# modal-labs/modal-client

Measured on AMD Instinct MI355X. Metric: map_items_per_sec, higher is better.
Workload: dtype bf16; 1 GPU; model=Function.map fan-out (BASELINE config 3), global_batch=12500, seq_len=0, parallelism=map1, dynamic_batching=64, chunk_items=256, workers=8

## Files before the change

csrc/core.cpp:

```cpp

#include <pybind11/pybind11.h>
#include <pybind11/stl.h>

#include "lane.h"
#include "ring.h"

#include <algorithm>
#include <atomic>
#include <functional>
#include <thread>
#include <cerrno>
#include <cstdint>
#include <cstring>
#include <fcntl.h>
#include <stdexcept>
#include <string>
#include <sys/mman.h>
#include <sys/stat.h>
#include <unistd.h>
#include <vector>

namespace py = pybind11;

namespace {

using modal_amd::BellFile;
using modal_amd::Ring;
using modal_amd::RingHub;

constexpr uint64_t kGilReleaseBytes = 64 * 1024;

bool ring_push(Ring& ring, py::buffer buf) {
  py::buffer_info info = buf.request();
  const uint8_t* src = static_cast<const uint8_t*>(info.ptr);
  const uint64_t n = (uint64_t)info.size * (uint64_t)info.itemsize;
  uint8_t* dst = ring.reserve(n);
  if (!dst) return false;
  if (n >= kGilReleaseBytes) {
    py::gil_scoped_release release;
    std::memcpy(dst, src, n);
  } else {
    std::memcpy(dst, src, n);
  }
  ring.commit();
  return true;
}

py::list ring_pop_all(Ring& ring, size_t max_frames) {
  py::list out;
  ring.pop(
      [&](const uint8_t* ptr, size_t len) {
        out.append(py::bytes(reinterpret_cast<const char*>(ptr), len));
      },
      max_frames);
  return out;
}

py::list hub_drain(RingHub& hub) {
  py::list out;
  hub.drain([&](int slot, const uint8_t* ptr, size_t len) {
    out.append(py::make_tuple(slot, py::bytes(reinterpret_cast<const char*>(ptr), len)));
  });
  return out;
}

using modal_amd::Assignment;
using modal_amd::ChunkDone;
using modal_amd::ChunkLane;
using modal_amd::FrameKind;

py::str sv_str(std::string_view s) { return py::str(s.data(), s.size()); }

py::tuple done_tuple(const ChunkDone& d) {
  py::object cis = py::none();
  if (!d.cis_nil) {
    py::list items;
    for (int64_t v : d.cis) items.append(py::int_(v));
    cis = std::move(items);
  }
  return py::make_tuple(sv_str(d.token), sv_str(d.call_id), sv_str(d.chunk_id),
                        sv_str(d.function_id), py::int_(d.count),
                        py::bytes(d.data.data(), d.data.size()), cis);
}

py::list assignment_list(const std::vector<Assignment>& assignments) {
  py::list out;
  for (const auto& a : assignments) out.append(py::make_tuple(a.token, a.worker_slot));
  return out;
}

py::object parse_chunk_done_py(py::buffer buf) {
  py::buffer_info info = buf.request();
  ChunkDone done;
  FrameKind kind = modal_amd::parse_chunk_done(
      static_cast<const uint8_t*>(info.ptr), (size_t)info.size * (size_t)info.itemsize, &done);
  if (kind != FrameKind::kDoneClean) return py::none();
  return done_tuple(done);
}

int lane_submit(ChunkLane& lane, int fn_slot, const std::string& token, uint64_t count,
                py::buffer frame, bool front) {
  py::buffer_info info = frame.request();
  return lane.submit(fn_slot, token, count, static_cast<const uint8_t*>(info.ptr),
                     (size_t)info.size * (size_t)info.itemsize, front);
}

py::tuple lane_drain(ChunkLane& lane, RingHub& hub) {
  py::list completions, raw;
  std::vector<Assignment> assignments;
  lane.drain(
      hub,
      [&](int slot, const ChunkDone& done) {
        completions.append(py::make_tuple(slot, done_tuple(done)));
      },
      [&](int slot, const uint8_t* ptr, size_t len) {
        raw.append(py::make_tuple(slot, py::bytes(reinterpret_cast<const char*>(ptr), len)));
      },
      &assignments);
  return py::make_tuple(completions, raw, assignment_list(assignments));
}

py::bytes pack_payloads(const std::vector<py::bytes>& items) {
  uint64_t total = 0;
  std::vector<std::pair<const char*, size_t>> views;
  views.reserve(items.size());
  for (const auto& item : items) {
    char* ptr;
    Py_ssize_t n;
    if (PyBytes_AsStringAndSize(item.ptr(), &ptr, &n) != 0)
      throw std::runtime_error("pack_payloads: not bytes");
    views.emplace_back(ptr, (size_t)n);
    total += 4 + (uint64_t)n;
  }
  std::string out;
  out.resize(total);
  {
    py::gil_scoped_release release;
    char* dst = out.data();
    for (const auto& [ptr, n] : views) {
      uint32_t len32 = (uint32_t)n;
      std::memcpy(dst, &len32, 4);
      std::memcpy(dst + 4, ptr, n);
      dst += 4 + n;
    }
  }
  return py::bytes(out);
}

py::list unpack_payloads(py::buffer buf) {
  py::buffer_info info = buf.request();
  const char* src = static_cast<const char*>(info.ptr);
  size_t n = (size_t)info.size * (size_t)info.itemsize;
  py::list out;
  size_t pos = 0;
  while (pos + 4 <= n) {
    uint32_t len32;
    std::memcpy(&len32, src + pos, 4);
    if (pos + 4 + len32 > n) throw std::runtime_error("unpack_payloads: truncated");
    out.append(py::bytes(src + pos + 4, len32));
    pos += 4 + len32;
  }
  if (pos != n) throw std::runtime_error("unpack_payloads: trailing bytes");
  return out;
}

}



static constexpr int kSegSize = 4096;
static constexpr int kMinMatch = 4;
static constexpr int kMFLimit = 12;
static constexpr int kLastLiterals = 5;

static inline uint32_t lz4_hash(uint32_t v) { return (v * 2654435761u) >> (32 - 12); }

static size_t lz4_compress_one(const uint8_t* src, size_t n, uint8_t* dst, size_t dst_cap) {
  uint16_t table[1 << 12];
  std::memset(table, 0, sizeof(table));
  size_t op = 0, ip = 0, anchor = 0;
  auto emit = [&](size_t lit_start, size_t lit_len, int match_len) -> bool {
    size_t need = 1 + lit_len + (lit_len >= 15 ? 1 + (lit_len - 15) / 255 : 0) +
                  (match_len >= 0 ? 2 + 1 + 16 : 0);
    if (op + need + 8 > dst_cap) return false;
    int ml = match_len >= 0 ? match_len - kMinMatch : 0;
    uint8_t token = (uint8_t)((lit_len < 15 ? lit_len : 15) << 4);
    if (match_len >= 0) token |= (uint8_t)(ml < 15 ? ml : 15);
    dst[op++] = token;
    if (lit_len >= 15) {
      size_t rest = lit_len - 15;
      while (rest >= 255) { dst[op++] = 255; rest -= 255; }
      dst[op++] = (uint8_t)rest;
    }
    std::memcpy(dst + op, src + lit_start, lit_len);
    op += lit_len;
    return true;
  };
  if (n >= (size_t)(kMinMatch + kLastLiterals)) {
    size_t mflimit = n >= kMFLimit ? n - kMFLimit : 0;
    while (ip < mflimit) {
      uint32_t seq;
      std::memcpy(&seq, src + ip, 4);
      uint32_t h = lz4_hash(seq);
      size_t cand = table[h];
      table[h] = (uint16_t)ip;
      uint32_t cseq;
      bool ok = cand < ip && ip - cand <= 0xFFFF;
      if (ok) { std::memcpy(&cseq, src + cand, 4); ok = cseq == seq; }
      if (ok) {
        size_t mlen = kMinMatch;
        size_t maxm = n - kLastLiterals - ip;
        while (mlen < maxm && src[cand + mlen] == src[ip + mlen]) mlen++;
        if (!emit(anchor, ip - anchor, (int)mlen)) return 0;
        size_t off = ip - cand;
        dst[op++] = (uint8_t)(off & 0xFF);
        dst[op++] = (uint8_t)(off >> 8);
        int ml = (int)mlen - kMinMatch;
        if (ml >= 15) {
          int rest = ml - 15;
          while (rest >= 255) { dst[op++] = 255; rest -= 255; }
          dst[op++] = (uint8_t)rest;
        }
        ip += mlen;
        anchor = ip;
      } else {
        ip++;
      }
    }
  }
  if (!emit(anchor, n - anchor, -1)) return 0;
  return op;
}

static bool lz4_decompress_one(const uint8_t* src, size_t comp_len,
                               uint8_t* dst, size_t raw_len) {
  size_t ip = 0, op = 0;
  while (ip < comp_len) {
    uint8_t token = src[ip++];
    size_t lit = token >> 4;
    if (lit == 15) {
      uint8_t b;
      do { if (ip >= comp_len) return false; b = src[ip++]; lit += b; } while (b == 255);
    }
    if (ip + lit > comp_len || op + lit > raw_len) return false;
    std::memcpy(dst + op, src + ip, lit);
    ip += lit; op += lit;
    if (ip >= comp_len) break;
    if (ip + 2 > comp_len) return false;
    size_t off = src[ip] | ((size_t)src[ip + 1] << 8);
    ip += 2;
    if (off == 0 || off > op) return false;
    size_t mlen = (token & 0xF) + kMinMatch;
    if ((token & 0xF) == 15) {
      uint8_t b;
      do { if (ip >= comp_len) return false; b = src[ip++]; mlen += b; } while (b == 255);
    }
    if (op + mlen > raw_len) return false;
    if (off >= mlen) {
      std::memcpy(dst + op, dst + op - off, mlen);
    } else {
      for (size_t k = 0; k < mlen; k++) dst[op + k] = dst[op - off + k];
    }
    op += mlen;
  }
  return op == raw_len;
}

static void parallel_for(size_t n, const std::function<void(size_t, size_t)>& body) {
  unsigned hw = std::thread::hardware_concurrency();
  size_t n_threads = std::min<size_t>(std::max(1u, hw / 2), 8);
  if (n < 8 || n_threads <= 1) { body(0, n); return; }
  std::vector<std::thread> threads;
  size_t chunk = (n + n_threads - 1) / n_threads;
  for (size_t t = 0; t < n_threads; t++) {
    size_t lo = t * chunk, hi = std::min(n, lo + chunk);
    if (lo >= hi) break;
    threads.emplace_back([&body, lo, hi] { body(lo, hi); });
  }
  for (auto& th : threads) th.join();
}

py::object malz_compress(py::bytes data, double min_gain) {
  char* buf; ssize_t n_s;
  if (PyBytes_AsStringAndSize(data.ptr(), &buf, &n_s) != 0) throw py::error_already_set();
  size_t n = (size_t)n_s;
  size_t n_seg = (n + kSegSize - 1) / kSegSize;
  if (n_seg == 0) return py::none();
  std::vector<uint32_t> comp_lens(n_seg, 0);
  std::vector<std::vector<uint8_t>> outs(n_seg);
  const uint8_t* src = (const uint8_t*)buf;
  {
    py::gil_scoped_release release;
    parallel_for(n_seg, [&](size_t lo, size_t hi) {
      for (size_t i = lo; i < hi; i++) {
        size_t seg_off = i * kSegSize;
        size_t seg_len = std::min((size_t)kSegSize, n - seg_off);
        outs[i].resize(kSegSize);
        size_t c = lz4_compress_one(src + seg_off, seg_len, outs[i].data(), seg_len > 1 ? seg_len - 1 : 0);
        if (c > 0 && c < seg_len) {
          comp_lens[i] = (uint32_t)c;
          outs[i].resize(c);
        } else {
          comp_lens[i] = 0;
          outs[i].clear();
        }
      }
    });
  }
  size_t total = 0;
  for (size_t i = 0; i < n_seg; i++) {
    size_t seg_len = std::min((size_t)kSegSize, n - i * kSegSize);
    total += comp_lens[i] ? comp_lens[i] : seg_len;
  }
  if ((double)total >= (double)n * min_gain) return py::none();
  size_t header = 6 + 12 + 4 * n_seg;
  py::bytes out_obj(nullptr, (ssize_t)(header + total));
  uint8_t* out = (uint8_t*)PyBytes_AsString(out_obj.ptr());
  std::memcpy(out, "MALZ41", 6);
  uint64_t n64 = n;
  uint32_t ns32 = (uint32_t)n_seg;
  std::memcpy(out + 6, &n64, 8);
  std::memcpy(out + 14, &ns32, 4);
  std::memcpy(out + 18, comp_lens.data(), 4 * n_seg);
  size_t op = header;
  for (size_t i = 0; i < n_seg; i++) {
    size_t seg_off = i * kSegSize;
    size_t seg_len = std::min((size_t)kSegSize, n - seg_off);
    if (comp_lens[i]) {
      std::memcpy(out + op, outs[i].data(), comp_lens[i]);
      op += comp_lens[i];
    } else {
      std::memcpy(out + op, src + seg_off, seg_len);
      op += seg_len;
    }
  }
  return out_obj;
}

py::bytes malz_decompress(py::bytes blob) {
  char* buf; ssize_t bn;
  if (PyBytes_AsStringAndSize(blob.ptr(), &buf, &bn) != 0) throw py::error_already_set();
  if (bn < 18 || std::memcmp(buf, "MALZ41", 6) != 0)
    throw std::runtime_error("not a MALZ41 container");
  uint64_t raw_len;
  uint32_t n_seg;
  std::memcpy(&raw_len, buf + 6, 8);
  std::memcpy(&n_seg, buf + 14, 4);
  size_t header = 6 + 12 + 4 * (size_t)n_seg;
  if ((size_t)bn < header) throw std::runtime_error("truncated container header");
  std::vector<uint32_t> comp_lens(n_seg);
  std::memcpy(comp_lens.data(), buf + 18, 4 * (size_t)n_seg);
  std::vector<size_t> seg_payload_off(n_seg);
  size_t pos = header;
  for (size_t i = 0; i < n_seg; i++) {
    seg_payload_off[i] = pos;
    size_t seg_len = std::min((size_t)kSegSize, (size_t)raw_len - i * kSegSize);
    pos += comp_lens[i] ? comp_lens[i] : seg_len;
  }
  if (pos > (size_t)bn) throw std::runtime_error("truncated container payload");
  py::bytes out_obj(nullptr, (ssize_t)raw_len);
  uint8_t* out = (uint8_t*)PyBytes_AsString(out_obj.ptr());
  const uint8_t* src = (const uint8_t*)buf;
  std::atomic<bool> ok{true};
  {
    py::gil_scoped_release release;
    parallel_for(n_seg, [&](size_t lo, size_t hi) {
      for (size_t i = lo; i < hi; i++) {
        size_t seg_off = i * kSegSize;
        size_t seg_len = std::min((size_t)kSegSize, (size_t)raw_len - seg_off);
        if (comp_lens[i] == 0) {
          std::memcpy(out + seg_off, src + seg_payload_off[i], seg_len);
        } else if (!lz4_decompress_one(src + seg_payload_off[i], comp_lens[i],
                                       out + seg_off, seg_len)) {
          ok.store(false, std::memory_order_relaxed);
        }
      }
    });
  }
  if (!ok.load()) throw std::runtime_error("corrupt LZ4 segment");
  return out_obj;
}




#include <sys/syscall.h>
#include <sys/resource.h>
#include <sched.h>
#include <signal.h>

namespace {

struct clone_args_compat {
  uint64_t flags;
  uint64_t pidfd;
  uint64_t child_tid;
  uint64_t parent_tid;
  uint64_t exit_signal;
  uint64_t stack;
  uint64_t stack_size;
  uint64_t tls;
  uint64_t set_tid;
  uint64_t set_tid_size;
  uint64_t cgroup;
};

#ifndef CLONE_INTO_CGROUP
#define CLONE_INTO_CGROUP 0x200000000ULL
#endif

}

static int64_t spawn_supervised(const std::vector<std::string>& argv,
                                const std::string& cwd,
                                const std::vector<std::string>& env,
                                const std::string& cgroup_dir,
                                int64_t rlimit_as_mib,
                                int stdin_fd, int stdout_fd, int stderr_fd) {
  if (argv.empty()) throw std::runtime_error("empty argv");
  int cg_fd = -1;
  if (!cgroup_dir.empty()) {
    cg_fd = ::open(cgroup_dir.c_str(), O_DIRECTORY | O_RDONLY | O_CLOEXEC);
    if (cg_fd < 0)
      throw std::runtime_error("open cgroup dir: " + std::string(strerror(errno)));
  }

  std::vector<char*> cargv;
  cargv.reserve(argv.size() + 1);
  for (const auto& a : argv) cargv.push_back(const_cast<char*>(a.c_str()));
  cargv.push_back(nullptr);
  std::vector<char*> cenv;
  cenv.reserve(env.size() + 1);
  for (const auto& e : env) cenv.push_back(const_cast<char*>(e.c_str()));
  cenv.push_back(nullptr);

  clone_args_compat ca{};
  ca.exit_signal = SIGCHLD;
  if (cg_fd >= 0) {
    ca.flags = CLONE_INTO_CGROUP;
    ca.cgroup = (uint64_t)cg_fd;
  }

  long pid = syscall(SYS_clone3, &ca, sizeof(ca));
  if (pid < 0 && cg_fd >= 0 && (errno == EINVAL || errno == ENOSYS || errno == EPERM ||
                                errno == EBADF || errno == EOPNOTSUPP)) {
    ::close(cg_fd);
    cg_fd = -1;
    throw std::runtime_error("clone3(CLONE_INTO_CGROUP) unavailable: " +
                             std::string(strerror(errno)));
  }
  if (pid < 0) {
    if (cg_fd >= 0) ::close(cg_fd);
    throw std::runtime_error("clone3: " + std::string(strerror(errno)));
  }
  if (pid == 0) {
    ::setsid();
    if (stdin_fd >= 0) ::dup2(stdin_fd, 0);
    if (stdout_fd >= 0) ::dup2(stdout_fd, 1);
    if (stderr_fd >= 0) ::dup2(stderr_fd, 2);
    for (int fd = 3; fd < 1024; ++fd) ::close(fd);
    if (!cwd.empty() && ::chdir(cwd.c_str()) != 0) _exit(126);
    if (rlimit_as_mib > 0) {
      struct rlimit rl;
      rl.rlim_cur = rl.rlim_max = (rlim_t)rlimit_as_mib << 20;
      ::setrlimit(RLIMIT_AS, &rl);
    }
    ::execve(cargv[0], cargv.data(), cenv.data());
    _exit(127);
  }
  if (cg_fd >= 0) ::close(cg_fd);
  return (int64_t)pid;
}


PYBIND11_MODULE(_core, m) {
  m.doc() = "modal_amd native core: shm ring transport + batch framing";
  py::class_<BellFile, std::shared_ptr<BellFile>>(m, "BellFile")
      .def(py::init<const std::string&, bool>(), py::arg("path"), py::arg("create") = false);
  py::class_<Ring, std::shared_ptr<Ring>>(m, "ShmRing")
      .def(py::init<const std::string&, uint64_t, bool>(), py::arg("path"),
           py::arg("capacity") = (uint64_t)64 << 20, py::arg("create") = false)
      .def("push", &ring_push)
      .def("pop_all", &ring_pop_all, py::arg("max_frames") = 0)
      .def("pending_bytes", &Ring::pending_bytes)
      .def("capacity", &Ring::capacity)
      .def("too_large", &Ring::too_large)
      .def("bell_wakes", &Ring::bell_wakes)
      .def("set_shared_bell", &Ring::set_shared_bell);
  py::class_<RingHub>(m, "RingHub")
      .def(py::init<const std::string&, int>(), py::arg("bell_path") = "",
           py::arg("timeout_ms") = 20)
      .def("add_ring", &RingHub::add_ring)
      .def("remove_ring", &RingHub::remove_ring)
      .def("fd", &RingHub::fd)
      .def("drain", &hub_drain)
      .def("close", &RingHub::close)
      .def("stats", [](RingHub& hub) {
        py::dict d;
        d["notifies"] = hub.notifies();
        d["waits"] = hub.waits();
        d["drains"] = hub.drains();
        d["producer_wakes"] = hub.producer_wakes();
        d["rings"] = hub.ring_count();
        return d;
      });
  py::class_<ChunkLane>(m, "ChunkLane")
      .def(py::init<>())
      .def("add_worker", &ChunkLane::add_worker)
      .def("remove_worker", &ChunkLane::remove_worker)
      .def("set_eligible", &ChunkLane::set_eligible)
      .def("set_cap", &ChunkLane::set_cap, py::arg("fn_slot"), py::arg("items"),
           py::arg("min_chunks") = 1)
      .def("submit", &lane_submit, py::arg("fn_slot"), py::arg("token"), py::arg("count"),
           py::arg("frame"), py::arg("front") = false)
      .def("kick", [](ChunkLane& lane, int fn_slot) {
        std::vector<Assignment> out;
        lane.kick(fn_slot, &out);
        return assignment_list(out);
      })
      .def("complete", [](ChunkLane& lane, int worker_slot, const std::string& token) {
        std::vector<Assignment> out;
        lane.complete(worker_slot, token, &out);
        return assignment_list(out);
      })
      .def("cancel", &ChunkLane::cancel)
      .def("drop_queue", &ChunkLane::drop_queue)
      .def("drain", &lane_drain)
      .def("queued", &ChunkLane::queued)
      .def("inflight", &ChunkLane::inflight)
      .def("outstanding_items", &ChunkLane::outstanding_items)
      .def("pushed", &ChunkLane::pushed);
  m.def("parse_chunk_done", &parse_chunk_done_py);
  m.def("pack_payloads", &pack_payloads);
  m.def("malz_compress", &malz_compress, py::arg("data"), py::arg("min_gain") = 0.95);
  m.def("malz_decompress", &malz_decompress);
  m.def("unpack_payloads", &unpack_payloads);
  m.def("spawn_supervised", &spawn_supervised, py::arg("argv"), py::arg("cwd"),
        py::arg("env"), py::arg("cgroup_dir") = "", py::arg("rlimit_as_mib") = 0,
        py::arg("stdin_fd") = -1, py::arg("stdout_fd") = -1, py::arg("stderr_fd") = -1,
        "clone3(CLONE_INTO_CGROUP) + execve supervisor (atomic cgroup placement)");
}
```

csrc/lane.h:

```cpp

#pragma once

#include <algorithm>
#include <cstdint>
#include <cstring>
#include <deque>
#include <memory>
#include <string>
#include <string_view>
#include <unordered_map>
#include <unordered_set>
#include <utility>
#include <vector>

#include "ring.h"

namespace modal_amd {


struct MsgReader {
  const uint8_t* p;
  const uint8_t* end;

  bool need(size_t n) const { return (size_t)(end - p) >= n; }

  bool be(size_t n, uint64_t* out) {
    if (!need(n)) return false;
    uint64_t v = 0;
    for (size_t i = 0; i < n; i++) v = (v << 8) | p[i];
    p += n;
    *out = v;
    return true;
  }

  bool read_str(std::string_view* out) {
    if (!need(1)) return false;
    uint8_t tag = *p++;
    uint64_t n;
    if ((tag & 0xe0) == 0xa0) n = tag & 0x1f;
    else if (tag == 0xd9) { if (!be(1, &n)) return false; }
    else if (tag == 0xda) { if (!be(2, &n)) return false; }
    else if (tag == 0xdb) { if (!be(4, &n)) return false; }
    else return false;
    if (!need(n)) return false;
    *out = std::string_view(reinterpret_cast<const char*>(p), (size_t)n);
    p += n;
    return true;
  }

  bool read_bin(std::string_view* out) {
    if (!need(1)) return false;
    uint8_t tag = *p++;
    uint64_t n;
    if (tag == 0xc4) { if (!be(1, &n)) return false; }
    else if (tag == 0xc5) { if (!be(2, &n)) return false; }
    else if (tag == 0xc6) { if (!be(4, &n)) return false; }
    else return false;
    if (!need(n)) return false;
    *out = std::string_view(reinterpret_cast<const char*>(p), (size_t)n);
    p += n;
    return true;
  }

  bool read_int(int64_t* out) {
    if (!need(1)) return false;
    uint8_t tag = *p++;
    uint64_t v;
    if (tag <= 0x7f) { *out = tag; return true; }
    if (tag >= 0xe0) { *out = (int8_t)tag; return true; }
    switch (tag) {
      case 0xcc: if (!be(1, &v)) return false; *out = (int64_t)v; return true;
      case 0xcd: if (!be(2, &v)) return false; *out = (int64_t)v; return true;
      case 0xce: if (!be(4, &v)) return false; *out = (int64_t)v; return true;
      case 0xcf:
        if (!be(8, &v) || v > (uint64_t)INT64_MAX) return false;
        *out = (int64_t)v;
        return true;
      case 0xd0: if (!be(1, &v)) return false; *out = (int8_t)v; return true;
      case 0xd1: if (!be(2, &v)) return false; *out = (int16_t)v; return true;
      case 0xd2: if (!be(4, &v)) return false; *out = (int32_t)v; return true;
      case 0xd3: if (!be(8, &v)) return false; *out = (int64_t)v; return true;
      default: return false;
    }
  }

  bool read_map_header(uint64_t* n) {
    if (!need(1)) return false;
    uint8_t tag = *p++;
    if ((tag & 0xf0) == 0x80) { *n = tag & 0x0f; return true; }
    if (tag == 0xde) return be(2, n);
    if (tag == 0xdf) return be(4, n);
    return false;
  }

  bool read_array_header(uint64_t* n) {
    if (!need(1)) return false;
    uint8_t tag = *p++;
    if ((tag & 0xf0) == 0x90) { *n = tag & 0x0f; return true; }
    if (tag == 0xdc) return be(2, n);
    if (tag == 0xdd) return be(4, n);
    return false;
  }

  bool skip(int depth = 0) {
    if (depth > 32 || !need(1)) return false;
    uint8_t tag = *p++;
    uint64_t n;
    if (tag <= 0x7f || tag >= 0xe0) return true;
    if ((tag & 0xe0) == 0xa0) return adv(tag & 0x1f);
    if ((tag & 0xf0) == 0x90) return skip_n(tag & 0x0f, depth);
    if ((tag & 0xf0) == 0x80) return skip_n(2 * (uint64_t)(tag & 0x0f), depth);
    switch (tag) {
      case 0xc0: case 0xc2: case 0xc3: return true;
      case 0xc4: case 0xd9: return be(1, &n) && adv(n);
      case 0xc5: case 0xda: return be(2, &n) && adv(n);
      case 0xc6: case 0xdb: return be(4, &n) && adv(n);
      case 0xc7: return be(1, &n) && adv(n + 1);
      case 0xc8: return be(2, &n) && adv(n + 1);
      case 0xc9: return be(4, &n) && adv(n + 1);
      case 0xca: return adv(4);
      case 0xcb: return adv(8);
      case 0xcc: case 0xd0: return adv(1);
      case 0xcd: case 0xd1: return adv(2);
      case 0xce: case 0xd2: return adv(4);
      case 0xcf: case 0xd3: return adv(8);
      case 0xd4: return adv(2);
      case 0xd5: return adv(3);
      case 0xd6: return adv(5);
      case 0xd7: return adv(9);
      case 0xd8: return adv(17);
      case 0xdc: return be(2, &n) && skip_n(n, depth);
      case 0xdd: return be(4, &n) && skip_n(n, depth);
      case 0xde: return be(2, &n) && skip_n(2 * n, depth);
      case 0xdf: return be(4, &n) && skip_n(2 * n, depth);
      default: return false;
    }
  }

 private:
  bool adv(uint64_t n) {
    if (!need(n)) return false;
    p += n;
    return true;
  }
  bool skip_n(uint64_t n, int depth) {
    for (uint64_t i = 0; i < n; i++)
      if (!skip(depth + 1)) return false;
    return true;
  }
};

struct ChunkDone {
  std::string_view token, call_id, chunk_id, function_id, data;
  int64_t count = 0;
  bool cis_nil = true;
  std::vector<int64_t> cis;
};

enum class FrameKind {
  kOther,
  kDoneOther,
  kDoneClean,
};

inline bool ascii_only(std::string_view s) {
  for (unsigned char c : s)
    if (c >= 0x80) return false;
  return true;
}

inline FrameKind parse_chunk_done(const uint8_t* buf, size_t len, ChunkDone* out) {
  MsgReader r{buf, buf + len};
  uint64_t n_keys;
  if (!r.read_map_header(&n_keys)) return FrameKind::kOther;
  enum { T = 1, TOKEN = 2, CALL = 4, CHUNK = 8, FN = 16, COUNT = 32, DATA = 64, CIS = 128 };
  unsigned seen = 0;
  bool clean = n_keys == 8;
  bool is_done = false, has_token = false;
  std::string_view token;
  for (uint64_t i = 0; i < n_keys; i++) {
    std::string_view key;
    const uint8_t* key_at = r.p;
    if (!r.read_str(&key)) {
      r.p = key_at;
      if (!r.skip() || !r.skip()) return FrameKind::kOther;
      clean = false;
      continue;
    }
    unsigned bit = 0;
    if (key == "t") bit = T;
    else if (key == "token") bit = TOKEN;
    else if (key == "call_id") bit = CALL;
    else if (key == "chunk_id") bit = CHUNK;
    else if (key == "function_id") bit = FN;
    else if (key == "count") bit = COUNT;
    else if (key == "data") bit = DATA;
    else if (key == "cis") bit = CIS;
    if (bit == 0 || (seen & bit)) {
      if (bit & (T | TOKEN)) return FrameKind::kOther;
      if (!r.skip()) return FrameKind::kOther;
      clean = false;
      continue;
    }
    seen |= bit;
    const uint8_t* value_at = r.p;
    bool ok = true;
    std::string_view sv;
    switch (bit) {
      case T:
        ok = r.read_str(&sv);
        if (ok) is_done = sv == "chunk_done";
        break;
      case TOKEN:
        ok = r.read_str(&sv) && ascii_only(sv);
        if (ok) { token = sv; has_token = true; }
        break;
      case CALL: ok = r.read_str(&out->call_id) && ascii_only(out->call_id); break;
      case CHUNK: ok = r.read_str(&out->chunk_id) && ascii_only(out->chunk_id); break;
      case FN: ok = r.read_str(&out->function_id) && ascii_only(out->function_id); break;
      case COUNT: ok = r.read_int(&out->count) && out->count >= 0; break;
      case DATA: ok = r.read_bin(&out->data); break;
      case CIS: {
        if (r.need(1) && *r.p == 0xc0) {
          r.p++;
          out->cis_nil = true;
          break;
        }
        uint64_t n;
        ok = r.read_array_header(&n) && n <= (uint64_t)(r.end - r.p);
        out->cis_nil = false;
        out->cis.clear();
        for (uint64_t k = 0; ok && k < n; k++) {
          int64_t v;
          ok = r.read_int(&v);
          if (ok) out->cis.push_back(v);
        }
        break;
      }
    }
    if (!ok) {
      r.p = value_at;
      if (!r.skip()) return FrameKind::kOther;
      clean = false;
      if (bit == T) return FrameKind::kOther;
      if (bit == TOKEN) has_token = false;
    }
  }
  if (r.p != r.end) return FrameKind::kOther;
  if (!is_done || !has_token) return FrameKind::kOther;
  out->token = token;
  if (clean && seen == 255) return FrameKind::kDoneClean;
  return FrameKind::kDoneOther;
}


struct Assignment {
  std::string token;
  int worker_slot;
};

class ChunkLane {
 public:
  void add_worker(int slot, std::shared_ptr<Ring> ring) {
    Worker& w = workers_[slot];
    w.ring = std::move(ring);
  }

  std::vector<std::string> remove_worker(int slot) {
    std::vector<std::string> tokens;
    auto it = workers_.find(slot);
    if (it == workers_.end()) return tokens;
    for (auto& entry : it->second.inflight) tokens.push_back(entry.first);
    workers_.erase(it);
    for (auto& fn : fns_) fn.second.eligible.erase(slot);
    return tokens;
  }

  void set_eligible(int fn_slot, int worker_slot, bool on) {
    Fn& fn = fns_[fn_slot];
    if (on && workers_.count(worker_slot)) fn.eligible.insert(worker_slot);
    else fn.eligible.erase(worker_slot);
  }

  void set_cap(int fn_slot, uint64_t items, uint32_t min_chunks) {
    Fn& fn = fns_[fn_slot];
    fn.cap_items = items;
    fn.min_chunks = min_chunks;
  }

  int submit(int fn_slot, const std::string& token, uint64_t count, const uint8_t* frame,
             size_t len, bool front) {
    Fn& fn = fns_[fn_slot];
    if (fn.queue.empty() || front) {
      int slot = place(fn_slot, fn, token, count, frame, len, fn.queue.size());
      if (slot >= 0) return slot;
    }
    Queued q{token, count, std::string(reinterpret_cast<const char*>(frame), len)};
    if (front) fn.queue.push_front(std::move(q));
    else fn.queue.push_back(std::move(q));
    return -1;
  }

  void kick(int fn_slot, std::vector<Assignment>* out) {
    auto it = fns_.find(fn_slot);
    if (it == fns_.end()) return;
    Fn& fn = it->second;
    while (!fn.queue.empty()) {
      Queued& q = fn.queue.front();
      int slot = place(fn_slot, fn, q.token, q.count,
                       reinterpret_cast<const uint8_t*>(q.frame.data()), q.frame.size(),
                       fn.queue.size());
      if (slot < 0) break;
      out->push_back(Assignment{std::move(q.token), slot});
      fn.queue.pop_front();
    }
  }

  bool complete(int worker_slot, std::string_view token, std::vector<Assignment>* out) {
    auto wit = workers_.find(worker_slot);
    if (wit == workers_.end()) return false;
    Worker& w = wit->second;
    auto it = w.inflight.find(std::string(token));
    if (it == w.inflight.end()) return false;
    int fn_slot = it->second.fn_slot;
    Load& load = w.load[fn_slot];
    load.items -= std::min(load.items, it->second.count);
    if (load.chunks) load.chunks--;
    w.inflight.erase(it);
    kick(fn_slot, out);
    return true;
  }

  std::vector<std::string> cancel(const std::vector<std::string>& tokens) {
    std::unordered_set<std::string_view> drop(tokens.begin(), tokens.end());
    std::vector<std::string> dropped;
    for (auto& entry : fns_) {
      auto& q = entry.second.queue;
      auto keep = q.begin();
      for (auto it = q.begin(); it != q.end(); ++it) {
        if (drop.count(it->token)) {
          dropped.push_back(std::move(it->token));
        } else {
          if (keep != it) *keep = std::move(*it);
          ++keep;
        }
      }
      q.erase(keep, q.end());
    }
    return dropped;
  }

  std::vector<std::string> drop_queue(int fn_slot) {
    std::vector<std::string> tokens;
    auto it = fns_.find(fn_slot);
    if (it == fns_.end()) return tokens;
    for (auto& q : it->second.queue) tokens.push_back(std::move(q.token));
    it->second.queue.clear();
    return tokens;
  }

  template <typename OnClean, typename OnRaw>
  void drain(RingHub& hub, OnClean&& on_clean, OnRaw&& on_raw, std::vector<Assignment>* out) {
    ChunkDone done;
    hub.drain([&](int slot, const uint8_t* ptr, size_t len) {
      FrameKind kind = parse_chunk_done(ptr, len, &done);
      if (kind != FrameKind::kOther) complete(slot, done.token, out);
      if (kind == FrameKind::kDoneClean) on_clean(slot, done);
      else on_raw(slot, ptr, len);
    });
  }

  size_t queued(int fn_slot) const {
    auto it = fns_.find(fn_slot);
    return it == fns_.end() ? 0 : it->second.queue.size();
  }

  size_t inflight(int worker_slot) const {
    auto it = workers_.find(worker_slot);
    return it == workers_.end() ? 0 : it->second.inflight.size();
  }

  uint64_t outstanding_items(int fn_slot, int worker_slot) const {
    auto it = workers_.find(worker_slot);
    if (it == workers_.end()) return 0;
    auto lit = it->second.load.find(fn_slot);
    return lit == it->second.load.end() ? 0 : lit->second.items;
  }

  uint64_t pushed() const { return pushed_; }

 private:
  struct Queued {
    std::string token;
    uint64_t count;
    std::string frame;
  };
  struct Load {
    uint64_t items = 0;
    uint32_t chunks = 0;
  };
  struct Inflight {
    int fn_slot;
    uint64_t count;
  };
  struct Worker {
    std::shared_ptr<Ring> ring;
    std::unordered_map<int, Load> load;
    std::unordered_map<std::string, Inflight> inflight;
  };
  struct Fn {
    uint64_t cap_items = 256;
    uint32_t min_chunks = 1;
    std::deque<Queued> queue;
    std::unordered_set<int> eligible;
  };

  static bool has_credit(const Fn& fn, const Load& load, size_t backlog) {
    if (load.items < fn.cap_items) return true;
    return load.chunks < fn.min_chunks && backlog > fn.eligible.size();
  }

  int place(int fn_slot, Fn& fn, const std::string& token, uint64_t count,
            const uint8_t* frame, size_t len, size_t backlog) {
    std::vector<std::pair<uint64_t, int>> order;
    for (int slot : fn.eligible) {
      auto it = workers_.find(slot);
      if (it == workers_.end()) continue;
      const Load& load = it->second.load[fn_slot];
      if (has_credit(fn, load, backlog)) order.emplace_back(load.items, slot);
    }
    std::sort(order.begin(), order.end());
    for (auto& cand : order) {
      Worker& w = workers_[cand.second];
      if (w.ring->too_large(len) || !w.ring->push(frame, len)) continue;
      Load& load = w.load[fn_slot];
      load.items += count;
      load.chunks++;
      w.inflight[token] = Inflight{fn_slot, count};
      pushed_++;
      return cand.second;
    }
    return -1;
  }

  std::unordered_map<int, Worker> workers_;
  std::unordered_map<int, Fn> fns_;
  uint64_t pushed_ = 0;
};

}
```

modal_amd/flash.py:

```python

from __future__ import annotations

import math
import time
from dataclasses import dataclass, field
from typing import Callable, Optional


@dataclass
class FlashEndpoint:
    name: str
    url: str
    registered_at: float = field(default_factory=time.time)


class FlashManager:

    def __init__(self) -> None:
        self.endpoints: dict[str, FlashEndpoint] = {}

    def register(self, name: str, url: str) -> FlashEndpoint:
        ep = FlashEndpoint(name, url)
        self.endpoints[name] = ep
        return ep

    def deregister(self, name: str) -> None:
        self.endpoints.pop(name, None)

    def list(self) -> list[FlashEndpoint]:
        return list(self.endpoints.values())


class FlashAutoscaler:

    def __init__(
        self,
        get_metric: Callable[[], float],
        target_value: float,
        *,
        min_replicas: int = 1,
        max_replicas: int = 8,
        scale_up_stabilization: float = 0.0,
        scale_down_stabilization: float = 300.0,
        tolerance: float = 0.1,
    ):
        self.get_metric = get_metric
        self.target_value = target_value
        self.min_replicas = min_replicas
        self.max_replicas = max_replicas
        self.scale_up_stabilization = scale_up_stabilization
        self.scale_down_stabilization = scale_down_stabilization
        self.tolerance = tolerance
        self._pending_desired: Optional[int] = None
        self._pending_since: float = 0.0

    def compute_desired(self, current_replicas: int, metric_value: float) -> int:
        if current_replicas == 0:
            return self.min_replicas if metric_value > 0 else 0
        ratio = metric_value / self.target_value
        if abs(ratio - 1.0) <= self.tolerance:
            return current_replicas
        desired = math.ceil(current_replicas * ratio)
        return max(self.min_replicas, min(self.max_replicas, desired))

    def decide(self, current_replicas: int, now: Optional[float] = None) -> int:
        now = now if now is not None else time.time()
        desired = self.compute_desired(current_replicas, self.get_metric())
        if desired == current_replicas:
            self._pending_desired = None
            return current_replicas
        window = (
            self.scale_up_stabilization
            if desired > current_replicas
            else self.scale_down_stabilization
        )
        if self._pending_desired is None or (
            (self._pending_desired > current_replicas) != (desired > current_replicas)
        ):
            self._pending_desired = desired
            self._pending_since = now
        if desired > current_replicas:
            self._pending_desired = min(self._pending_desired, desired)
        else:
            self._pending_desired = max(self._pending_desired, desired)
        if now - self._pending_since >= window:
            applied = self._pending_desired
            self._pending_desired = None
            return applied
        return current_replicas


def scrape_prometheus_metric(url: str, metric_name: str, timeout: float = 2.0) -> Optional[float]:
    import urllib.request

    try:
        with urllib.request.urlopen(url, timeout=timeout) as resp:
            text = resp.read().decode()
    except Exception:
        return None
    total = None
    for line in text.splitlines():
        if line.startswith("#") or not line.startswith(metric_name):
            continue
        head = line.split("{", 1)[0].split(None, 1)[0]
        if head != metric_name:
            continue
        try:
            value = float(line.rsplit(None, 1)[1])
        except (ValueError, IndexError):
            continue
        total = value if total is None else total + value
    return total


class FlashAutoscalerLoop:

    def __init__(
        self,
        scheduler: "object",
        function_id: str,
        target_value: float,
        *,
        metric_urls: Optional[list] = None,
        metric_name: Optional[str] = None,
        get_metric: Optional[Callable[[], float]] = None,
        interval: float = 2.0,
        min_replicas: int = 1,
        max_replicas: int = 8,
        scale_up_stabilization: float = 0.0,
        scale_down_stabilization: float = 60.0,
        tolerance: float = 0.1,
    ):
        self.scheduler = scheduler
        self.function_id = function_id
        self.interval = interval
        self._task = None

        def _metric() -> float:
            if metric_urls and metric_name:
                values = [
                    v
                    for v in (
                        scrape_prometheus_metric(u, metric_name) for u in metric_urls
                    )
                    if v is not None
                ]
                return sum(values) / len(values) if values else 0.0
            if get_metric is not None:
                return get_metric()
            pool = scheduler.pool
            backlog = len(pool.pending.get(function_id, ()))
            inflight = sum(
                w.outstanding.get(function_id, 0) for w in pool.workers.values()
            )
            replicas = max(1, self.current_replicas())
            return (backlog + inflight) / replicas

        self.autoscaler = FlashAutoscaler(
            _metric,
            target_value,
            min_replicas=min_replicas,
            max_replicas=max_replicas,
            scale_up_stabilization=scale_up_stabilization,
            scale_down_stabilization=scale_down_stabilization,
            tolerance=tolerance,
        )

    def current_replicas(self) -> int:
        fdef = self.scheduler.functions.get(self.function_id)
        pool = self.scheduler.pool
        return sum(
            1
            for w in pool.workers.values()
            if w.alive and not w.draining and (fdef is None or w.has_gpu or not fdef.needs_gpu)
        )

    async def tick(self, now: Optional[float] = None) -> int:
        current = self.current_replicas()
        desired = self.autoscaler.decide(current, now)
        if desired > current:
            fdef = self.scheduler.functions.get(self.function_id)
            gpu = 0 if (fdef is not None and fdef.needs_gpu) else None
            for _ in range(desired - current):
                await self.scheduler.pool.spawn_worker(gpu_index=gpu)
        elif desired < current:
            pool = self.scheduler.pool
            victims = [
                w
                for w in pool.workers.values()
                if w.alive and not w.draining and not w.inflight
            ][: current - desired]
            for w in victims:
                w.draining = True
                try:
                    await w.conn.send({"t": "shutdown"})
                except Exception:
                    pass
        return desired

    async def _loop(self) -> None:
        import asyncio

        while True:
            try:
                await self.tick()
            except asyncio.CancelledError:
                raise
            except Exception:
                pass
            await asyncio.sleep(self.interval)

    def start(self) -> None:
        import asyncio

        if self._task is None:
            self._task = asyncio.get_running_loop().create_task(self._loop())

    def stop(self) -> None:
        if self._task is not None:
            self._task.cancel()
            self._task = None
```

modal_amd/scheduler/calls.py:

```python

from __future__ import annotations

import asyncio
import time
from collections import deque
from dataclasses import dataclass, field
from typing import Any, Optional

from ..utils.ids import new_id

GENERIC_STATUS_UNSPECIFIED = 0
GENERIC_STATUS_SUCCESS = 1
GENERIC_STATUS_FAILURE = 2
GENERIC_STATUS_TERMINATED = 3
GENERIC_STATUS_TIMEOUT = 4
GENERIC_STATUS_INTERNAL_FAILURE = 5
GENERIC_STATUS_INIT_FAILURE = 6

MAX_INTERNAL_FAILURE_COUNT = 8

MAX_INPUTS_OUTSTANDING_DEFAULT = 1000


@dataclass
class RetryPolicy:

    max_retries: int = 0
    backoff_coefficient: float = 2.0
    initial_delay_ms: int = 1000
    max_delay_ms: int = 60_000

    def delay_ms(self, retry_count: int) -> float:
        if retry_count <= 0:
            return self.initial_delay_ms
        delay = self.initial_delay_ms * (self.backoff_coefficient ** (retry_count - 1))
        return min(delay, self.max_delay_ms)

    def to_dict(self) -> dict:
        return {
            "max_retries": self.max_retries,
            "backoff_coefficient": self.backoff_coefficient,
            "initial_delay_ms": self.initial_delay_ms,
            "max_delay_ms": self.max_delay_ms,
        }

    @classmethod
    def from_dict(cls, d: Optional[dict]) -> "RetryPolicy":
        return cls(**d) if d else cls()


@dataclass
class FunctionDef:

    function_id: str
    app_id: str
    name: str
    definition: bytes
    definition_kind: str = "serialized"
    is_generator: bool = False
    needs_gpu: bool = False
    gpu_count: int = 0
    timeout: Optional[float] = None
    retry_policy: RetryPolicy = field(default_factory=RetryPolicy)
    max_concurrent_inputs: int = 1
    target_concurrent_inputs: int = 0
    batch_max_size: int = 0
    batch_linger_ms: int = 0
    is_method: bool = False
    is_class_service: bool = False
    cluster_size: int = 0
    min_containers: int = 0
    max_containers: int = 0
    buffer_containers: int = 0
    scaledown_window: float = 60.0
    definition_version: int = 1
    metadata: dict = field(default_factory=dict)
    web_config: Optional[dict] = None
    secret_ids: list = field(default_factory=list)
    volume_mounts: dict = field(default_factory=dict)
    schedule: Optional[dict] = None
    image_id: Optional[str] = None
    placement: Optional[dict] = None
    proxy_url: Optional[str] = None

    def placement_tag(self) -> str:
        return "gpu" if self.needs_gpu else "any"

    def public_metadata(self) -> dict:
        return {
            "function_name": self.name,
            "is_generator": self.is_generator,
            "needs_gpu": self.needs_gpu,
            "is_method": self.is_method,
            "cluster_size": self.cluster_size,
            "batch_max_size": self.batch_max_size,
            "definition_id": self.function_id,
            **self.metadata,
        }


@dataclass(slots=True)
class InputRecord:
    call_id: str
    idx: int
    input_id: str
    payload: bytes
    payload_blob: Optional[str] = None
    method_name: str = ""
    retry_count: int = 0
    internal_failures: int = 0
    status: int = GENERIC_STATUS_UNSPECIFIED
    final: bool = False
    output: Optional[bytes] = None
    output_blob: Optional[str] = None
    output_format: int = 0
    exc_repr: Optional[str] = None
    worker_id: Optional[int] = None
    enqueued_at: float = 0.0
    started_at: float = 0.0
    finished_at: float = 0.0
    tensors: Optional[list] = None
    cancelled: bool = False
    cluster: Optional[dict] = None
    chunk_id: Optional[str] = None
    chunk_index: int = 0
    out_chunk: Optional[str] = None
    out_ci: int = 0

    @property
    def token(self) -> str:
        return f"{self.call_id}:{self.idx}:{self.retry_count}"


class ChunkGroup:

    __slots__ = (
        "chunk_id", "base_idx", "count", "method", "state", "worker_id", "done_cis",
        "internal_failures",
    )

    def __init__(self, chunk_id: str, base_idx: int, count: int, method: str = ""):
        self.chunk_id = chunk_id
        self.base_idx = base_idx
        self.count = count
        self.method = method
        self.state = "pending"
        self.worker_id: Optional[int] = None
        self.done_cis: Optional[set] = None
        self.internal_failures = 0

    @property
    def token(self) -> str:
        return f"g:{self.chunk_id}"


class CallRecord:

    def __init__(
        self,
        function_id: str,
        kind: str,
        return_exceptions: bool = False,
    ):
        self.call_id = new_id("function_call")
        self.function_id = function_id
        self.kind = kind
        self.return_exceptions = return_exceptions
        self.inputs: dict[int, InputRecord] = {}
        self.chunks: dict[str, dict] = {}
        self.chunk_groups: dict[str, ChunkGroup] = {}
        self.next_idx = 0
        self.num_inputs_final: Optional[int] = None
        self.completed: int = 0
        self.cancelled = False
        self.created_at = time.time()
        self.finished_at: Optional[float] = None
        self.output_ready: asyncio.Queue[int] = asyncio.Queue()
        self.output_pushback: deque = deque()
        self._waiters: dict[int, asyncio.Future] = {}
        self.gen_queues: dict[int, asyncio.Queue] = {}
        self.done_event = asyncio.Event()


    def _drop_chunk(self, chunk_id: str) -> None:
        chunk = self.chunks.pop(chunk_id, None)
        if chunk is None:
            return
        data = chunk.get("data")
        if isinstance(data, dict) and data.get("xfer"):
            import os

            try:
                os.unlink(data["xfer"])
            except OSError:
                pass

    def add_input(
        self,
        payload: bytes,
        method_name: str = "",
        tensors: Optional[list] = None,
        payload_blob: Optional[str] = None,
    ) -> InputRecord:
        idx = self.next_idx
        self.next_idx += 1
        rec = InputRecord(
            call_id=self.call_id,
            idx=idx,
            input_id=f"in-{self.call_id[3:]}-{idx}",
            payload=payload,
            payload_blob=payload_blob,
            method_name=method_name,
            enqueued_at=time.time(),
            tensors=tensors,
        )
        self.inputs[idx] = rec
        return rec

    def add_chunk(self, chunk_id: str, payload: Any, count: int, method: str = "") -> ChunkGroup:
        group = ChunkGroup(chunk_id, self.next_idx, count, method)
        self.next_idx += count
        self.chunks[chunk_id] = {"data": payload, "refs": count}
        self.chunk_groups[chunk_id] = group
        return group

    def materialize_chunk_item(self, group: ChunkGroup, ci: int) -> InputRecord:
        idx = group.base_idx + ci
        rec = self.inputs.get(idx)
        if rec is not None:
            return rec
        rec = InputRecord(
            call_id=self.call_id,
            idx=idx,
            input_id=f"in-{self.call_id[3:]}-{idx}",
            payload=b"",
            enqueued_at=time.time(),
            method_name=group.method,
        )
        rec.chunk_id = group.chunk_id
        rec.chunk_index = ci
        self.inputs[idx] = rec
        return rec

    def complete_chunk_success(self, group: ChunkGroup, cis: Optional[list], out_chunk: str) -> None:
        if group.state == "done":
            return
        n = group.count if cis is None else len(cis)
        chunk = self.chunks.get(group.chunk_id)
        if chunk is not None:
            chunk["refs"] -= n
            if chunk["refs"] <= 0:
                self._drop_chunk(group.chunk_id)
        self.completed += n
        if cis is None:
            group.state = "done"
            self.output_ready.put_nowait(("g", group.base_idx, group.count, out_chunk, None))
        else:
            group.done_cis = set(cis)
            group.state = "done"
            self.output_ready.put_nowait(("g", group.base_idx, group.count, out_chunk, list(cis)))
        self._check_done()

    def finish_inputs(self) -> None:
        self.num_inputs_final = self.next_idx
        self._check_done()

    def _check_done(self) -> None:
        if self.num_inputs_final is not None and self.completed >= self.num_inputs_final:
            if not self.done_event.is_set():
                self.finished_at = time.time()
            self.done_event.set()

    def post_output(
        self,
        idx: int,
        status: int,
        output: Optional[bytes],
        output_format: int,
        exc_repr: Optional[str],
        retry_count: int,
        output_blob: Optional[str] = None,
        out_chunk: Optional[str] = None,
        out_ci: int = 0,
    ) -> bool:
        rec = self.inputs.get(idx)
        if rec is None or rec.final:
            return False
        if retry_count != rec.retry_count:
            return False
        rec.status = status
        rec.output = output
        rec.output_blob = output_blob
        rec.out_chunk = out_chunk
        rec.out_ci = out_ci
        rec.output_format = output_format
        rec.exc_repr = exc_repr
        rec.final = True
        rec.finished_at = time.time()
        if rec.chunk_id:
            chunk = self.chunks.get(rec.chunk_id)
            if chunk is not None:
                chunk["refs"] -= 1
                if chunk["refs"] <= 0:
                    self._drop_chunk(rec.chunk_id)
        self.completed += 1
        self.output_ready.put_nowait(idx)
        waiter = self._waiters.pop(idx, None)
        if waiter is not None and not waiter.done():
            waiter.set_result(rec)
        self._check_done()
        return True

    def post_outputs_bulk(self, triples: list, out_chunk: str) -> int:
        ready: list[int] = []
        now = time.time()
        for idx, retry_count, ci in triples:
            rec = self.inputs.get(idx)
            if rec is None or rec.final or retry_count != rec.retry_count:
                continue
            rec.status = GENERIC_STATUS_SUCCESS
            rec.out_chunk = out_chunk
            rec.out_ci = ci
            rec.final = True
            rec.finished_at = now
            if rec.chunk_id:
                chunk = self.chunks.get(rec.chunk_id)
                if chunk is not None:
                    chunk["refs"] -= 1
                    if chunk["refs"] <= 0:
                        self._drop_chunk(rec.chunk_id)
            ready.append(idx)
            waiter = self._waiters.pop(idx, None)
            if waiter is not None and not waiter.done():
                waiter.set_result(rec)
        if ready:
            self.completed += len(ready)
            self.output_ready.put_nowait(ready)
            self._check_done()
        return len(ready)

    async def wait_output(self, idx: int, timeout: Optional[float] = None) -> InputRecord:
        rec = self.inputs[idx]
        if rec.final:
            return rec
        fut = self._waiters.get(idx)
        if fut is None:
            fut = asyncio.get_running_loop().create_future()
            self._waiters[idx] = fut
        if timeout is None:
            return await asyncio.shield(fut)
        return await asyncio.wait_for(asyncio.shield(fut), timeout)

    def gen_queue(self, idx: int) -> asyncio.Queue:
        q = self.gen_queues.get(idx)
        if q is None:
            q = asyncio.Queue()
            self.gen_queues[idx] = q
        return q

    def stats(self) -> dict:
        return {
            "total": self.next_idx,
            "completed": self.completed,
            "pending": self.next_idx - self.completed,
            "final": self.num_inputs_final is not None,
        }
```

modal_amd/scheduler/core.py:

```python

from __future__ import annotations

import asyncio
import logging
import os
import tempfile
import time
from collections import deque
from typing import Any, Optional

from ..exception import InvalidError, NotFoundError
from ..utils.ids import new_id
from .blobs import INLINE_LIMIT, BlobStore
from .calls import (
    GENERIC_STATUS_FAILURE,
    GENERIC_STATUS_INTERNAL_FAILURE,
    GENERIC_STATUS_SUCCESS,
    GENERIC_STATUS_TERMINATED,
    MAX_INPUTS_OUTSTANDING_DEFAULT,
    MAX_INTERNAL_FAILURE_COUNT,
    CallRecord,
    FunctionDef,
    InputRecord,
    RetryPolicy,
)
from .services import Services
from .workerhost import WorkerPool

OUTPUT_POLL_TIMEOUT = 55.0


def _load_or_create_auth_token(run_dir: str) -> str:
    path = os.path.join(run_dir, "auth.token")
    try:
        with open(path) as f:
            token = f.read().strip()
        if token:
            return token
    except OSError:
        pass
    import secrets

    token = secrets.token_hex(16)
    fd = os.open(path, os.O_WRONLY | os.O_CREAT | os.O_TRUNC, 0o600)
    with os.fdopen(fd, "w") as f:
        f.write(token)
    return token


def read_auth_token(socket_path: str) -> str:
    try:
        with open(os.path.join(os.path.dirname(socket_path), "auth.token")) as f:
            return f.read().strip()
    except OSError:
        return ""


class AppState:
    def __init__(self, app_id: str, description: str, ephemeral: bool, environment: str):
        self.app_id = app_id
        self.description = description
        self.ephemeral = ephemeral
        self.environment = environment
        self.state = "running"
        self.created_at = time.time()
        self.last_heartbeat = time.time()
        self.objects: dict[str, tuple[str, dict]] = {}
        self.deployment_name: Optional[str] = None
        self.logs: deque = deque(maxlen=10_000)
        self.log_subscribers: list[asyncio.Queue] = []
        self.log_seq = 0
        self.log_event = asyncio.Event()


class RPCAdapter:

    _ALLOWED = {
        "app_create", "app_publish", "app_heartbeat", "app_client_disconnect", "app_stop",
        "app_list", "app_history", "app_rollback", "app_set_objects", "app_get_object",
        "function_create", "function_update", "function_update_autoscaler",
        "queue_get_or_create", "queue_put", "queue_get", "queue_len", "queue_clear",
        "queue_peek", "queue_delete",
        "dict_get_or_create", "dict_update", "dict_get", "dict_pop", "dict_contains",
        "dict_len", "dict_items", "dict_clear", "dict_delete",
        "secret_get_or_create", "secret_env",
        "blob_put", "blob_get", "blob_path",
        "function_lookup", "function_map", "function_put_inputs", "function_put_chunk",
        "function_finish_inputs",
        "function_get_outputs", "function_call_cancel", "function_call_info",
        "function_get_current_stats", "generator_poll", "node_stats", "node_metrics",
        "container_exec", "container_stop", "endpoint_list",
        "app_lookup", "app_get_layout", "cluster_hello",
        "volume_get_or_create", "volume_put_file_blocks", "volume_get_file", "volume_list_files",
        "volume_remove_file", "volume_copy_files", "volume_commit", "volume_reload",
        "volume_delete", "volume_rename", "volume_dir",
        "sandbox_create", "sandbox_wait", "sandbox_terminate", "sandbox_poll", "sandbox_stdio_read",
        "sandbox_stdin_write", "sandbox_exec", "sandbox_list", "sandbox_set_tags",
        "sandbox_from_name", "sandbox_snapshot_fs", "sandbox_fs_op", "sandbox_resize",
        "sandbox_snapshot_dir", "sandbox_mount_image", "sandbox_unmount_image",
        "sandbox_connect_token", "named_objects_list", "named_object_delete", "image_publish", "image_from_name",
        "proxy_get_or_create", "proxy_stats",
        "image_get_or_create", "image_info", "mount_get_or_create",
        "device_transfer", "tensor_pull_relay",
        "worker_snapshot", "worker_restore", "start_grpc_bridge", "app_get_logs",
        "object_info", "secret_update", "volume_info", "app_set_tags", "app_get_tags",
    }

    def __init__(self, scheduler: "Scheduler"):
        self._scheduler = scheduler

    def __getattr__(self, name: str) -> Any:
        if name in RPCAdapter._ALLOWED:
            return getattr(self._scheduler, name)
        raise AttributeError(name)


class Scheduler:
    def __init__(self, run_dir: Optional[str] = None):
        from ..config import config

        self.run_dir = run_dir or config.get("run_dir") or tempfile.mkdtemp(prefix="modal-amd-")
        os.makedirs(self.run_dir, exist_ok=True)
        try:
            os.chmod(self.run_dir, 0o700)
        except OSError:
            pass
        self.auth_token = _load_or_create_auth_token(self.run_dir)
        self.apps: dict[str, AppState] = {}
        self.app_names: dict[tuple[str, str], str] = {}
        self.functions: dict[str, FunctionDef] = {}
        self.function_names: dict[tuple[str, str, str], str] = {}
        self.calls: dict[str, CallRecord] = {}
        self.out_chunks: dict[str, dict] = {}
        self._out_chunk_order: list[str] = []
        self._out_chunk_seq = 0
        self.services = Services()
        self.blob_store = BlobStore(os.path.join(self.run_dir, "blobs"))
        from .sandboxes import SandboxService
        from .volumes import VolumeService

        self.sandbox_service = SandboxService(self.run_dir)
        self.volume_service = VolumeService(self.run_dir, self.blob_store)
        from .images import ImageService

        self.image_service = ImageService(self.run_dir, self.blob_store)
        self.mounts: dict[str, str] = {}
        self._mounts_by_hash: dict[str, str] = {}
        from .web import WebGateway

        self.web_gateway = WebGateway(self)
        self.pool = WorkerPool(self)
        self.rpc_adapter = RPCAdapter(self)
        self._started = False
        self._start_lock = asyncio.Lock()
        self.default_environment = "main"
        self._extra: dict[str, Any] = {}
        self._persist_task: Optional[asyncio.Task] = None
        self._persist_digest = b""
        from collections import deque as _deque

        self.metrics_counters = {"inputs_total": 0, "outputs_total": 0, "failures_total": 0}
        self._unary_latencies: Any = _deque(maxlen=4096)
        self._rate_window: Any = _deque(maxlen=64)
        from . import persist

        try:
            persist.load(self)
        except Exception:
            logging.getLogger("modal_amd.scheduler").warning(
                "state restore failed", exc_info=True
            )
        try:
            from . import wal

            wal.replay(self)
        except Exception:
            logging.getLogger("modal_amd.scheduler").warning(
                "WAL replay failed", exc_info=True
            )

    async def start(self) -> None:
        async with self._start_lock:
            if self._started:
                return
            await self.pool.start()
            from .cron import ScheduleRunner

            self.schedule_runner = ScheduleRunner(self)
            self.schedule_runner.start()
            self._persist_task = asyncio.get_running_loop().create_task(self._persist_loop())
            self._call_gc_task = asyncio.get_running_loop().create_task(self._call_gc_loop())
            if os.environ.get("MODAL_AMD_GRPC") == "1":
                await self.start_grpc_bridge()
            self._started = True

    async def start_grpc_bridge(self) -> str:
        bridge = self._extra.get("grpc_bridge")
        if bridge is None:
            from ..proto.bridge import GrpcBridge

            bridge = GrpcBridge(self)
            await bridge.start()
            self._extra["grpc_bridge"] = bridge
        return bridge.socket_path

    async def stop(self) -> None:
        if not self._started:
            return
        bridge = self._extra.pop("grpc_bridge", None)
        if bridge is not None:
            try:
                await bridge.stop()
            except Exception:
                pass
        if getattr(self, "schedule_runner", None) is not None:
            self.schedule_runner.stop()
        if self._persist_task is not None:
            self._persist_task.cancel()
            self._persist_task = None
        if getattr(self, "_call_gc_task", None) is not None:
            self._call_gc_task.cancel()
            self._call_gc_task = None
        from . import persist

        try:
            self._persist_digest = persist.save_if_changed(self, self._persist_digest)
        except Exception:
            pass
        await self.sandbox_service.shutdown()
        await self.web_gateway.stop()
        await self.pool.stop()
        self._started = False

    CALL_RETENTION_SECONDS = float(os.environ.get("MODAL_AMD_CALL_RETENTION", "3600"))

    def _gc_calls_once(self) -> int:
        now = time.time()
        dropped = 0
        for call_id, rec in list(self.calls.items()):
            if (
                rec.done_event.is_set()
                and rec.finished_at is not None
                and now - rec.finished_at > self.CALL_RETENTION_SECONDS
            ):
                self.calls.pop(call_id, None)
                for chunk_id in list(rec.chunks):
                    rec._drop_chunk(chunk_id)
                dropped += 1
        for app_id, app in list(self.apps.items()):
            if (
                app.state == "stopped"
                and now - app.last_heartbeat > self.CALL_RETENTION_SECONDS
            ):
                self.apps.pop(app_id, None)
                dropped += 1
        for fid, fdef in list(self.functions.items()):
            if fdef.app_id and fdef.app_id not in self.apps:
                self.functions.pop(fid, None)
                dropped += 1
        self.function_names = {
            k: v for k, v in self.function_names.items() if v in self.functions
        }
        svc = self.sandbox_service
        for sb_id, sb in list(svc.sandboxes.items()):
            if (
                sb.main.returncode is not None
                and all(e.returncode is not None for e in sb.execs.values())
                and now - sb.created_at > self.CALL_RETENTION_SECONDS
            ):
                svc.sandboxes.pop(sb_id, None)
                dropped += 1
        return dropped

    async def _call_gc_loop(self) -> None:
        gc_rounds = 0
        while True:
            await asyncio.sleep(60.0)
            gc_rounds += 1
            if gc_rounds % 10 == 0:
                try:
                    from .isolation import cleanup_stale_cgroups

                    cleanup_stale_cgroups()
                except Exception:
                    pass
            try:
                self._gc_calls_once()
            except Exception:
                pass

    async def _persist_loop(self) -> None:
        from . import persist

        while True:
            await asyncio.sleep(2.0)
            try:
                self._persist_digest = persist.save_if_changed(self, self._persist_digest)
            except Exception:
                logging.getLogger("modal_amd.scheduler").warning(
                    "state snapshot failed", exc_info=True
                )

    def log(self, message: str) -> None:
        import logging

        logging.getLogger("modal_amd.scheduler").debug(message)

    async def app_create(
        self, description: str = "", ephemeral: bool = True, environment: str = ""
    ) -> dict:
        app_id = new_id("app")
        env = environment or self.default_environment
        self.apps[app_id] = AppState(app_id, description, ephemeral, env)
        return {"app_id": app_id}

    async def app_publish(self, app_id: str, name: str) -> dict:
        app = self._app(app_id)
        app.deployment_name = name
        app.state = "deployed"
        app.ephemeral = False
        previous = self.app_names.get((app.environment, name))
        self.app_names[(app.environment, name)] = app_id
        history = self._extra.setdefault("deploy_history", {}).setdefault(
            (app.environment, name), []
        )
        history.append({"app_id": app_id, "deployed_at": time.time(), "version": len(history) + 1})
        for tag, (object_id, _meta) in app.objects.items():
            if object_id.startswith("fu-"):
                self.function_names[(app.environment, name, tag)] = object_id
        return {"app_id": app_id, "url": f"local://{name}", "version": len(history)}

    async def app_history(self, name: str, environment: str = "") -> list:
        env = environment or self.default_environment
        return list(self._extra.get("deploy_history", {}).get((env, name), []))

    async def app_rollback(self, name: str, environment: str = "", version: int = -1) -> dict:
        env = environment or self.default_environment
        history = self._extra.get("deploy_history", {}).get((env, name), [])
        if not history:
            raise NotFoundError(f"No deployment history for '{name}'")
        entry = history[version if version != -1 else -2 if len(history) > 1 else -1]
        app_id = entry["app_id"]
        app = self._app(app_id)
        self.app_names[(env, name)] = app_id
        for tag, (object_id, _meta) in app.objects.items():
            if object_id.startswith("fu-"):
                self.function_names[(env, name, tag)] = object_id
        return {"app_id": app_id, "version": entry["version"]}

    async def app_lookup(self, name: str, environment: str = "") -> dict:
        env = environment or self.default_environment
        app_id = self.app_names.get((env, name))
        if app_id is None:
            raise NotFoundError(f"App '{name}' not found in environment '{env}'")
        return {"app_id": app_id}

    async def app_set_objects(self, app_id: str, objects: dict[str, tuple[str, dict]]) -> None:
        self._app(app_id).objects.update(objects)

    async def app_get_object(self, app_name: str, tag: str, environment: str = "") -> dict:
        env = environment or self.default_environment
        app_id = self.app_names.get((env, app_name))
        if app_id is None:
            raise NotFoundError(f"App '{app_name}' not found in environment '{env}'")
        entry = self._app(app_id).objects.get(tag)
        if entry is None:
            raise NotFoundError(f"App '{app_name}' has no object tagged '{tag}'")
        object_id, meta = entry
        return {"object_id": object_id, "metadata": meta or {}}

    async def app_get_layout(self, app_id: str) -> dict:
        return self.app_layout(app_id)

    def app_layout(self, app_id: str) -> dict:
        app = self.apps.get(app_id)
        if app is None:
            return {"app_id": app_id, "objects": {}}
        return {
            "app_id": app_id,
            "objects": {tag: [oid, meta] for tag, (oid, meta) in app.objects.items()},
        }

    async def app_heartbeat(self, app_id: str) -> None:
        self._app(app_id).last_heartbeat = time.time()

    async def app_client_disconnect(self, app_id: str) -> None:
        app = self.apps.get(app_id)
        if app is None:
            return
        if app.ephemeral:
            app.state = "stopped"
            await self._cancel_app_calls(app_id)
            await self._notify_app_stop(app_id)

    async def _notify_app_stop(self, app_id: str) -> None:

        async def one(w: Any) -> None:
            try:
                await w.conn.call("app_stop", {"app_id": app_id}, timeout=30)
            except Exception:
                pass

        await asyncio.gather(*(one(w) for w in list(self.pool.workers.values())))

    async def app_stop(self, app_id: str) -> None:
        app = self._app(app_id)
        app.state = "stopped"
        if app.deployment_name:
            self.app_names.pop((app.environment, app.deployment_name), None)
        await self._cancel_app_calls(app_id)
        await self._notify_app_stop(app_id)

    async def app_list(self, environment: str = "") -> list[dict]:
        env = environment or self.default_environment
        return [
            {
                "app_id": a.app_id,
                "description": a.description,
                "state": a.state,
                "name": a.deployment_name,
                "created_at": a.created_at,
            }
            for a in self.apps.values()
            if a.environment == env
        ]

    async def _cancel_app_calls(self, app_id: str) -> None:
        fids = {fid for fid, f in self.functions.items() if f.app_id == app_id}
        for call in self.calls.values():
            if call.function_id in fids and not call.done_event.is_set():
                await self.function_call_cancel(call.call_id, terminate_containers=False)

    def _app(self, app_id: str) -> AppState:
        app = self.apps.get(app_id)
        if app is None:
            raise NotFoundError(f"App {app_id} not found")
        return app

    async def function_create(
        self,
        app_id: str,
        name: str,
        definition: bytes,
        options: Optional[dict] = None,
    ) -> dict:
        options = options or {}
        fid = new_id("function")
        fdef = FunctionDef(
            function_id=fid,
            app_id=app_id,
            name=name,
            definition=definition,
            definition_kind=options.get("definition_kind", "serialized"),
            is_generator=bool(options.get("is_generator")),
            needs_gpu=bool(options.get("needs_gpu")),
            gpu_count=int(options.get("gpu_count", 1 if options.get("needs_gpu") else 0)),
            timeout=options.get("timeout"),
            retry_policy=RetryPolicy.from_dict(options.get("retries")),
            max_concurrent_inputs=int(options.get("max_concurrent_inputs", 1)),
            target_concurrent_inputs=int(options.get("target_concurrent_inputs", 0)),
            batch_max_size=int(options.get("batch_max_size", 0)),
            batch_linger_ms=int(options.get("batch_linger_ms", 0)),
            is_method=bool(options.get("is_method")),
            is_class_service=bool(options.get("is_class_service")),
            cluster_size=int(options.get("cluster_size", 0)),
            min_containers=int(options.get("min_containers", 0)),
            max_containers=int(options.get("max_containers", 0)),
            buffer_containers=int(options.get("buffer_containers", 0)),
            scaledown_window=float(options.get("scaledown_window", 60.0)),
            metadata={
                **(options.get("metadata") or {}),
                **(
                    {"enable_memory_snapshot": True}
                    if options.get("enable_memory_snapshot")
                    else {}
                ),
            },
            web_config=options.get("web_config"),
            secret_ids=list(options.get("secret_ids") or []),
            volume_mounts=dict(options.get("volume_mounts") or {}),
            schedule=options.get("schedule"),
            image_id=options.get("image_id"),
            placement=options.get("placement"),
            proxy_url=options.get("proxy_url"),
        )
        self.functions[fid] = fdef
        if fdef.min_containers or fdef.buffer_containers:
            asyncio.get_running_loop().create_task(self.pool.ensure_min(fdef))
        if fdef.web_config:
            await self.web_gateway.ensure_started()
            label = fdef.web_config.get("label") or name
            fdef.metadata["web_url"] = self.web_gateway.register(label, fid)
        app = self.apps.get(app_id)
        if app is not None:
            app.objects[name] = (fid, fdef.public_metadata())
        return {"function_id": fid, "metadata": fdef.public_metadata()}

    async def function_update(self, function_id: str, definition: bytes, options: Optional[dict] = None) -> None:
        fdef = self.functions[function_id]
        fdef.definition = definition
        fdef.definition_version += 1
        for key, value in (options or {}).items():
            if hasattr(fdef, key):
                setattr(fdef, key, value)

    async def function_lookup(self, app_name: str, name: str, environment: str = "") -> dict:
        env = environment or self.default_environment
        fid = self.function_names.get((env, app_name, name))
        if fid is None:
            raise NotFoundError(f"Function '{app_name}/{name}' not found")
        return {"function_id": fid, "metadata": self.functions[fid].public_metadata()}

    async def node_stats(self) -> dict:
        workers = []
        for w in self.pool.workers.values():
            row = {
                "worker_id": w.worker_id,
                "task_id": w.task_id,
                "gpu_index": w.gpu_index,
                "alive": w.alive,
                "inflight": len(w.inflight),
                "last_heartbeat_age": max(0.0, time.time() - w.last_heartbeat),
            }
            if w.gpu_stats:
                row["gpu"] = w.gpu_stats
            workers.append(row)
        return {
            "workers": workers,
            "pending_inputs": sum(len(q) for q in self.pool.pending.values()),
            "active_calls": sum(
                1 for c in self.calls.values() if not c.done_event.is_set()
            ),
        }

    def _worker_by_task(self, task_id: str) -> Any:
        for w in self.pool.workers.values():
            if w.task_id == task_id:
                return w
        raise NotFoundError(f"Container {task_id} not found")

    async def container_exec(self, task_id: str, cmd: list, timeout: float = 60.0) -> dict:
        w = self._worker_by_task(task_id)
        return await w.conn.call("exec_command", {"cmd": cmd, "timeout": timeout}, timeout=timeout + 10)

    async def container_stop(self, task_id: str) -> None:
        w = self._worker_by_task(task_id)
        w.draining = True
        await w.conn.send({"t": "shutdown"})

    async def endpoint_list(self) -> list:
        gw = self.web_gateway
        return [
            {"label": label, "function_id": fid,
             "url": gw.url_for(label) if gw.port else None}
            for label, fid in gw.routes.items()
        ]

    async def node_metrics(self) -> str:
        now = time.time()
        counters = self.metrics_counters
        self._rate_window.append((now, counters["outputs_total"]))
        lines = [
            "# TYPE modal_amd_inputs_total counter",
            f"modal_amd_inputs_total {counters['inputs_total']}",
            "# TYPE modal_amd_outputs_total counter",
            f"modal_amd_outputs_total {counters['outputs_total']}",
            "# TYPE modal_amd_failures_total counter",
            f"modal_amd_failures_total {counters['failures_total']}",
        ]
        if len(self._rate_window) >= 2:
            (t0, c0), (t1, c1) = self._rate_window[0], self._rate_window[-1]
            if t1 > t0:
                lines += [
                    "# TYPE modal_amd_items_per_sec gauge",
                    f"modal_amd_items_per_sec {(c1 - c0) / (t1 - t0):.3f}",
                ]
        if self._unary_latencies:
            lat = sorted(self._unary_latencies)
            lines += [
                "# TYPE modal_amd_unary_latency_seconds summary",
                f'modal_amd_unary_latency_seconds{{quantile="0.5"}} {lat[len(lat) // 2]:.6f}',
                f'modal_amd_unary_latency_seconds{{quantile="0.99"}} {lat[min(len(lat) - 1, int(len(lat) * 0.99))]:.6f}',
            ]
        lines += [
            "# TYPE modal_amd_workers gauge",
            f"modal_amd_workers {len(self.pool.workers)}",
            "# TYPE modal_amd_pending_inputs gauge",
            f"modal_amd_pending_inputs {sum(len(q) for q in self.pool.pending.values())}",
            "# TYPE modal_amd_active_calls gauge",
            f"modal_amd_active_calls {sum(1 for c in self.calls.values() if not c.done_event.is_set())}",
        ]
        gpu_lines = []
        for w in self.pool.workers.values():
            if w.gpu_stats and w.gpu_index is not None:
                g = w.gpu_stats
                gpu_lines.append(
                    f'modal_amd_gpu_hbm_free_bytes{{gpu="{w.gpu_index}",worker="{w.worker_id}"}} {g.get("hbm_free", 0)}'
                )
                gpu_lines.append(
                    f'modal_amd_gpu_hbm_total_bytes{{gpu="{w.gpu_index}",worker="{w.worker_id}"}} {g.get("hbm_total", 0)}'
                )
        if gpu_lines:
            lines.append("# TYPE modal_amd_gpu_hbm_free_bytes gauge")
            lines.extend(gpu_lines)
        return "\n".join(lines) + "\n"

    async def function_get_current_stats(self, function_id: str) -> dict:
        backlog = len(self.pool.pending.get(function_id, ()))
        runners = sum(
            1 for w in self.pool.workers.values() if w.outstanding.get(function_id, 0) > 0
        )
        return {"backlog": backlog, "num_total_tasks": runners}

    async def function_update_autoscaler(
        self,
        function_id: str,
        min_containers: Optional[int] = None,
        max_containers: Optional[int] = None,
        buffer_containers: Optional[int] = None,
        scaledown_window: Optional[float] = None,
    ) -> None:
        fdef = self.functions[function_id]
        if min_containers is not None:
            fdef.min_containers = min_containers
        if max_containers is not None:
            fdef.max_containers = max_containers
        if buffer_containers is not None:
            fdef.buffer_containers = buffer_containers
        if scaledown_window is not None:
            fdef.scaledown_window = scaledown_window

    async def function_map(
        self,
        function_id: str,
        kind: str = "unary",
        pipelined_inputs: Optional[list] = None,
        return_exceptions: bool = False,
    ) -> dict:
        if function_id not in self.functions:
            raise NotFoundError(f"Function {function_id} not found")
        record = CallRecord(function_id, kind, return_exceptions)
        self.calls[record.call_id] = record
        from . import wal

        if wal.journaled(self, record):
            record.durable = True
            wal.journal_created(self, record)
        if pipelined_inputs:
            await self.function_put_inputs(record.call_id, pipelined_inputs)
        return {
            "function_call_id": record.call_id,
            "retry_policy": self.functions[function_id].retry_policy.to_dict(),
            "max_inputs_outstanding": max(
                MAX_INPUTS_OUTSTANDING_DEFAULT,
                1024 * max(
                    sum(1 for w in self.pool.workers.values() if w.alive), 1
                ),
            ),
            "sync_client_retries_enabled": True,
        }

    async def function_put_inputs(
        self, function_call_id: str, items: list, chunks: Optional[dict] = None
    ) -> list:
        record = self._call(function_call_id)
        self.metrics_counters["inputs_total"] += len(items)
        fdef = self.functions.get(record.function_id)
        if chunks:
            for chunk_id, data in chunks.items():
                record.chunks[chunk_id] = {"data": data, "refs": 0}
        out = []
        batch_recs = []
        for item in items:
            if isinstance(item, (bytes, bytearray)):
                item = {"payload": bytes(item)}
            if fdef is not None and fdef.cluster_size > 1:
                recs = await self._put_gang_input(record, fdef, item)
                out.append({"idx": recs[0].idx, "input_id": recs[0].input_id})
                continue
            rec = record.add_input(
                item.get("payload") or b"",
                item.get("method", ""),
                tensors=item.get("tensors"),
                payload_blob=item.get("payload_blob"),
            )
            if getattr(record, "durable", False):
                from . import wal

                wal.journal_input(self, record, rec)
            chunk_id = item.get("chunk")
            if chunk_id:
                rec.chunk_id = chunk_id
                rec.chunk_index = item.get("ci", 0)
                chunk = record.chunks.get(chunk_id)
                if chunk is not None:
                    chunk["refs"] += 1
            batch_recs.append(rec)
            out.append({"idx": rec.idx, "input_id": rec.input_id})
        if batch_recs:
            self.pool.enqueue_many(record.function_id, batch_recs)
        return out

    async def _put_gang_input(self, record: CallRecord, fdef: FunctionDef, item: dict) -> list:
        import socket

        n = fdef.cluster_size
        cluster_id = new_id("task")
        sock = socket.socket()
        sock.bind(("127.0.0.1", 0))
        port = sock.getsockname()[1]
        sock.close()
        recs = []
        for rank in range(n):
            rec = record.add_input(
                item.get("payload") or b"",
                item.get("method", ""),
                payload_blob=item.get("payload_blob"),
            )
            rec.cluster = {
                "rank": rank,
                "size": n,
                "cluster_id": cluster_id,
                "master_port": port,
            }
            recs.append(rec)
        await self.pool.dispatch_gang(fdef, recs)
        return recs

    async def function_put_chunk(
        self,
        function_call_id: str,
        chunk_id: str,
        payload: Any,
        count: int,
        method: str = "",
    ) -> dict:
        record = self._call(function_call_id)
        fdef = self.functions.get(record.function_id)
        fast = (
            fdef is not None
            and fdef.cluster_size <= 1
            and not fdef.is_generator
            and not fdef.timeout
            and not fdef.web_config
            and not os.environ.get("MODAL_AMD_NO_RANGE")
        )
        if not fast:
            items = [{"chunk": chunk_id, "ci": ci, "method": method} for ci in range(count)]
            return {
                "items": await self.function_put_inputs(
                    function_call_id, items, chunks={chunk_id: payload}
                )
            }
        group = record.add_chunk(chunk_id, payload, count, method)
        self.metrics_counters["inputs_total"] += count
        self.pool.enqueue_chunk(record, group, record.function_id)
        return {"idx_base": group.base_idx, "count": count}

    async def function_finish_inputs(self, function_call_id: str) -> None:
        record = self._call(function_call_id)
        record.finish_inputs()
        if getattr(record, "durable", False):
            from . import wal

            wal.journal_finish(self, record)

    async def function_wait_output(
        self, function_call_id: str, idx: int = 0, timeout: Optional[float] = None
    ) -> InputRecord:
        return await self._call(function_call_id).wait_output(idx, timeout)

    async def function_get_outputs(
        self,
        function_call_id: str,
        max_values: int = 256,
        timeout: float = OUTPUT_POLL_TIMEOUT,
        clear_on_success: bool = True,
    ) -> list[dict]:
        record = self._call(function_call_id)
        out: list[dict] = []
        n_vals = 0

        def expand(entry: Any) -> None:
            nonlocal n_vals
            if type(entry) is tuple and entry and entry[0] == "g":
                _tag, base, count, out_chunk, cis = entry[:5]
                val_off = entry[5] if len(entry) > 5 else 0
                n = count if cis is None else len(cis)
                budget = max_values - n_vals
                if n > budget:
                    cis_full = list(range(count)) if cis is None else cis
                    head, tail = cis_full[:budget], cis_full[budget:]
                    if head:
                        out.append(
                            {
                                "group": True,
                                "idx_base": base,
                                "count": count,
                                "cis": head,
                                "val_off": val_off,
                                "out_chunk": out_chunk,
                                "status": 1,
                            }
                        )
                        n_vals += len(head)
                    record.output_pushback.append(
                        ("g", base, count, out_chunk, tail, val_off + len(head))
                    )
                    return
                out.append(
                    {
                        "group": True,
                        "idx_base": base,
                        "count": count,
                        "cis": cis,
                        "val_off": val_off,
                        "out_chunk": out_chunk,
                        "status": 1,
                    }
                )
                n_vals += n
            elif isinstance(entry, list):
                for pos, idx in enumerate(entry):
                    if n_vals >= max_values:
                        record.output_pushback.append(entry[pos:])
                        return
                    out.append(self._output_item(record, idx))
                    n_vals += 1
            else:
                out.append(self._output_item(record, entry))
                n_vals += 1

        def take_nowait() -> Any:
            if record.output_pushback:
                return record.output_pushback.popleft()
            return record.output_ready.get_nowait()

        deadline = time.time() + timeout
        while not out:
            if record.output_pushback:
                entry = record.output_pushback.popleft()
            else:
                try:
                    remaining = deadline - time.time()
                    if remaining <= 0:
                        break
                    entry = await asyncio.wait_for(record.output_ready.get(), remaining)
                except asyncio.TimeoutError:
                    break
            expand(entry)
            while n_vals < max_values:
                try:
                    entry = take_nowait()
                except asyncio.QueueEmpty:
                    break
                expand(entry)
        chunks_seen: set[str] = set()
        for item in out:
            cid = item.get("out_chunk")
            if cid and cid not in chunks_seen:
                chunks_seen.add(cid)
                chunk = self.out_chunks.get(cid)
                if chunk is not None:
                    item["chunk_data"] = chunk["data"]
        if clear_on_success:
            for item in out:
                cid = item.get("out_chunk")
                if item.get("group"):
                    n = item["count"] if item["cis"] is None else len(item["cis"])
                else:
                    n = 1
                    rec = record.inputs.get(item["idx"])
                    if rec is not None:
                        rec.payload = b""
                if cid:
                    chunk = self.out_chunks.get(cid)
                    if chunk is not None:
                        chunk["refs"] -= n
                        if chunk["refs"] <= 0:
                            self.out_chunks.pop(cid, None)
        return out

    def _output_item(self, record: CallRecord, idx: int) -> dict:
        rec = record.inputs[idx]
        item = {
            "idx": idx,
            "input_id": rec.input_id,
            "status": rec.status,
            "data": rec.output,
            "data_blob": rec.output_blob,
            "format": rec.output_format,
            "exc": rec.exc_repr,
            "retry_count": rec.retry_count,
        }
        if rec.out_chunk:
            item["out_chunk"] = rec.out_chunk
            item["out_ci"] = rec.out_ci
        return item

    async def function_call_cancel(
        self, function_call_id: str, terminate_containers: bool = False
    ) -> None:
        record = self._call(function_call_id)
        record.cancelled = True
        tokens = []
        for rec in record.inputs.values():
            if not rec.final:
                rec.cancelled = True
                tokens.append(rec.token)
                self.finalize_input(
                    rec, GENERIC_STATUS_TERMINATED, None, 0, "input cancelled", rec.retry_count
                )
        for group in record.chunk_groups.values():
            if group.state != "done":
                group.state = "done"
                tokens.append(group.token)
                for ci in range(group.count):
                    if record.inputs.get(group.base_idx + ci) is not None:
                        continue
                    rec = record.materialize_chunk_item(group, ci)
                    rec.cancelled = True
                    self.finalize_input(
                        rec, GENERIC_STATUS_TERMINATED, None, 0, "input cancelled", rec.retry_count
                    )
        await self.pool.cancel_inputs(tokens, terminate=terminate_containers)

    async def function_call_info(self, function_call_id: str) -> dict:
        record = self._call(function_call_id)
        return {
            "function_call_id": record.call_id,
            "function_id": record.function_id,
            "kind": record.kind,
            **record.stats(),
        }

    def _call(self, function_call_id: str) -> CallRecord:
        record = self.calls.get(function_call_id)
        if record is None:
            raise NotFoundError(f"Function call {function_call_id} not found")
        return record

    def register_out_chunk(self, data: bytes, refs: int) -> str:
        self._out_chunk_seq += 1
        chunk_id = f"oc{self._out_chunk_seq}"
        self.out_chunks[chunk_id] = {"data": data, "refs": refs}
        self._out_chunk_order.append(chunk_id)
        while len(self._out_chunk_order) > 20_000:
            old = self._out_chunk_order.pop(0)
            self.out_chunks.pop(old, None)
        return chunk_id

    def on_worker_output(
        self,
        call_id: str,
        idx: int,
        retry_count: int,
        status: int,
        output: Optional[bytes],
        output_format: int,
        exc_repr: Optional[str],
        output_blob: Optional[str] = None,
        out_chunk: Optional[str] = None,
        out_ci: int = 0,
    ) -> None:
        record = self.calls.get(call_id)
        if record is None:
            return
        rec = record.inputs.get(idx)
        if rec is None or rec.final or rec.retry_count != retry_count:
            return
        fdef = self.functions.get(record.function_id)
        if rec.cluster is not None and status in (
            GENERIC_STATUS_FAILURE,
            GENERIC_STATUS_INTERNAL_FAILURE,
        ):
            asyncio.get_running_loop().create_task(
                self._fail_gang_siblings(record, rec, exc_repr)
            )
        elif status == GENERIC_STATUS_FAILURE and fdef is not None:
            policy = fdef.retry_policy
            if rec.retry_count < policy.max_retries and not rec.cancelled:
                rec.retry_count += 1
                delay_s = policy.delay_ms(rec.retry_count) / 1000.0
                if delay_s <= 0:
                    self.pool.enqueue(rec)
                else:
                    self.pool.enqueue_delayed(rec, delay_s)
                return
        elif status == GENERIC_STATUS_INTERNAL_FAILURE:
            rec.internal_failures += 1
            if rec.internal_failures <= MAX_INTERNAL_FAILURE_COUNT and not rec.cancelled:
                self.pool.enqueue(rec, front=True)
                return
        self.finalize_input(
            rec, status, output, output_format, exc_repr, retry_count, output_blob,
            out_chunk, out_ci,
        )

    async def _fail_gang_siblings(self, record: CallRecord, failed: InputRecord, exc_repr: Optional[str]) -> None:
        try:
            await self._fail_gang_siblings_inner(record, failed, exc_repr)
        except Exception:
            logging.getLogger("modal_amd.scheduler").warning(
                "gang teardown failed", exc_info=True
            )

    async def _fail_gang_siblings_inner(
        self, record: CallRecord, failed: InputRecord, exc_repr: Optional[str]
    ) -> None:
        cluster_id = failed.cluster["cluster_id"]
        siblings = [
            r
            for r in record.inputs.values()
            if r.cluster is not None
            and r.cluster["cluster_id"] == cluster_id
            and r.idx != failed.idx
            and not r.final
        ]
        tokens = []
        for r in siblings:
            r.cancelled = True
            tokens.append(r.token)
        if tokens:
            await self.pool.cancel_inputs(tokens, terminate=True)
        for r in siblings:
            if not r.final:
                self.finalize_input(
                    r,
                    GENERIC_STATUS_TERMINATED,
                    None,
                    0,
                    f"gang member rank {failed.cluster['rank']} failed: {exc_repr}",
                    r.retry_count,
                )

    def finalize_input(
        self,
        rec: InputRecord,
        status: int,
        output: Optional[bytes],
        output_format: int,
        exc_repr: Optional[str],
        retry_count: int,
        output_blob: Optional[str] = None,
        out_chunk: Optional[str] = None,
        out_ci: int = 0,
    ) -> None:
        record = self.calls.get(rec.call_id)
        if record is None:
            return
        self.metrics_counters["outputs_total"] += 1
        if status != GENERIC_STATUS_SUCCESS:
            self.metrics_counters["failures_total"] += 1
        if record.kind == "unary":
            self._unary_latencies.append(time.time() - record.created_at)
        record.post_output(
            rec.idx, status, output, output_format, exc_repr, retry_count, output_blob,
            out_chunk, out_ci,
        )
        if getattr(record, "durable", False) and rec.final:
            from . import wal

            wal.journal_result(self, record, rec)
            if (
                record.num_inputs_final is not None
                and record.completed >= record.num_inputs_final
            ):
                wal.drop(self, record.call_id)

    def on_generator_data(self, msg: dict) -> None:
        call_id, idx_s, _ = msg["token"].rsplit(":", 2)
        record = self.calls.get(call_id)
        if record is None:
            return
        record.gen_queue(int(idx_s)).put_nowait(
            (msg.get("index", 0), msg.get("data"), msg.get("format", 0), bool(msg.get("done")))
        )

    async def generator_poll(
        self, function_call_id: str, idx: int = 0, timeout: float = OUTPUT_POLL_TIMEOUT
    ) -> list:
        record = self._call(function_call_id)
        q = record.gen_queue(idx)
        out = []
        try:
            item = await asyncio.wait_for(q.get(), timeout)
            out.append(list(item))
            while True:
                out.append(list(q.get_nowait()))
        except (asyncio.TimeoutError, asyncio.QueueEmpty):
            pass
        return out

    def on_worker_log(self, handle: Any, msg: dict) -> None:
        app_id = msg.get("app_id", "")
        entry = {
            "ts": time.time(),
            "task_id": handle.task_id,
            "fd": msg.get("fd", 1),
            "data": msg.get("data", ""),
            "app_id": app_id,
        }
        app = self.apps.get(app_id)
        if app is not None:
            app.logs.append(entry)
            app.log_seq += 1
            app.log_event.set()
            for sub in app.log_subscribers:
                sub.put_nowait(entry)
        else:
            for a in self.apps.values():
                if a.state == "running":
                    for sub in a.log_subscribers:
                        sub.put_nowait(entry)

    def resolve_function_env(self, fdef: FunctionDef) -> dict[str, str]:
        env: dict[str, str] = {}
        if fdef.image_id:
            state = self.image_service.by_id.get(fdef.image_id)
            if state is not None:
                env.update(state.env)
        for secret_id in fdef.secret_ids:
            try:
                env.update(self.services.secret_env(secret_id))
            except Exception:
                pass
        if fdef.proxy_url:
            env["HTTP_PROXY"] = env["http_proxy"] = fdef.proxy_url
            env["HTTPS_PROXY"] = env["https_proxy"] = fdef.proxy_url
        return env

    def resolve_function_pythonpaths(self, fdef: FunctionDef) -> list[str]:
        if fdef.image_id:
            state = self.image_service.by_id.get(fdef.image_id)
            if state is not None:
                return list(state.python_paths)
        return []

    async def ensure_mesh(self) -> dict:
        state = self._extra.setdefault(
            "mesh", {"formed": False, "ranks": {}, "lock": asyncio.Lock(), "ready": {}}
        )
        async with state["lock"]:
            if state["formed"]:
                return state
            members = [w for w in self.pool.workers.values() if w.alive]
            gpu_members = [w for w in members if w.has_gpu]
            if gpu_members and self.pool._gpu_count() > 0:
                members = gpu_members
                backend = "nccl"
            else:
                backend = "gloo"
            if len(members) < 2:
                raise NotFoundError("device mesh needs >= 2 workers")
            members.sort(key=lambda w: w.worker_id)
            import socket as socket_mod

            sock = socket_mod.socket()
            sock.bind(("127.0.0.1", 0))
            port = sock.getsockname()[1]
            sock.close()
            ranks = {w.task_id: i for i, w in enumerate(members)}
            events = {w.task_id: asyncio.Event() for w in members}
            state["ready"] = events
            for w in members:
                await w.conn.send(
                    {
                        "t": "mesh_init",
                        "rank": ranks[w.task_id],
                        "world": len(members),
                        "port": port,
                        "backend": backend,
                    }
                )
            await asyncio.wait_for(
                asyncio.gather(*(e.wait() for e in events.values())), timeout=120
            )
            state["ranks"] = ranks
            state["backend"] = backend
            state["formed"] = True
            return state

    def on_mesh_ready(self, handle: Any, ok: bool) -> None:
        state = self._extra.get("mesh")
        if state:
            event = state["ready"].get(handle.task_id)
            if event is not None and ok:
                event.set()

    def _worker_by_task(self, task_id: str) -> Any:
        for w in self.pool.workers.values():
            if w.task_id == task_id:
                return w
        return None

    async def device_transfer(
        self, owner_task: str, token: str, meta: dict, dest_task: str
    ) -> dict:
        try:
            state = await self.ensure_mesh()
        except Exception:
            return {"fallback": True}
        ranks = state["ranks"]
        if owner_task not in ranks or dest_task not in ranks or owner_task == dest_task:
            return {"fallback": True}
        owner = self._worker_by_task(owner_task)
        dest = self._worker_by_task(dest_task)
        if owner is None or dest is None:
            return {"fallback": True}
        xfer_id = new_id("blob")
        await dest.conn.send(
            {"t": "dev_recv", "xfer_id": xfer_id, "meta": meta, "src_rank": ranks[owner_task]}
        )
        await owner.conn.send(
            {"t": "dev_send", "token": token, "dst_rank": ranks[dest_task], "xfer_id": xfer_id}
        )
        return {"xfer_id": xfer_id, "src_rank": ranks[owner_task]}

    async def tensor_pull_relay(self, owner_task: str, token: str) -> Optional[bytes]:
        owner = self._worker_by_task(owner_task)
        if owner is None:
            return None
        return await owner.conn.call("tensor_pull", {"token": token}, timeout=120)

    async def cluster_hello(self, cluster_id: str, rank: int, world_size: int, addr: str = "") -> dict:
        key = f"cluster:{cluster_id}"
        state = self._extra.setdefault(key, {"members": {}, "event": asyncio.Event()})
        state["members"][rank] = addr
        if len(state["members"]) >= world_size:
            state["event"].set()
        await state["event"].wait()
        return {
            "cluster_id": cluster_id,
            "rank": rank,
            "world_size": world_size,
            "addrs": [state["members"].get(r, "") for r in range(world_size)],
        }

    async def app_get_logs(
        self,
        app_id: str,
        offset: int = 0,
        timeout: float = 55.0,
        max_entries: int = 1000,
    ) -> dict:
        app = self._app(app_id)
        deadline = time.time() + min(timeout, OUTPUT_POLL_TIMEOUT)
        while app.log_seq <= offset:
            remaining = deadline - time.time()
            if remaining <= 0 or app.state == "stopped":
                return {"entries": [], "next_offset": offset, "dropped": 0,
                        "app_state": app.state}
            app.log_event.clear()
            try:
                await asyncio.wait_for(app.log_event.wait(), remaining)
            except asyncio.TimeoutError:
                pass
        oldest = app.log_seq - len(app.logs)
        start = max(offset, oldest)
        dropped = start - offset
        skip = start - oldest
        entries = list(app.logs)[skip : skip + max_entries]
        return {
            "entries": entries,
            "next_offset": start + len(entries),
            "dropped": dropped,
            "app_state": app.state,
        }

    async def worker_snapshot(
        self, worker_id: int, block_addressed: bool = False, float_codec: Any = False
    ) -> dict:
        if float_codec not in (False, True, "auto"):
            raise InvalidError(f'float_codec is False, True or "auto", got {float_codec!r}')
        if float_codec and not block_addressed:
            raise InvalidError("float_codec needs block_addressed=True")
        w = self.pool.workers.get(int(worker_id))
        if w is None:
            raise NotFoundError(f"worker {worker_id} not connected")
        rpc = "snapshot_manifest" if block_addressed else "snapshot_state"
        params = {"float_codec": float_codec} if float_codec else None
        data = await w.conn.call(rpc, params, timeout=300)
        blob_id = self.blob_store.put(data)
        return {"snapshot_id": blob_id}

    async def worker_restore(
        self, snapshot_id: str, gpu_index: Optional[int] = None
    ) -> dict:
        import json as _json

        state_path = os.path.join(self.run_dir, f"restore-{new_id('task')[3:]}.json")
        state = {
            "task_id": new_id("task"),
            "snapshot_id": snapshot_id,
            "snapshot_path": self.blob_store.open_path(snapshot_id),
            "blob_root": self.blob_store.root,
            "env": {},
            "snapshot_debug": False,
        }
        with open(state_path, "w") as f:
            _json.dump(state, f)
        wid = self.pool._next_worker_id
        proc = await self.pool.spawn_worker(
            gpu_index=gpu_index,
            extra_env={"MODAL_AMD_RESTORE_STATE_PATH": state_path},
        )
        deadline = time.time() + 120
        while time.time() < deadline:
            if wid in self.pool.workers:
                return {"worker_id": wid, "degraded": False}
            rc = proc.poll() if proc is not None else None
            if rc is not None:
                self.pool._pending_spawns = max(0, self.pool._pending_spawns - 1)
                wid2 = self.pool._next_worker_id
                await self.pool.spawn_worker(gpu_index=gpu_index)
                while time.time() < deadline:
                    if wid2 in self.pool.workers:
                        return {"worker_id": wid2, "degraded": True, "exit_code": rc}
                    await asyncio.sleep(0.1)
                break
            await asyncio.sleep(0.1)
        raise InvalidError("restored worker never connected")

    async def named_objects_list(self, kind: str, environment: str = "") -> list:
        env = environment or self.default_environment
        if kind == "volume":
            store = self.volume_service.by_name
        elif kind == "queue":
            store = self.services.queue_names.by_name
        elif kind == "dict":
            store = self.services.dict_names.by_name
        elif kind == "secret":
            store = self.services.secret_names.by_name
        else:
            raise InvalidError(f"Unknown object kind {kind!r}")
        return [
            {"name": name, "object_id": oid}
            for (e, name), oid in sorted(store.items())
            if e == env
        ]

    async def named_object_delete(self, kind: str, name: str, environment: str = "") -> None:
        env = environment or self.default_environment
        rows = await self.named_objects_list(kind, env)
        oid = next((r["object_id"] for r in rows if r["name"] == name), None)
        if oid is None:
            raise NotFoundError(f"{kind} '{name}' not found in environment '{env}'")
        if kind == "volume":
            await self.volume_service.delete(oid)
        elif kind == "queue":
            self.services.queue_delete(oid)
        elif kind == "dict":
            self.services.dict_delete(oid)
        elif kind == "secret":
            self.services.secrets.pop(oid, None)
            self.services.secret_names.by_name = {
                k: v for k, v in self.services.secret_names.by_name.items() if v != oid
            }

    async def object_info(self, object_id: str) -> dict:
        return self.services.object_info(object_id)

    async def volume_info(self, volume_id: str) -> dict:
        vol = self.volume_service._get(volume_id)
        return {
            "name": vol.name,
            "files": len(vol.manifest),
            "created_at": getattr(vol, "created_at", None),
        }

    async def secret_update(self, secret_id: str, env: dict) -> None:
        st = self.services.secrets.get(secret_id)
        if st is None:
            raise NotFoundError(f"Secret {secret_id} not found")
        st.env.update({k: str(v) for k, v in env.items()})

    async def app_set_tags(self, app_id: str, tags: dict) -> None:
        app = self._app(app_id)
        if not hasattr(app, "tags"):
            app.tags = {}
        app.tags.update({str(k): str(v) for k, v in tags.items()})

    async def app_get_tags(self, app_id: str) -> dict:
        return dict(getattr(self._app(app_id), "tags", {}) or {})

    async def blob_put(self, data: bytes) -> dict:
        digest = await asyncio.get_running_loop().run_in_executor(None, self.blob_store.put, data)
        return {"blob_id": digest}

    async def blob_get(self, blob_id: str) -> bytes:
        return await asyncio.get_running_loop().run_in_executor(None, self.blob_store.get, blob_id)

    async def blob_path(self, blob_id: str) -> str:
        return self.blob_store.open_path(blob_id)

    def maybe_blob(self, payload: bytes, limit: int = INLINE_LIMIT) -> dict:
        if len(payload) <= limit:
            return {"payload": payload}
        digest = self.blob_store.put(payload)
        return {"payload_blob": digest}

    async def volume_get_or_create(self, name=None, environment="main", create_if_missing=False, ephemeral=False) -> dict:
        return await self.volume_service.get_or_create(name, environment, create_if_missing, ephemeral)

    async def volume_put_file_blocks(
        self, volume_id, rel_path, block_digests, size, mode=0o644, content_tmp=None
    ) -> dict:
        return await self.volume_service.put_file_blocks(
            volume_id, rel_path, block_digests, size, mode, content_tmp=content_tmp
        )

    async def volume_get_file(self, volume_id, rel_path, offset=0, n_bytes=-1) -> bytes:
        return await self.volume_service.get_file(volume_id, rel_path, offset, n_bytes)

    async def volume_list_files(self, volume_id, rel_path="/", recursive=True) -> list:
        return await self.volume_service.list_files(volume_id, rel_path, recursive)

    async def volume_remove_file(self, volume_id, rel_path, recursive=False) -> None:
        return await self.volume_service.remove_file(volume_id, rel_path, recursive)

    async def volume_copy_files(self, volume_id, src_paths, dst_path) -> None:
        return await self.volume_service.copy_files(volume_id, src_paths, dst_path)

    async def volume_commit(self, volume_id) -> dict:
        return await self.volume_service.commit(volume_id)

    async def volume_reload(self, volume_id) -> None:
        return await self.volume_service.reload(volume_id)

    async def volume_delete(self, volume_id) -> None:
        return await self.volume_service.delete(volume_id)

    async def volume_rename(self, volume_id, new_name, environment="main") -> None:
        return await self.volume_service.rename(volume_id, new_name, environment)

    async def volume_dir(self, volume_id) -> str:
        return self.volume_service.volume_dir(volume_id)

    async def sandbox_create(self, **kwargs: Any) -> dict:
        volume_mounts = kwargs.pop("volume_mounts", None) or {}
        volume_paths = {}
        for path, spec in volume_mounts.items():
            vid = spec["volume_id"] if isinstance(spec, dict) else spec
            vol_dir = self.volume_service.volume_dir(vid)
            if isinstance(spec, dict) and spec.get("sub_path"):
                vol_dir = os.path.join(vol_dir, spec["sub_path"].strip("/"))
                os.makedirs(vol_dir, exist_ok=True)
            volume_paths[path] = vol_dir
        restore_image = kwargs.pop("restore_image_id", None)
        restore_blob = None
        image_fsroot = None
        if restore_image:
            restore_blob = self._extra.get("snapshot_blobs", {}).get(restore_image)
            img = self.image_service.by_id.get(restore_image)
            if img is not None and os.path.isdir(img.fsroot) and os.listdir(img.fsroot):
                image_fsroot = img.fsroot
        return await self.sandbox_service.create(
            volume_paths=volume_paths,
            restore_blob=restore_blob,
            image_fsroot=image_fsroot,
            blob_store=self.blob_store,
            **kwargs,
        )

    async def sandbox_exec(
        self, sandbox_id, cmd, env=None, workdir=None, timeout=None, exec_id=None,
        pty=False, rows=24, cols=80,
    ) -> dict:
        return await self.sandbox_service.exec(
            sandbox_id, cmd, env, workdir, timeout, exec_id, pty=pty, rows=rows, cols=cols
        )

    async def sandbox_resize(self, target_id, rows, cols) -> None:
        await self.sandbox_service.resize(target_id, rows, cols)

    async def sandbox_stdio_read(self, target_id, fd, offset=0, max_bytes=1 << 20, timeout=55.0) -> dict:
        return await self.sandbox_service.stdio_read(target_id, fd, offset, max_bytes, timeout)

    async def sandbox_stdin_write(self, target_id, offset, data, eof=False) -> int:
        return await self.sandbox_service.stdin_write(target_id, offset, data, eof)

    async def sandbox_wait(self, target_id, timeout=None, raise_on_timeout=True) -> dict:
        return await self.sandbox_service.wait(target_id, timeout, raise_on_timeout)

    async def sandbox_poll(self, target_id) -> dict:
        return await self.sandbox_service.poll(target_id)

    async def sandbox_terminate(self, sandbox_id) -> None:
        return await self.sandbox_service.terminate(sandbox_id)

    async def sandbox_list(self, app_id=None, tags=None) -> list:
        return await self.sandbox_service.list(app_id, tags)

    async def sandbox_set_tags(self, sandbox_id, tags) -> None:
        return await self.sandbox_service.set_tags(sandbox_id, tags)

    async def sandbox_from_name(self, name, environment="main") -> dict:
        sid = await self.sandbox_service.from_name(name, environment)
        return {"sandbox_id": sid}

    async def sandbox_snapshot_fs(self, sandbox_id) -> dict:
        resp = await self.sandbox_service.snapshot_fs(sandbox_id, self.blob_store)
        self._extra.setdefault("snapshot_blobs", {})[resp["image_id"]] = resp["blob_id"]
        return resp

    async def sandbox_snapshot_dir(self, sandbox_id: str, path: str) -> dict:
        import shutil

        sb = self.sandbox_service._get(sandbox_id)
        src = os.path.normpath(os.path.join(sb.workdir, path.lstrip("/")))
        if not os.path.isdir(src):
            raise InvalidError(f"{path!r} is not a directory in sandbox {sandbox_id}")
        resp = await self.image_service.get_or_create(
            [{"kind": "base", "name": "snapshot", "sandbox": sandbox_id, "path": path,
              "nonce": os.urandom(8).hex()}],
            build=False,
        )
        state = self.image_service.by_id[resp["image_id"]]
        dst = os.path.join(state.fsroot, path.lstrip("/"))
        await asyncio.get_running_loop().run_in_executor(
            None, lambda: shutil.copytree(src, dst, symlinks=True)
        )
        state.built = True
        state.build_log = f"snapshot of {sandbox_id}:{path}"
        return {"image_id": state.image_id}

    async def sandbox_mount_image(self, sandbox_id: str, path: str, image_id: str) -> None:
        sb = self.sandbox_service._get(sandbox_id)
        state = self.image_service.by_id.get(image_id)
        if state is None:
            raise NotFoundError(f"Image {image_id} not found")
        link = os.path.normpath(os.path.join(sb.workdir, path.lstrip("/")))
        src = os.path.join(state.fsroot, path.lstrip("/"))
        if not os.path.isdir(src):
            src = state.fsroot
        os.makedirs(os.path.dirname(link), exist_ok=True)
        if os.path.islink(link):
            os.unlink(link)
        elif os.path.exists(link):
            raise InvalidError(f"{path!r} already exists in sandbox {sandbox_id}")
        os.symlink(src, link)

    async def sandbox_unmount_image(self, sandbox_id: str, path: str) -> None:
        sb = self.sandbox_service._get(sandbox_id)
        link = os.path.normpath(os.path.join(sb.workdir, path.lstrip("/")))
        if os.path.islink(link):
            os.unlink(link)

    async def sandbox_connect_token(
        self, sandbox_id: str, port: int = 8080, user_metadata: Any = None
    ) -> dict:
        if not isinstance(port, int) or not (1 <= port <= 65535):
            raise InvalidError("port must be between 1 and 65535")
        self.sandbox_service._get(sandbox_id)
        import secrets as _secrets

        token = _secrets.token_urlsafe(24)
        self._extra.setdefault("sandbox_connect_tokens", {})[token] = {
            "sandbox_id": sandbox_id,
            "port": port,
            "user_metadata": user_metadata,
            "created_at": time.time(),
        }
        return {"url": f"http://127.0.0.1:{port}", "token": token}

    async def sandbox_fs_op(self, sandbox_id: str, op: str, path: str = "", **kwargs: Any) -> Any:
        sb = self.sandbox_service._get(sandbox_id)
        base = sb.workdir
        full = os.path.normpath(os.path.join(base, path.lstrip("/"))) if path else base
        loop = asyncio.get_running_loop()
        if op == "read":
            def _read() -> bytes:
                with open(full, "rb") as f:
                    f.seek(kwargs.get("offset", 0))
                    return f.read(kwargs.get("n", -1))

            return await loop.run_in_executor(None, _read)
        if op == "write":
            def _write() -> int:
                mode = "ab" if kwargs.get("append") else ("r+b" if kwargs.get("offset") else "wb")
                if kwargs.get("offset") and not os.path.exists(full):
                    open(full, "wb").close()
                with open(full, mode) as f:
                    if kwargs.get("offset"):
                        f.seek(kwargs["offset"])
                    return f.write(kwargs.get("data", b""))

            return await loop.run_in_executor(None, _write)
        if op == "ls":
            return sorted(os.listdir(full))
        if op == "stat":
            st = os.stat(full)
            return {"size": st.st_size, "mtime": st.st_mtime, "is_dir": os.path.isdir(full)}
        if op == "mkdir":
            os.makedirs(full, exist_ok=kwargs.get("parents", False) or kwargs.get("exist_ok", False))
            return None
        if op == "rm":
            if os.path.isdir(full) and not os.path.islink(full):
                if kwargs.get("recursive"):
                    import shutil

                    shutil.rmtree(full)
                else:
                    os.rmdir(full)
            else:
                os.unlink(full)
            return None
        if op == "exists":
            return os.path.exists(full)
        raise InvalidError(f"Unknown fs op {op!r}")

    async def proxy_get_or_create(self, name: str, environment: str = "") -> dict:
        from .localproxy import LocalForwardProxy

        proxy = self._extra.get("local_proxy")
        if proxy is None:
            proxy = LocalForwardProxy()
            await proxy.start()
            self._extra["local_proxy"] = proxy
        env = environment or self.default_environment
        ids = self._extra.setdefault("proxy_ids", {})
        pid = ids.get((env, name))
        if pid is None:
            pid = new_id("tunnel")
            ids[(env, name)] = pid
        return {"proxy_id": pid, "url": proxy.url, "port": proxy.port}

    async def proxy_stats(self) -> dict:
        proxy = self._extra.get("local_proxy")
        if proxy is None:
            return {"running": False}
        return {
            "running": True,
            "port": proxy.port,
            "connections": proxy.connections,
            "bytes_relayed": proxy.bytes_relayed,
        }

    async def image_get_or_create(self, recipe: list) -> dict:
        return await self.image_service.get_or_create(recipe)

    async def image_info(self, image_id: str) -> dict:
        return await self.image_service.info(image_id)

    async def image_publish(self, image_id: str, name: str, environment: str = "") -> dict:
        if self.image_service.by_id.get(image_id) is None:
            raise NotFoundError(f"Image {image_id} not found")
        env = environment or self.default_environment
        if ":" not in name:
            name = f"{name}:latest"
        self._extra.setdefault("image_names", {})[(env, name)] = image_id
        return {"name": name}

    async def image_from_name(self, name: str, environment: str = "") -> dict:
        env = environment or self.default_environment
        if ":" not in name:
            name = f"{name}:latest"
        image_id = self._extra.get("image_names", {}).get((env, name))
        if image_id is None:
            raise NotFoundError(f"Image '{name}' not found in environment '{env}'")
        return {"image_id": image_id}

    async def mount_get_or_create(self, manifest: list) -> dict:
        import hashlib
        import json as _json

        key = hashlib.sha256(
            _json.dumps(sorted(manifest), sort_keys=True).encode()
        ).hexdigest()
        existing = self._mounts_by_hash.get(key)
        if existing:
            return {"mount_id": existing, "dir": self.mounts[existing]}
        mount_id = new_id("mount")
        root = os.path.join(self.run_dir, "mounts", mount_id)
        for remote_path, blob_id, _mode in manifest:
            dest = os.path.join(root, remote_path.lstrip("/"))
            self.blob_store.materialize(blob_id, dest)
        self.mounts[mount_id] = root
        self._mounts_by_hash[key] = mount_id
        return {"mount_id": mount_id, "dir": root}

    def __getattr__(self, name: str) -> Any:
        if name.startswith(("queue_", "dict_", "secret_")):
            target = getattr(self.services, name, None)
            if target is not None:
                if asyncio.iscoroutinefunction(target):
                    return target

                async def _async_wrap(*args: Any, **kwargs: Any) -> Any:
                    return target(*args, **kwargs)

                return _async_wrap
        raise AttributeError(name)
```

modal_amd/scheduler/workerhost.py:

```python

from __future__ import annotations

import asyncio
import heapq
import os
import subprocess
import sys
import time
from collections import deque
from typing import TYPE_CHECKING, Any, Optional

import msgpack

from ..utils.ids import new_id
from .calls import (
    GENERIC_STATUS_INTERNAL_FAILURE,
    MAX_INTERNAL_FAILURE_COUNT,
    FunctionDef,
    InputRecord,
)
from .transport import Connection, _core, native_lane_enabled

_CPU_COUNT = os.cpu_count()

if TYPE_CHECKING:
    from .core import Scheduler

DEFAULT_PIPELINE_DEPTH = 256

LANE_MIN_CHUNKS = max(1, int(os.environ.get("MODAL_AMD_LANE_MIN_CHUNKS", "1")))
LANE_MAX_FRAME = 8 << 20


class WorkerHandle:
    def __init__(
        self,
        worker_id: int,
        conn: Connection,
        gpu_index: Optional[int],
        proc: Optional[subprocess.Popen] = None,
        external: bool = False,
    ):
        self.worker_id = worker_id
        self.task_id = new_id("task")
        self.conn = conn
        self.gpu_index = gpu_index
        self.proc = proc
        self.external = external
        self.alive = True
        self.last_heartbeat = time.time()
        self.last_active = time.time()
        self.gpu_stats: Optional[dict] = None
        self.paged = False
        self.inflight: dict[str, InputRecord] = {}
        self.outstanding: dict[str, int] = {}
        self.functions_loaded: set[str] = set()
        self.defs_version: dict[str, int] = {}
        self.chunks_sent: set[str] = set()
        self.draining = False
        self.hub_slot: Optional[int] = None
        self.lane_fns: set[str] = set()

    @property
    def has_gpu(self) -> bool:
        return self.gpu_index is not None

    def credit_for(self, fdef: FunctionDef) -> int:
        return credit_cap(fdef) - self.outstanding.get(fdef.function_id, 0)


def credit_cap(fdef: FunctionDef) -> int:
    cap = max(fdef.max_concurrent_inputs * 2, DEFAULT_PIPELINE_DEPTH)
    if fdef.batch_max_size:
        cap = max(cap, fdef.batch_max_size * 2)
    return cap


class WorkerPool:
    def __init__(self, scheduler: "Scheduler"):
        self.scheduler = scheduler
        self.run_dir = scheduler.run_dir
        self.socket_path = os.path.join(self.run_dir, "scheduler.sock")
        self.workers: dict[int, WorkerHandle] = {}
        self._next_worker_id = 0
        self._server: Optional[asyncio.AbstractServer] = None
        self._dispatch_wake = asyncio.Event()
        self._dispatch_task: Optional[asyncio.Task] = None
        self._retry_task: Optional[asyncio.Task] = None
        self._stopping = False
        self.pending: dict[str, deque[InputRecord]] = {}
        self.delayed: list[tuple[float, int, str, InputRecord]] = []
        self._delay_seq = 0
        self._spawn_lock = asyncio.Lock()
        self._pending_spawns = 0
        self._worker_ready = asyncio.Event()
        self._procs: list[subprocess.Popen] = []
        self._hub: Any = None
        self._hub_bell = os.path.join(self.run_dir, "hub.bell")
        self._hub_conns: dict[int, Connection] = {}
        self._next_hub_slot = 0
        self._lane: Any = None
        self._lane_workers: dict[int, WorkerHandle] = {}
        self._lane_fn_slots: dict[str, int] = {}
        self._lane_fn_version: dict[str, Optional[int]] = {}
        self._lane_groups: dict[str, tuple] = {}
        self._lane_refresh_fns: set[str] = set()

    def _start_hub(self) -> None:
        if not native_lane_enabled():
            return
        try:
            self._hub = _core.RingHub(self._hub_bell, 20)
            self._lane = _core.ChunkLane()
            asyncio.get_running_loop().add_reader(self._hub.fd(), self._on_hub_ready)
        except Exception as exc:
            self._hub = None
            self._lane = None
            self.scheduler.log(f"native lane unavailable: {exc!r}")

    def _stop_hub(self) -> None:
        hub, self._hub = self._hub, None
        self._lane = None
        if hub is not None:
            try:
                asyncio.get_running_loop().remove_reader(hub.fd())
            except Exception:
                pass
            hub.close()
        self._hub_conns.clear()
        self._lane_workers.clear()

    def _on_hub_ready(self) -> None:
        hub, lane = self._hub, self._lane
        if hub is None or lane is None:
            return
        completions, raw_frames, assignments = lane.drain(hub)
        for token, slot in assignments:
            self._lane_assigned(token, slot)
        workers = self._lane_workers
        for slot, fields in completions:
            w = workers.get(slot)
            if w is not None:
                w.conn.ring_frames_received += 1
                try:
                    self._chunk_done_fields(w, *fields)
                except Exception as exc:
                    self.scheduler.log(f"lane completion error: {exc!r}")
        conns = self._hub_conns
        for slot, body in raw_frames:
            conn = conns.get(slot)
            if conn is not None:
                try:
                    conn.on_ring_frame(body)
                except Exception as exc:
                    self.scheduler.log(f"lane frame error: {exc!r}")

    def _lane_fn_slot(self, fdef: FunctionDef) -> int:
        fid = fdef.function_id
        slot = self._lane_fn_slots.get(fid)
        if slot is None:
            slot = self._lane_fn_slots[fid] = len(self._lane_fn_slots)
            self._lane_fn_version[fid] = None
        if self._lane_fn_version[fid] != fdef.definition_version:
            for w in self._lane_workers.values():
                if fid in w.lane_fns:
                    w.lane_fns.discard(fid)
                    self._lane.set_eligible(slot, w.hub_slot, False)
            self._lane.set_cap(slot, credit_cap(fdef), LANE_MIN_CHUNKS)
            self._lane_fn_version[fid] = fdef.definition_version
        return slot

    def _lane_submit(self, record: Any, group: Any, fdef: FunctionDef, front: bool) -> bool:
        if self._lane is None or not self._lane_workers:
            return False
        chunk = record.chunks.get(group.chunk_id) or {}
        frame = msgpack.packb(
            {
                "t": "inputs_chunk",
                "function_id": fdef.function_id,
                "call_id": record.call_id,
                "chunk_id": group.chunk_id,
                "token": group.token,
                "count": group.count,
                "payload": chunk.get("data"),
                "method": group.method,
                "max_concurrent": fdef.max_concurrent_inputs,
            },
            use_bin_type=True,
        )
        if len(frame) > LANE_MAX_FRAME:
            return False
        fn_slot = self._lane_fn_slot(fdef)
        token = group.token
        self._lane_groups[token] = (record, group)
        slot = self._lane.submit(fn_slot, token, group.count, frame, front)
        if slot >= 0:
            self._lane_assigned(token, slot)
        else:
            self._lane_refresh_fns.add(fdef.function_id)
            self._dispatch_wake.set()
        return True

    def _lane_assigned(self, token: str, slot: int) -> None:
        entry = self._lane_groups.get(token)
        w = self._lane_workers.get(slot)
        if entry is None or w is None:
            return
        record, group = entry
        group.state = "inflight"
        group.worker_id = w.worker_id
        w.last_active = time.time()
        w.inflight[token] = ("g", record, group)
        w.conn.ring_frames_sent += 1
        fid = record.function_id
        w.outstanding[fid] = w.outstanding.get(fid, 0) + group.count

    def _lane_revoke(self, w: WorkerHandle) -> None:
        if self._lane is not None and w.hub_slot is not None:
            for fid in w.lane_fns:
                self._lane.set_eligible(self._lane_fn_slots[fid], w.hub_slot, False)
        w.lane_fns.clear()

    async def _lane_dispatch(self) -> None:
        lane = self._lane
        for fid in list(self._lane_refresh_fns):
            self._lane_refresh_fns.discard(fid)
            fn_slot = self._lane_fn_slots.get(fid)
            if lane is None or fn_slot is None:
                continue
            fdef = self.scheduler.functions.get(fid)
            if fdef is None:
                for token in lane.drop_queue(fn_slot):
                    self._lane_groups.pop(token, None)
                continue
            fn_slot = self._lane_fn_slot(fdef)
            await self.ensure_workers(fdef.needs_gpu)
            candidates = [
                w
                for w in self.workers.values()
                if w.alive and not w.draining and (w.has_gpu or not fdef.needs_gpu)
            ]
            candidates = self._apply_placement(fdef, candidates)
            chosen = {w.worker_id for w in candidates}
            for w in list(self._lane_workers.values()):
                if fid in w.lane_fns and w.worker_id not in chosen:
                    w.lane_fns.discard(fid)
                    lane.set_eligible(fn_slot, w.hub_slot, False)
            for w in candidates:
                if w.hub_slot is None or (fid in w.lane_fns and not w.paged):
                    continue
                try:
                    await self._ensure_unpaged(w)
                    if w.defs_version.get(fid, 0) != fdef.definition_version or (
                        fid not in w.functions_loaded
                    ):
                        await self._send_def(w, fdef)
                except Exception:
                    continue
                if (
                    w.alive
                    and not w.draining
                    and not w.paged
                    and w.hub_slot in self._lane_workers
                    and self._lane_fn_version.get(fid) == fdef.definition_version
                ):
                    w.lane_fns.add(fid)
                    lane.set_eligible(fn_slot, w.hub_slot, True)
            for token, slot in lane.kick(fn_slot):
                self._lane_assigned(token, slot)
            backlog = lane.queued(fn_slot)
            if backlog:
                await self._maybe_scale_up(fdef, backlog=backlog, active=len(candidates))

    async def start(self) -> None:
        os.makedirs(self.run_dir, exist_ok=True)
        self._start_hub()
        self._server = await asyncio.start_unix_server(self._on_connect, path=self.socket_path)
        try:
            os.chmod(self.socket_path, 0o600)
        except OSError:
            pass
        self._dispatch_task = asyncio.get_running_loop().create_task(self._dispatch_loop())
        self._retry_task = asyncio.get_running_loop().create_task(self._retry_loop())
        self._health_task = asyncio.get_running_loop().create_task(self._health_loop())

    async def _scaledown_once(self) -> None:
        window = min(
            (f.scaledown_window for f in self.scheduler.functions.values() if f.scaledown_window),
            default=60.0,
        )
        floor = max(
            (f.min_containers + f.buffer_containers for f in self.scheduler.functions.values()),
            default=0,
        )
        now = time.time()
        idle = [
            w
            for w in self.workers.values()
            if w.alive
            and not w.draining
            and not w.inflight
            and not w.external
            and now - w.last_active > window
        ]
        reapable = []
        for w in idle:
            if not w.paged and self._hosts_snapshot_fn(w):
                self._lane_revoke(w)
                w.paged = True
                try:
                    await w.conn.call("gpu_snapshot", timeout=120)
                except Exception:
                    w.paged = False
                continue
            if w.paged:
                continue
            reapable.append(w)
        alive = sum(1 for w in self.workers.values() if w.alive)
        excess = alive - max(floor, 1)
        for w in reapable[: max(excess, 0)]:
            w.draining = True
            self._lane_revoke(w)
            try:
                await w.conn.send({"t": "shutdown"})
            except Exception:
                pass

    def _hosts_snapshot_fn(self, w: WorkerHandle) -> bool:
        for fid in w.functions_loaded:
            fdef = self.scheduler.functions.get(fid)
            if fdef is not None and fdef.metadata.get("enable_memory_snapshot"):
                return True
        return False

    async def _ensure_unpaged(self, w: WorkerHandle) -> None:
        if w.paged:
            w.paged = False
            try:
                await w.conn.call("gpu_restore", timeout=300)
            except Exception:
                pass

    async def _health_loop(self) -> None:
        while True:
            await asyncio.sleep(15.0)
            try:
                await self._scaledown_once()
            except Exception:
                pass
            now = time.time()
            for w in list(self.workers.values()):
                if not w.alive:
                    continue
                stale = now - w.last_heartbeat
                if stale > 60.0 and w.inflight:
                    self.scheduler.log(
                        f"worker {w.worker_id} missed heartbeats for {stale:.0f}s; recycling"
                    )
                    try:
                        if w.proc is not None:
                            w.proc.kill()
                    except Exception:
                        pass
                    await w.conn.close()

    async def stop(self) -> None:
        self._stopping = True
        for task in (self._dispatch_task, self._retry_task, getattr(self, "_health_task", None)):
            if task is not None:
                task.cancel()
        for w in list(self.workers.values()):
            try:
                await w.conn.send({"t": "shutdown"})
            except Exception:
                pass
        deadline = time.time() + 3.0
        for w in list(self.workers.values()):
            if w.proc is not None:
                try:
                    w.proc.wait(timeout=max(0.05, deadline - time.time()))
                except subprocess.TimeoutExpired:
                    w.proc.kill()
        for w in list(self.workers.values()):
            await w.conn.close()
        self._stop_hub()
        for proc in self._procs:
            if proc.poll() is None:
                try:
                    proc.terminate()
                    proc.wait(timeout=2)
                except Exception:
                    try:
                        proc.kill()
                    except Exception:
                        pass
        if self._server is not None:
            self._server.close()
            try:
                await self._server.wait_closed()
            except Exception:
                pass
        try:
            os.unlink(self.socket_path)
        except OSError:
            pass

    def _gpu_count(self) -> int:
        if os.environ.get("MODAL_AMD_FAKE_GPUS"):
            return int(os.environ["MODAL_AMD_FAKE_GPUS"])
        try:
            import torch

            if torch.cuda.is_available():
                return torch.cuda.device_count()
        except Exception:
            pass
        return 0

    async def spawn_worker(self, gpu_index: Optional[int] = None, extra_env: Optional[dict] = None) -> Any:
        worker_id = self._next_worker_id
        self._next_worker_id += 1
        env = dict(os.environ)
        env["MODAL_AMD_WORKER_SOCKET"] = self.socket_path
        env["MODAL_AMD_WORKER_ID"] = str(worker_id)
        env["MODAL_AMD_IS_REMOTE"] = "1"
        if gpu_index is not None:
            env["MODAL_AMD_GPU_INDEX"] = str(gpu_index)
            env["HIP_VISIBLE_DEVICES"] = str(gpu_index)
            env["CUDA_VISIBLE_DEVICES"] = str(gpu_index)
        if extra_env:
            env.update(extra_env)
        self._pending_spawns += 1
        proc = subprocess.Popen(
            [sys.executable, "-m", "modal_amd.runtime.worker"],
            env=env,
            cwd=os.getcwd(),
            start_new_session=True,
        )
        self._procs.append(proc)
        return proc

    async def ensure_workers(self, needs_gpu: bool) -> None:
        have = [w for w in self.workers.values() if w.alive and (w.has_gpu or not needs_gpu)]
        if needs_gpu:
            have = [w for w in have if w.has_gpu]
        if have or self._pending_spawns > 0:
            return
        async with self._spawn_lock:
            have = [w for w in self.workers.values() if w.alive and ((w.has_gpu and needs_gpu) or not needs_gpu)]
            if have or self._pending_spawns > 0:
                return
            from ..config import config

            n_gpus = self._gpu_count()
            if needs_gpu or n_gpus > 0:
                count = config.get("worker_count") or max(n_gpus, 1)
                for i in range(count):
                    await self.spawn_worker(gpu_index=i % n_gpus if n_gpus else None)
            else:
                count = config.get("worker_count") or min(max((_CPU_COUNT or 4) // 2, 1), 8)
                for _ in range(count):
                    await self.spawn_worker(gpu_index=None)

    async def wait_for_worker(self, needs_gpu: bool, timeout: float = 120.0) -> None:
        deadline = time.time() + timeout
        while True:
            if any(w.alive and (w.has_gpu or not needs_gpu) for w in self.workers.values()):
                return
            await self.ensure_workers(needs_gpu)
            self._worker_ready.clear()
            remaining = deadline - time.time()
            if remaining <= 0:
                raise TimeoutError("No worker became available")
            try:
                await asyncio.wait_for(self._worker_ready.wait(), min(remaining, 1.0))
            except asyncio.TimeoutError:
                pass

    async def _on_connect(self, reader: asyncio.StreamReader, writer: asyncio.StreamWriter) -> None:
        conn: Connection = None

        handle_holder: dict = {}

        authed = False

        async def handler(msg: dict) -> None:
            nonlocal authed
            kind = msg.get("t")
            if not authed:
                if kind != "hello" or msg.get("auth") != self.scheduler.auth_token:
                    await conn.close()
                    return
                authed = True
                conn.rpc_target = self.scheduler.rpc_adapter
            if kind == "hello":
                role = msg.get("role", "worker")
                if role == "worker":
                    worker_id = msg.get("worker_id")
                    if worker_id is None or worker_id < 0:
                        worker_id = self._next_worker_id
                        self._next_worker_id += 1
                    gpu_index = msg.get("gpu_index")
                    handle = WorkerHandle(
                        worker_id,
                        conn,
                        gpu_index,
                        external=bool(msg.get("external")),
                    )
                    handle_holder["h"] = handle
                    to_worker = os.path.join(self.run_dir, f"ring.{handle.task_id}.in")
                    from_worker = os.path.join(self.run_dir, f"ring.{handle.task_id}.out")
                    rings_ok = conn.attach_rings(to_worker, from_worker, create=True)
                    lane = rings_ok and self._hub is not None and conn.enable_lane()
                    if lane:
                        handle.hub_slot = self._next_hub_slot
                        self._next_hub_slot += 1
                        self._hub_conns[handle.hub_slot] = conn
                        self._hub.add_ring(handle.hub_slot, conn.ring_in)
                        self._lane.add_worker(handle.hub_slot, conn.ring_out)
                        self._lane_workers[handle.hub_slot] = handle
                        conn.sync_handler = lambda m, h=handle: self._on_lane_frame(h, m)
                        self._lane_refresh_fns.update(
                            rec.function_id for rec, _g in self._lane_groups.values()
                        )
                    self.workers[worker_id] = handle
                    self._pending_spawns = max(0, self._pending_spawns - 1)
                    self._worker_ready.set()
                    self._dispatch_wake.set()
                    await conn.send(
                        {
                            "t": "hello_ack",
                            "task_id": handle.task_id,
                            "worker_id": worker_id,
                            "ring_in": to_worker if rings_ok else None,
                            "ring_out": from_worker if rings_ok else None,
                            "lane_bell": self._hub_bell if lane else None,
                        },
                        via_socket=True,
                    )
                    asyncio.get_running_loop().create_task(self._watch_worker(handle))
                else:
                    await conn.send({"t": "hello_ack"})
                return
            if kind == "putc":
                asyncio.get_running_loop().create_task(
                    self.scheduler.function_put_chunk(**msg["p"])
                )
                return
            handle = handle_holder.get("h")
            if handle is None:
                return
            if kind == "outputs":
                self._on_outputs(handle, msg)
            elif kind == "outputs_chunk":
                self._on_outputs_chunk(handle, msg)
            elif kind == "chunk_done":
                self._on_chunk_done(handle, msg)
            elif kind == "gen_data":
                self.scheduler.on_generator_data(msg)
            elif kind == "hb":
                handle.last_heartbeat = time.time()
                if msg.get("gpu"):
                    handle.gpu_stats = msg["gpu"]
            elif kind == "mesh_ready":
                self.scheduler.on_mesh_ready(handle, bool(msg.get("ok")))
            elif kind == "log":
                self.scheduler.on_worker_log(handle, msg)

        conn = Connection(reader, writer, handler, rpc_target=None)
        conn.start()

    def _on_lane_frame(self, handle: WorkerHandle, msg: dict) -> bool:
        kind = msg.get("t")
        if kind == "chunk_done":
            self._on_chunk_done(handle, msg)
        elif kind == "outputs":
            self._on_outputs(handle, msg)
        elif kind == "outputs_chunk":
            self._on_outputs_chunk(handle, msg)
        elif kind == "hb":
            handle.last_heartbeat = time.time()
            if msg.get("gpu"):
                handle.gpu_stats = msg["gpu"]
        else:
            return False
        return True

    async def _watch_worker(self, handle: WorkerHandle) -> None:
        await handle.conn.wait_closed()
        handle.alive = False
        self.workers.pop(handle.worker_id, None)
        lost: list[str] = []
        if handle.hub_slot is not None:
            self._hub_conns.pop(handle.hub_slot, None)
            self._lane_workers.pop(handle.hub_slot, None)
            handle.lane_fns.clear()
            if self._hub is not None:
                self._hub.remove_ring(handle.hub_slot)
            if self._lane is not None:
                lost = self._lane.remove_worker(handle.hub_slot)
        if self._stopping:
            return
        for token in lost:
            entry = self._lane_groups.get(token)
            if entry is not None and token not in handle.inflight:
                handle.inflight[token] = ("g", entry[0], entry[1])
        for token, entry in list(handle.inflight.items()):
            if type(entry) is tuple:
                _tag, record, group = entry
                if group.state == "done" or record.cancelled:
                    self._lane_groups.pop(token, None)
                    continue
                group.internal_failures += 1
                if group.internal_failures > MAX_INTERNAL_FAILURE_COUNT:
                    self._lane_groups.pop(token, None)
                    for ci in range(group.count):
                        rec = record.materialize_chunk_item(group, ci)
                        self.scheduler.finalize_input(
                            rec,
                            GENERIC_STATUS_INTERNAL_FAILURE,
                            None,
                            0,
                            f"worker died while executing chunk (x{group.internal_failures})",
                            rec.retry_count,
                        )
                    group.state = "done"
                else:
                    group.state = "pending"
                    group.worker_id = None
                    self.enqueue_chunk(record, group, record.function_id, front=True)
                continue
            rec = entry
            if rec.final:
                continue
            rec.internal_failures += 1
            rec.worker_id = None
            if rec.internal_failures > MAX_INTERNAL_FAILURE_COUNT:
                self.scheduler.finalize_input(
                    rec,
                    GENERIC_STATUS_INTERNAL_FAILURE,
                    None,
                    0,
                    f"worker died while executing input (x{rec.internal_failures})",
                    rec.retry_count,
                )
            else:
                self.enqueue(rec, front=True)
        handle.inflight.clear()

    def _on_outputs(self, handle: WorkerHandle, msg: dict) -> None:
        for item in msg["items"]:
            token = item["token"]
            rec = handle.inflight.pop(token, None)
            call_id, idx_s, retry_s = token.rsplit(":", 2)
            if rec is not None:
                fid = rec.call_id
            fdef_id = item.get("function_id")
            if fdef_id:
                cnt = handle.outstanding.get(fdef_id, 0)
                if cnt > 0:
                    handle.outstanding[fdef_id] = cnt - 1
            self.scheduler.on_worker_output(
                call_id=call_id,
                idx=int(idx_s),
                retry_count=int(retry_s),
                status=item["status"],
                output=item.get("data"),
                output_format=item.get("format", 0),
                exc_repr=item.get("exc"),
                output_blob=item.get("data_blob"),
            )
        self._dispatch_wake.set()

    def _on_outputs_chunk(self, handle: WorkerHandle, msg: dict) -> None:
        tokens = msg["tokens"]
        chunk_id = self.scheduler.register_out_chunk(msg["data"], len(tokens))
        fdef_id = msg.get("function_id")
        if fdef_id:
            cnt = handle.outstanding.get(fdef_id, 0)
            handle.outstanding[fdef_id] = max(cnt - len(tokens), 0)
        inflight_pop = handle.inflight.pop
        by_call: dict[str, list] = {}
        for ci, token in enumerate(tokens):
            inflight_pop(token, None)
            call_id, idx_s, retry_s = token.rsplit(":", 2)
            by_call.setdefault(call_id, []).append((int(idx_s), int(retry_s), ci))
        for call_id, triples in by_call.items():
            record = self.scheduler.calls.get(call_id)
            if record is not None:
                record.post_outputs_bulk(triples, chunk_id)
                if getattr(record, "durable", False):
                    import pickle as _pickle

                    from . import wal

                    values = _pickle.loads(msg["data"])
                    for idx, _retry, ci in triples:
                        rec = record.inputs.get(idx)
                        if rec is not None and rec.final:
                            wal.journal_result(
                                self.scheduler, record, rec,
                                output=_pickle.dumps(values[ci], 4),
                                output_format=1,
                            )
                    if (
                        record.num_inputs_final is not None
                        and record.completed >= record.num_inputs_final
                    ):
                        wal.drop(self.scheduler, record.call_id)
        self._dispatch_wake.set()

    def enqueue(self, rec: InputRecord, front: bool = False, function_id: Optional[str] = None) -> None:
        fid = function_id or self._function_id_of(rec)
        q = self.pending.setdefault(fid, deque())
        if front:
            q.appendleft(rec)
        else:
            q.append(rec)
        self._dispatch_wake.set()

    def enqueue_many(self, function_id: str, recs: list) -> None:
        q = self.pending.setdefault(function_id, deque())
        q.extend(recs)
        self._dispatch_wake.set()

    def enqueue_chunk(self, record: Any, group: Any, function_id: str, front: bool = False) -> None:
        if self._lane is not None:
            fdef = self.scheduler.functions.get(function_id)
            if fdef is not None and self._lane_submit(record, group, fdef, front):
                return
        q = self.pending.setdefault(function_id, deque())
        entry = ("g", record, group)
        if front:
            q.appendleft(entry)
        else:
            q.append(entry)
        self._dispatch_wake.set()

    def enqueue_delayed(self, rec: InputRecord, delay_s: float) -> None:
        self._delay_seq += 1
        heapq.heappush(
            self.delayed, (time.time() + delay_s, self._delay_seq, self._function_id_of(rec), rec)
        )

    def _function_id_of(self, rec: InputRecord) -> str:
        return self.scheduler.calls[rec.call_id].function_id

    async def _retry_loop(self) -> None:
        while True:
            if not self.delayed:
                await asyncio.sleep(0.05)
                continue
            ready_at, _, fid, rec = self.delayed[0]
            now = time.time()
            if ready_at <= now:
                heapq.heappop(self.delayed)
                if not rec.final and not rec.cancelled:
                    self.pending.setdefault(fid, deque()).append(rec)
                    self._dispatch_wake.set()
            else:
                await asyncio.sleep(min(ready_at - now, 0.5))

    async def _dispatch_loop(self) -> None:
        while True:
            await self._dispatch_wake.wait()
            self._dispatch_wake.clear()
            try:
                await self._dispatch_once()
            except asyncio.CancelledError:
                raise
            except Exception as exc:
                self.scheduler.log(f"dispatch error: {exc!r}")

    async def _dispatch_once(self) -> None:
        if self._lane_refresh_fns:
            await self._lane_dispatch()
        for fid, q in list(self.pending.items()):
            if not q:
                continue
            fdef = self.scheduler.functions.get(fid)
            if fdef is None:
                q.clear()
                continue
            await self.ensure_workers(fdef.needs_gpu)
            candidates = [
                w
                for w in self.workers.values()
                if w.alive and not w.draining and (w.has_gpu or not fdef.needs_gpu)
            ]
            if fdef.needs_gpu:
                candidates = [w for w in candidates if w.has_gpu]
            candidates = self._apply_placement(fdef, candidates)
            if not candidates:
                continue
            candidates.sort(key=lambda w: w.outstanding.get(fid, 0))
            for w in candidates:
                if not q:
                    break
                credit = w.credit_for(fdef)
                if credit <= 0:
                    continue
                batch: list[InputRecord] = []
                while q and credit > 0:
                    entry = q.popleft()
                    if type(entry) is tuple:
                        _tag, record, group = entry
                        if group.state != "pending" or record.cancelled:
                            continue
                        await self._send_group(w, record, group, fdef)
                        credit -= group.count
                        continue
                    rec = entry
                    if rec.final or rec.cancelled:
                        continue
                    batch.append(rec)
                    credit -= 1
                if batch:
                    await self._send_batch(w, fdef, batch)
            if q:
                await self._maybe_scale_up(fdef, backlog=len(q), active=len(candidates))

    def _apply_placement(self, fdef: FunctionDef, candidates: list) -> list:
        placement = fdef.placement
        if not placement:
            return candidates
        gpu_index = placement.get("gpu_index")
        if gpu_index is not None:
            return [w for w in candidates if w.gpu_index == gpu_index]
        gpu_set = placement.get("gpu_set")
        if gpu_set:
            subset = [w for w in candidates if w.gpu_index in gpu_set]
            if subset:
                return subset
        return candidates

    async def _maybe_scale_up(self, fdef: FunctionDef, backlog: int, active: int) -> None:
        if self._pending_spawns > 0:
            return
        limit = self._pool_limit(fdef)
        if fdef.max_containers:
            limit = min(limit, fdef.max_containers)
        current = sum(
            1 for w in self.workers.values() if w.alive and (w.has_gpu or not fdef.needs_gpu)
        )
        if current >= limit:
            return
        want = min(limit - current, max(1, backlog // DEFAULT_PIPELINE_DEPTH))
        n_gpus = self._gpu_count()
        for i in range(want):
            gpu_index = (current + i) % n_gpus if (fdef.needs_gpu and n_gpus) else (
                (current + i) % n_gpus if n_gpus else None
            )
            await self.spawn_worker(gpu_index=gpu_index)

    async def ensure_min(self, fdef: FunctionDef) -> None:
        want = min(fdef.min_containers + fdef.buffer_containers, self._pool_limit(fdef))
        current = sum(
            1 for w in self.workers.values() if w.alive and (w.has_gpu or not fdef.needs_gpu)
        ) + self._pending_spawns
        n_gpus = self._gpu_count()
        for i in range(max(0, want - current)):
            gpu_index = (current + i) % n_gpus if n_gpus else None
            await self.spawn_worker(gpu_index=gpu_index if fdef.needs_gpu or n_gpus else None)

    def _pool_limit(self, fdef: FunctionDef) -> int:
        from ..config import config

        n_gpus = self._gpu_count()
        configured = config.get("worker_count")
        if fdef.needs_gpu:
            return max(configured or 0, n_gpus, 1)
        if configured:
            return configured
        return min(max((_CPU_COUNT or 4) // 2, 1), 8)

    async def _send_def(self, w: WorkerHandle, fdef: FunctionDef) -> None:
        await w.conn.send(
            {
                "t": "def",
                "function_id": fdef.function_id,
                "app_id": fdef.app_id,
                "name": fdef.name,
                "definition": fdef.definition,
                "definition_kind": fdef.definition_kind,
                "is_generator": fdef.is_generator,
                "timeout": fdef.timeout,
                "max_concurrent_inputs": fdef.max_concurrent_inputs,
                "batch_max_size": fdef.batch_max_size,
                "batch_linger_ms": fdef.batch_linger_ms,
                "version": fdef.definition_version,
                "app_layout": self.scheduler.app_layout(fdef.app_id),
                "env": self.scheduler.resolve_function_env(fdef),
                "volumes": fdef.volume_mounts,
                "python_paths": self.scheduler.resolve_function_pythonpaths(fdef),
                "web_config": fdef.web_config,
            }
        )
        w.functions_loaded.add(fdef.function_id)
        w.defs_version[fdef.function_id] = fdef.definition_version

    async def _send_batch(self, w: WorkerHandle, fdef: FunctionDef, batch: list[InputRecord]) -> None:
        try:
            await self._ensure_unpaged(w)
            if (
                fdef.function_id not in w.functions_loaded
                or w.defs_version.get(fdef.function_id, 0) != fdef.definition_version
            ):
                await self._send_def(w, fdef)
            w.last_active = time.time()
            items = []
            chunks_needed: dict[str, bytes] = {}
            record = None
            for rec in batch:
                rec.worker_id = w.worker_id
                rec.started_at = time.time()
                w.inflight[rec.token] = rec
                item = {
                    "token": rec.token,
                    "input_id": rec.input_id,
                    "method": rec.method_name,
                    "retry_count": rec.retry_count,
                }
                if rec.chunk_id:
                    item["chunk"] = rec.chunk_id
                    item["ci"] = rec.chunk_index
                    if rec.chunk_id not in w.chunks_sent:
                        if record is None or record.call_id != rec.call_id:
                            record = self.scheduler.calls.get(rec.call_id)
                        chunk = record.chunks.get(rec.chunk_id) if record else None
                        if chunk is not None:
                            chunks_needed[rec.chunk_id] = chunk["data"]
                            w.chunks_sent.add(rec.chunk_id)
                else:
                    item["payload"] = rec.payload
                    if rec.payload_blob:
                        item["payload_blob"] = rec.payload_blob
                if rec.cluster:
                    item["cluster"] = rec.cluster
                items.append(item)
            w.outstanding[fdef.function_id] = w.outstanding.get(fdef.function_id, 0) + len(batch)
            frame = {"t": "inputs", "function_id": fdef.function_id, "items": items}
            if chunks_needed:
                frame["chunks"] = chunks_needed
            await w.conn.send(frame)
        except Exception:
            for rec in batch:
                if rec.token in w.inflight:
                    del w.inflight[rec.token]
                if not rec.final:
                    self.enqueue(rec, front=True)

    async def _send_group(self, w: WorkerHandle, record: Any, group: Any, fdef: FunctionDef) -> None:
        try:
            await self._ensure_unpaged(w)
            if (
                fdef.function_id not in w.functions_loaded
                or w.defs_version.get(fdef.function_id, 0) != fdef.definition_version
            ):
                await self._send_def(w, fdef)
            group.state = "inflight"
            group.worker_id = w.worker_id
            w.last_active = time.time()
            w.inflight[group.token] = ("g", record, group)
            w.outstanding[fdef.function_id] = (
                w.outstanding.get(fdef.function_id, 0) + group.count
            )
            chunk = record.chunks.get(group.chunk_id) or {}
            await w.conn.send(
                {
                    "t": "inputs_chunk",
                    "function_id": fdef.function_id,
                    "call_id": record.call_id,
                    "chunk_id": group.chunk_id,
                    "token": group.token,
                    "count": group.count,
                    "payload": chunk.get("data"),
                    "method": group.method,
                    "max_concurrent": fdef.max_concurrent_inputs,
                }
            )
        except Exception:
            w.inflight.pop(group.token, None)
            group.state = "pending"
            if not record.cancelled:
                self.enqueue_chunk(record, group, fdef.function_id, front=True)

    def _on_chunk_done(self, handle: WorkerHandle, msg: dict) -> None:
        if self._lane is not None and handle.hub_slot is not None:
            for token, slot in self._lane.complete(handle.hub_slot, msg["token"]):
                self._lane_assigned(token, slot)
        self._chunk_done_fields(
            handle,
            msg["token"],
            msg["call_id"],
            msg["chunk_id"],
            msg.get("function_id"),
            msg.get("count", 0),
            msg.get("data"),
            msg.get("cis"),
            msg.get("failed"),
            msg.get("exceptions"),
            msg.get("items"),
        )

    def _chunk_done_fields(
        self,
        handle: WorkerHandle,
        token: str,
        call_id: str,
        chunk_id: str,
        fid: Optional[str],
        count: int,
        data: Optional[bytes],
        cis: Optional[list],
        failed: Any = None,
        exceptions: Optional[dict] = None,
        items: Optional[dict] = None,
    ) -> None:
        from .calls import GENERIC_STATUS_FAILURE, GENERIC_STATUS_SUCCESS

        handle.inflight.pop(token, None)
        lane_owned = self._lane_groups.pop(token, None) is not None
        if fid:
            handle.outstanding[fid] = max(handle.outstanding.get(fid, 0) - count, 0)
        if not lane_owned or self.pending.get(fid):
            self._dispatch_wake.set()
        record = self.scheduler.calls.get(call_id)
        if record is None:
            return
        group = record.chunk_groups.get(chunk_id)
        if group is None or group.state == "done":
            return
        if failed:
            group.internal_failures += 1
            if group.internal_failures <= MAX_INTERNAL_FAILURE_COUNT and not record.cancelled:
                group.state = "pending"
                self.enqueue_chunk(record, group, record.function_id, front=True)
            else:
                from .calls import GENERIC_STATUS_INTERNAL_FAILURE as _GIF

                for ci in range(group.count):
                    rec = record.materialize_chunk_item(group, ci)
                    self.scheduler.finalize_input(
                        rec, _GIF, None, 0, "chunk repeatedly failed to start", rec.retry_count
                    )
                group.state = "done"
            return
        for ci_s, (exc_data, repr_s) in (exceptions or {}).items():
            ci = int(ci_s)
            rec = record.materialize_chunk_item(group, ci)
            self.scheduler.on_worker_output(
                call_id=record.call_id,
                idx=rec.idx,
                retry_count=rec.retry_count,
                status=GENERIC_STATUS_FAILURE,
                output=exc_data,
                output_format=1,
                exc_repr=repr_s,
            )
        for ci_s, item_data in (items or {}).items():
            ci = int(ci_s)
            rec = record.materialize_chunk_item(group, ci)
            self.scheduler.on_worker_output(
                call_id=record.call_id,
                idx=rec.idx,
                retry_count=rec.retry_count,
                status=GENERIC_STATUS_SUCCESS,
                output=item_data,
                output_format=1,
                exc_repr=None,
            )
        if data is not None:
            slot = self.scheduler.register_out_chunk(data, count if cis is None else len(cis))
            record.complete_chunk_success(group, cis, slot)
            self.scheduler.metrics_counters["outputs_total"] += (
                count if cis is None else len(cis)
            )
        else:
            group.state = "done"
            record._check_done()

    async def dispatch_gang(self, fdef: FunctionDef, recs: list) -> None:
        n = len(recs)
        deadline = time.time() + 120
        while True:
            await self.ensure_workers(fdef.needs_gpu)
            candidates = [
                w
                for w in self.workers.values()
                if w.alive and not w.draining and (w.has_gpu or not fdef.needs_gpu)
            ]
            if fdef.needs_gpu:
                candidates = [w for w in candidates if w.has_gpu]
            if len(candidates) >= n:
                break
            if time.time() > deadline:
                raise TimeoutError(
                    f"Gang of {n} workers unavailable (have {len(candidates)})"
                )
            await asyncio.sleep(0.05)
        candidates.sort(key=lambda w: (sum(w.outstanding.values()), w.worker_id))
        for rec, w in zip(recs, candidates):
            await self._send_batch(w, fdef, [rec])

    async def cancel_inputs(self, tokens: list[str], terminate: bool = False) -> None:
        if self._lane is not None:
            for token in self._lane.cancel([t for t in tokens if t in self._lane_groups]):
                self._lane_groups.pop(token, None)
        by_worker: dict[int, list[str]] = {}
        for w in self.workers.values():
            hit = [t for t in tokens if t in w.inflight]
            if hit:
                by_worker[w.worker_id] = hit
        for worker_id, toks in by_worker.items():
            w = self.workers.get(worker_id)
            if w is None:
                continue
            try:
                await w.conn.send({"t": "cancel", "tokens": toks, "terminate": terminate})
            except Exception:
                pass
```

Baseline: 1.694 million items/s.

## Move map chunk bookkeeping into a native C++ ledger with in-place frame encoding

```diff
diff --git a/csrc/core.cpp b/csrc/core.cpp
--- a/csrc/core.cpp
+++ b/csrc/core.cpp
@@ -118,6 +118,72 @@
       },
       &assignments);
   return py::make_tuple(completions, raw, assignment_list(assignments));
+}
+
+using modal_amd::ChunkFrame;
+using modal_amd::DrainSummary;
+using modal_amd::Exported;
+
+std::string_view bytes_view(const py::bytes& b) {
+  char* ptr;
+  Py_ssize_t n;
+  if (PyBytes_AsStringAndSize(b.ptr(), &ptr, &n) != 0) throw py::error_already_set();
+  return std::string_view(ptr, (size_t)n);
+}
+
+py::bytes encode_inputs_chunk(const std::string& function_id, const std::string& call_id,
+                              const std::string& chunk_id, const std::string& token,
+                              int64_t count, py::bytes payload, const std::string& method,
+                              int64_t max_concurrent) {
+  ChunkFrame f{function_id, call_id, chunk_id, token, bytes_view(payload), method,
+               count, max_concurrent};
+  size_t n = f.size();
+  if (n == 0) throw std::runtime_error("encode_inputs_chunk: field too long");
+  py::bytes out(nullptr, (ssize_t)n);
+  f.write(reinterpret_cast<uint8_t*>(PyBytes_AsString(out.ptr())));
+  return out;
+}
+
+int lane_put_chunk(ChunkLane& lane, int call_slot, const std::string& chunk_id,
+                   uint64_t base_idx, uint64_t count, py::bytes payload, bool front) {
+  return lane.put_chunk(call_slot, chunk_id, base_idx, count, bytes_view(payload), front);
+}
+
+py::tuple exported_tuple(const Exported& e) {
+  return py::make_tuple(e.token, e.call_slot, e.chunk_id, e.base_idx, e.count,
+                        py::bytes(e.payload), e.worker_slot);
+}
+
+py::list exported_list(const std::vector<Exported>& entries) {
+  py::list out;
+  for (const auto& e : entries) out.append(exported_tuple(e));
+  return out;
+}
+
+py::tuple lane_drain_ledger(ChunkLane& lane, RingHub& hub) {
+  py::list completions, raw, exports, calls, slots;
+  std::vector<Assignment> assignments;
+  DrainSummary summary;
+  lane.drain_ledger(
+      hub,
+      [&](int slot, const ChunkDone& done) {
+        completions.append(py::make_tuple(slot, done_tuple(done)));
+      },
+      [&](int slot, const uint8_t* ptr, size_t len) {
+        raw.append(py::make_tuple(slot, py::bytes(reinterpret_cast<const char*>(ptr), len)));
+      },
+      [&](Exported&& e) { exports.append(exported_tuple(e)); }, &assignments, &summary);
+  for (const auto& c : summary.calls) calls.append(py::make_tuple(c.call_slot, c.chunks, c.items));
+  for (const auto& s : summary.slots) slots.append(py::make_tuple(s.slot, s.completed, s.pushed));
+  return py::make_tuple(calls, slots, exports, completions, raw, assignment_list(assignments));
+}
+
+py::list lane_take_outputs(ChunkLane& lane, int call_slot, uint64_t max_items) {
+  bool over = false;
+  py::list out;
+  for (const auto& g : lane.take_outputs(call_slot, max_items, &over))
+    out.append(py::make_tuple(g.base_idx, g.count, py::bytes(g.data), over));
+  return out;
 }
 
 py::bytes pack_payloads(const std::vector<py::bytes>& items) {
@@ -529,8 +595,35 @@
       .def("queued", &ChunkLane::queued)
       .def("inflight", &ChunkLane::inflight)
       .def("outstanding_items", &ChunkLane::outstanding_items)
-      .def("pushed", &ChunkLane::pushed);
+      .def("pushed", &ChunkLane::pushed)
+      .def("set_fn_consts", &ChunkLane::set_fn_consts, py::arg("fn_slot"),
+           py::arg("function_id"), py::arg("max_concurrent"))
+      .def("set_max_frame", &ChunkLane::set_max_frame)
+      .def("open_call", &ChunkLane::open_call, py::arg("call_slot"), py::arg("fn_slot"),
+           py::arg("call_id"), py::arg("method"))
+      .def("put_chunk", &lane_put_chunk, py::arg("call_slot"), py::arg("chunk_id"),
+           py::arg("base_idx"), py::arg("count"), py::arg("payload"), py::arg("front") = false)
+      .def("drain_ledger", &lane_drain_ledger)
+      .def("take_outputs", &lane_take_outputs, py::arg("call_slot"), py::arg("max_items"))
+      .def("export_token", [](ChunkLane& lane, const std::string& token) {
+        return exported_list(lane.export_token(token));
+      })
+      .def("export_worker", [](ChunkLane& lane, int slot) {
+        return exported_list(lane.export_worker(slot));
+      })
+      .def("export_call", [](ChunkLane& lane, int call_slot) {
+        return exported_list(lane.export_call(call_slot));
+      })
+      .def("close_call", &ChunkLane::close_call)
+      .def("ledger_inflight", &ChunkLane::ledger_inflight)
+      .def("ledger_items", &ChunkLane::ledger_items)
+      .def("ledger_size", &ChunkLane::ledger_size)
+      .def("ledger_bytes", &ChunkLane::ledger_bytes)
+      .def("ready_groups", &ChunkLane::ready_groups);
   m.def("parse_chunk_done", &parse_chunk_done_py);
+  m.def("encode_inputs_chunk", &encode_inputs_chunk, py::arg("function_id"),
+        py::arg("call_id"), py::arg("chunk_id"), py::arg("token"), py::arg("count"),
+        py::arg("payload"), py::arg("method"), py::arg("max_concurrent"));
   m.def("pack_payloads", &pack_payloads);
   m.def("malz_compress", &malz_compress, py::arg("data"), py::arg("min_gain") = 0.95);
   m.def("malz_decompress", &malz_decompress);
diff --git a/csrc/lane.h b/csrc/lane.h
--- a/csrc/lane.h
+++ b/csrc/lane.h
@@ -147,6 +147,89 @@
     for (uint64_t i = 0; i < n; i++)
       if (!skip(depth + 1)) return false;
     return true;
+  }
+};
+
+
+struct MsgWriter {
+  uint8_t* p;
+
+  static size_t str_size(size_t n) { return n + (n < 32 ? 1 : n < 256 ? 2 : n < 65536 ? 3 : 5); }
+  static size_t bin_size(size_t n) { return n + (n < 256 ? 2 : n < 65536 ? 3 : 5); }
+  static size_t int_size(int64_t v) {
+    if (v >= 0) return v < 0x80 ? 1 : v <= 0xff ? 2 : v <= 0xffff ? 3 : v <= 0xffffffffLL ? 5 : 9;
+    return v >= -32 ? 1 : v >= -128 ? 2 : v >= -32768 ? 3 : v >= -2147483648LL ? 5 : 9;
+  }
+
+  void be(uint64_t v, int n) {
+    for (int i = n - 1; i >= 0; i--) *p++ = (uint8_t)(v >> (8 * i));
+  }
+  void raw(std::string_view s) {
+    if (!s.empty()) std::memcpy(p, s.data(), s.size());
+    p += s.size();
+  }
+  void str(std::string_view s) {
+    size_t n = s.size();
+    if (n < 32) *p++ = (uint8_t)(0xa0 | n);
+    else if (n < 256) { *p++ = 0xd9; be(n, 1); }
+    else if (n < 65536) { *p++ = 0xda; be(n, 2); }
+    else { *p++ = 0xdb; be(n, 4); }
+    raw(s);
+  }
+  void bin(std::string_view s) {
+    size_t n = s.size();
+    if (n < 256) { *p++ = 0xc4; be(n, 1); }
+    else if (n < 65536) { *p++ = 0xc5; be(n, 2); }
+    else { *p++ = 0xc6; be(n, 4); }
+    raw(s);
+  }
+  void integer(int64_t v) {
+    if (v >= 0) {
+      if (v < 0x80) *p++ = (uint8_t)v;
+      else if (v <= 0xff) { *p++ = 0xcc; be((uint64_t)v, 1); }
+      else if (v <= 0xffff) { *p++ = 0xcd; be((uint64_t)v, 2); }
+      else if (v <= 0xffffffffLL) { *p++ = 0xce; be((uint64_t)v, 4); }
+      else { *p++ = 0xcf; be((uint64_t)v, 8); }
+    } else if (v >= -32) *p++ = (uint8_t)(int8_t)v;
+    else if (v >= -128) { *p++ = 0xd0; be((uint64_t)v, 1); }
+    else if (v >= -32768) { *p++ = 0xd1; be((uint64_t)v, 2); }
+    else if (v >= -2147483648LL) { *p++ = 0xd2; be((uint64_t)v, 4); }
+    else { *p++ = 0xd3; be((uint64_t)v, 8); }
+  }
+};
+
+struct ChunkFrame {
+  std::string_view function_id, call_id, chunk_id, token, payload, method;
+  int64_t count = 0;
+  int64_t max_concurrent = 0;
+
+  size_t size() const {
+    for (std::string_view s : {function_id, call_id, chunk_id, token, payload, method})
+      if (s.size() > 0xffffffffULL) return 0;
+    using W = MsgWriter;
+    return 1 + W::str_size(1) + W::str_size(12)
+           + W::str_size(11) + W::str_size(function_id.size())
+           + W::str_size(7) + W::str_size(call_id.size())
+           + W::str_size(8) + W::str_size(chunk_id.size())
+           + W::str_size(5) + W::str_size(token.size())
+           + W::str_size(5) + W::int_size(count)
+           + W::str_size(7) + W::bin_size(payload.size())
+           + W::str_size(6) + W::str_size(method.size())
+           + W::str_size(14) + W::int_size(max_concurrent);
+  }
+
+  void write(uint8_t* dst) const {
+    MsgWriter w{dst};
+    *w.p++ = 0x89;
+    w.str("t"); w.str("inputs_chunk");
+    w.str("function_id"); w.str(function_id);
+    w.str("call_id"); w.str(call_id);
+    w.str("chunk_id"); w.str(chunk_id);
+    w.str("token"); w.str(token);
+    w.str("count"); w.integer(count);
+    w.str("payload"); w.bin(payload);
+    w.str("method"); w.str(method);
+    w.str("max_concurrent"); w.integer(max_concurrent);
   }
 };
 
@@ -259,6 +342,39 @@
   int worker_slot;
 };
 
+struct Exported {
+  std::string token;
+  int call_slot;
+  std::string chunk_id;
+  uint64_t base_idx, count;
+  std::string payload;
+  int worker_slot;
+};
+
+struct ReadyGroup {
+  uint64_t base_idx, count;
+  std::string data;
+};
+
+struct DrainSummary {
+  struct CallDone { int call_slot; uint64_t chunks, items; };
+  struct SlotDone { int slot; uint64_t completed, pushed; };
+  std::vector<CallDone> calls;
+  std::vector<SlotDone> slots;
+
+  void call_done(int call_slot, uint64_t items) {
+    for (auto& c : calls)
+      if (c.call_slot == call_slot) { c.chunks++; c.items += items; return; }
+    calls.push_back(CallDone{call_slot, 1, items});
+  }
+  SlotDone& slot(int s) {
+    for (auto& d : slots)
+      if (d.slot == s) return d;
+    slots.push_back(SlotDone{s, 0, 0});
+    return slots.back();
+  }
+};
+
 class ChunkLane {
  public:
   void add_worker(int slot, std::shared_ptr<Ring> ring) {
@@ -292,10 +408,10 @@
              size_t len, bool front) {
     Fn& fn = fns_[fn_slot];
     if (fn.queue.empty() || front) {
-      int slot = place(fn_slot, fn, token, count, frame, len, fn.queue.size());
+      int slot = place(fn_slot, fn, token, count, FrameSrc{frame, len, nullptr}, fn.queue.size());
       if (slot >= 0) return slot;
     }
-    Queued q{token, count, std::string(reinterpret_cast<const char*>(frame), len)};
+    Queued q{token, count, std::string(reinterpret_cast<const char*>(frame), len), false};
     if (front) fn.queue.push_front(std::move(q));
     else fn.queue.push_back(std::move(q));
     return -1;
@@ -307,13 +423,169 @@
     Fn& fn = it->second;
     while (!fn.queue.empty()) {
       Queued& q = fn.queue.front();
+      if (q.ledger) {
+        auto eit = ledger_.find(q.token);
+        if (eit == ledger_.end()) {
+          fn.queue.pop_front();
+          continue;
+        }
+        ChunkFrame f = frame_of(eit->first, eit->second);
+        int slot = place(fn_slot, fn, q.token, q.count, FrameSrc{nullptr, f.size(), &f},
+                         fn.queue.size());
+        if (slot < 0) break;
+        eit->second.worker_slot = slot;
+        if (summary_) summary_->slot(slot).pushed++;
+        fn.queue.pop_front();
+        continue;
+      }
       int slot = place(fn_slot, fn, q.token, q.count,
-                       reinterpret_cast<const uint8_t*>(q.frame.data()), q.frame.size(),
+                       FrameSrc{reinterpret_cast<const uint8_t*>(q.frame.data()),
+                                q.frame.size(), nullptr},
                        fn.queue.size());
       if (slot < 0) break;
       out->push_back(Assignment{std::move(q.token), slot});
       fn.queue.pop_front();
     }
+  }
+
+
+  void set_fn_consts(int fn_slot, std::string function_id, int64_t max_concurrent) {
+    Fn& fn = fns_[fn_slot];
+    fn.function_id = std::move(function_id);
+    fn.max_concurrent = max_concurrent;
+  }
+
+  void set_max_frame(size_t n) { max_frame_ = n; }
+
+  void open_call(int call_slot, int fn_slot, std::string call_id, std::string method) {
+    Call& call = calls_[call_slot];
+    call.fn_slot = fn_slot;
+    call.call_id = std::move(call_id);
+    call.method = std::move(method);
+    call.open = true;
+    fns_[fn_slot];
+  }
+
+  int put_chunk(int call_slot, std::string_view chunk_id, uint64_t base_idx, uint64_t count,
+                std::string_view payload, bool front) {
+    auto cit = calls_.find(call_slot);
+    if (cit == calls_.end() || !cit->second.open) return -3;
+    Call& call = cit->second;
+    Fn& fn = fns_[call.fn_slot];
+    std::string token = "g:";
+    token += chunk_id;
+    if (ledger_.count(token)) return -3;
+    ChunkFrame f{fn.function_id, call.call_id, chunk_id, token, payload, call.method,
+                 (int64_t)count, fn.max_concurrent};
+    size_t len = f.size();
+    if (len == 0 || (max_frame_ && len > max_frame_)) return -3;
+    int slot = -1;
+    if (fn.queue.empty() || front)
+      slot = place(call.fn_slot, fn, token, count, FrameSrc{nullptr, len, &f}, fn.queue.size());
+    LedgerEntry& e = ledger_[token];
+    e.call_slot = call_slot;
+    e.chunk_id.assign(chunk_id);
+    e.base_idx = base_idx;
+    e.count = count;
+    e.payload.assign(payload);
+    e.worker_slot = slot;
+    ledger_bytes_ += e.payload.size();
+    call.live++;
+    if (slot >= 0) return slot;
+    Queued q{std::move(token), count, std::string(), true};
+    if (front) fn.queue.push_front(std::move(q));
+    else fn.queue.push_back(std::move(q));
+    return fn.eligible.empty() ? -2 : -1;
+  }
+
+  std::vector<ReadyGroup> take_outputs(int call_slot, uint64_t max_items, bool* over) {
+    std::vector<ReadyGroup> out;
+    *over = false;
+    auto cit = calls_.find(call_slot);
+    if (cit == calls_.end()) return out;
+    auto& ready = cit->second.ready;
+    uint64_t taken = 0;
+    while (!ready.empty()) {
+      ReadyGroup& g = ready.front();
+      if (g.count > max_items - taken) {
+        if (out.empty()) {
+          *over = true;
+          out.push_back(std::move(g));
+          ready.pop_front();
+        }
+        break;
+      }
+      taken += g.count;
+      out.push_back(std::move(g));
+      ready.pop_front();
+    }
+    return out;
+  }
+
+  std::vector<Exported> export_token(const std::string& token) {
+    std::vector<Exported> out;
+    auto it = ledger_.find(token);
+    if (it != ledger_.end()) out.push_back(export_entry(it));
+    return out;
+  }
+
+  std::vector<Exported> export_worker(int worker_slot) {
+    std::vector<std::string> tokens;
+    auto wit = workers_.find(worker_slot);
+    if (wit != workers_.end())
+      for (auto& entry : wit->second.inflight)
+        if (ledger_.count(entry.first)) tokens.push_back(entry.first);
+    return export_tokens(tokens);
+  }
+
+  std::vector<Exported> export_call(int call_slot) {
+    std::vector<std::string> tokens;
+    for (auto& entry : ledger_)
+      if (entry.second.call_slot == call_slot) tokens.push_back(entry.first);
+    return export_tokens(tokens);
+  }
+
+  void close_call(int call_slot) {
+    auto cit = calls_.find(call_slot);
+    if (cit == calls_.end()) return;
+    Call& call = cit->second;
+    call.open = false;
+    call.ready.clear();
+    bool dropped = false;
+    for (auto it = ledger_.begin(); it != ledger_.end();) {
+      if (it->second.call_slot == call_slot && it->second.worker_slot < 0) {
+        ledger_bytes_ -= it->second.payload.size();
+        call.live--;
+        it = ledger_.erase(it);
+        dropped = true;
+      } else {
+        ++it;
+      }
+    }
+    if (dropped) {
+      auto& q = fns_[call.fn_slot].queue;
+      q.erase(std::remove_if(q.begin(), q.end(),
+                             [&](const Queued& e) { return e.ledger && !ledger_.count(e.token); }),
+              q.end());
+    }
+    if (call.live == 0) calls_.erase(cit);
+  }
+
+  size_t ledger_inflight(int worker_slot) const {
+    auto it = workers_.find(worker_slot);
+    return it == workers_.end() ? 0 : it->second.ledger_chunks;
+  }
+  uint64_t ledger_items(int fn_slot, int worker_slot) const {
+    auto it = workers_.find(worker_slot);
+    if (it == workers_.end()) return 0;
+    auto lit = it->second.load.find(fn_slot);
+    return lit == it->second.load.end() ? 0 : lit->second.ledger_items;
+  }
+  size_t ledger_size() const { return ledger_.size(); }
+  uint64_t ledger_bytes() const { return ledger_bytes_; }
+  size_t ready_groups(int call_slot) const {
+    auto it = calls_.find(call_slot);
+    return it == calls_.end() ? 0 : it->second.ready.size();
   }
 
   bool complete(int worker_slot, std::string_view token, std::vector<Assignment>* out) {
@@ -339,6 +611,7 @@
       auto keep = q.begin();
       for (auto it = q.begin(); it != q.end(); ++it) {
         if (drop.count(it->token)) {
+          if (it->ledger) forget(it->token);
           dropped.push_back(std::move(it->token));
         } else {
           if (keep != it) *keep = std::move(*it);
@@ -354,16 +627,51 @@
     std::vector<std::string> tokens;
     auto it = fns_.find(fn_slot);
     if (it == fns_.end()) return tokens;
-    for (auto& q : it->second.queue) tokens.push_back(std::move(q.token));
+    for (auto& q : it->second.queue) {
+      if (q.ledger) forget(q.token);
+      tokens.push_back(std::move(q.token));
+    }
     it->second.queue.clear();
     return tokens;
   }
 
   template <typename OnClean, typename OnRaw>
   void drain(RingHub& hub, OnClean&& on_clean, OnRaw&& on_raw, std::vector<Assignment>* out) {
+    DrainSummary summary;
+    drain_ledger(hub, on_clean, on_raw, [](Exported&&) {}, out, &summary);
+  }
+
+  template <typename OnClean, typename OnRaw, typename OnExport>
+  void drain_ledger(RingHub& hub, OnClean&& on_clean, OnRaw&& on_raw, OnExport&& on_export,
+                    std::vector<Assignment>* out, DrainSummary* summary) {
     ChunkDone done;
+    struct Scope {
+      DrainSummary*& ref;
+      ~Scope() { ref = nullptr; }
+    } scope{summary_};
+    summary_ = summary;
     hub.drain([&](int slot, const uint8_t* ptr, size_t len) {
       FrameKind kind = parse_chunk_done(ptr, len, &done);
+      if (kind != FrameKind::kOther && !ledger_.empty()) {
+        auto it = ledger_.find(std::string(done.token));
+        if (it != ledger_.end() && it->second.worker_slot == slot) {
+          LedgerEntry& e = it->second;
+          Call& call = calls_.at(e.call_slot);
+          bool whole = kind == FrameKind::kDoneClean && done.cis_nil &&
+                       (uint64_t)done.count == e.count;
+          if (!call.open || whole) {
+            if (call.open) {
+              call.ready.push_back(ReadyGroup{e.base_idx, e.count, std::string(done.data)});
+              summary->call_done(e.call_slot, e.count);
+            }
+            summary->slot(slot).completed++;
+            erase_entry(it);
+            complete(slot, done.token, out);
+            return;
+          }
+          on_export(export_entry(it));
+        }
+      }
       if (kind != FrameKind::kOther) complete(slot, done.token, out);
       if (kind == FrameKind::kDoneClean) on_clean(slot, done);
       else on_raw(slot, ptr, len);
@@ -394,10 +702,31 @@
     std::string token;
     uint64_t count;
     std::string frame;
+    bool ledger;
+  };
+  struct LedgerEntry {
+    int call_slot = 0;
+    std::string chunk_id;
+    uint64_t base_idx = 0, count = 0;
+    std::string payload;
+    int worker_slot = -1;
+  };
+  struct Call {
+    int fn_slot = 0;
+    std::string call_id, method;
+    bool open = true;
+    size_t live = 0;
+    std::deque<ReadyGroup> ready;
+  };
+  struct FrameSrc {
+    const uint8_t* data;
+    size_t len;
+    const ChunkFrame* encode;
   };
   struct Load {
     uint64_t items = 0;
     uint32_t chunks = 0;
+    uint64_t ledger_items = 0;
   };
   struct Inflight {
     int fn_slot;
@@ -407,13 +736,82 @@
     std::shared_ptr<Ring> ring;
     std::unordered_map<int, Load> load;
     std::unordered_map<std::string, Inflight> inflight;
+    size_t ledger_chunks = 0;
   };
   struct Fn {
     uint64_t cap_items = 256;
     uint32_t min_chunks = 1;
     std::deque<Queued> queue;
     std::unordered_set<int> eligible;
+    std::string function_id;
+    int64_t max_concurrent = 0;
   };
+
+  using LedgerMap = std::unordered_map<std::string, LedgerEntry>;
+
+  ChunkFrame frame_of(const std::string& token, const LedgerEntry& e) {
+    const Call& call = calls_.at(e.call_slot);
+    const Fn& fn = fns_.at(call.fn_slot);
+    return ChunkFrame{fn.function_id, call.call_id, e.chunk_id, token, e.payload, call.method,
+                      (int64_t)e.count, fn.max_concurrent};
+  }
+
+  void erase_entry(LedgerMap::iterator it) {
+    release_share(it->second);
+    auto cit = calls_.find(it->second.call_slot);
+    ledger_bytes_ -= it->second.payload.size();
+    ledger_.erase(it);
+    if (cit != calls_.end() && --cit->second.live == 0 && !cit->second.open) calls_.erase(cit);
+  }
+
+  void release_share(const LedgerEntry& e) {
+    if (e.worker_slot < 0) return;
+    auto wit = workers_.find(e.worker_slot);
+    auto cit = calls_.find(e.call_slot);
+    if (wit == workers_.end() || cit == calls_.end()) return;
+    Load& load = wit->second.load[cit->second.fn_slot];
+    load.ledger_items -= std::min(load.ledger_items, e.count);
+    if (wit->second.ledger_chunks) wit->second.ledger_chunks--;
+  }
+
+  void forget(const std::string& token) {
+    auto it = ledger_.find(token);
+    if (it != ledger_.end()) erase_entry(it);
+  }
+
+  Exported export_entry(LedgerMap::iterator it) {
+    LedgerEntry& e = it->second;
+    if (e.worker_slot < 0) {
+      ChunkFrame f = frame_of(it->first, e);
+      for (Queued& q : fns_.at(calls_.at(e.call_slot).fn_slot).queue) {
+        if (q.ledger && q.token == it->first) {
+          q.frame.resize(f.size());
+          f.write(reinterpret_cast<uint8_t*>(q.frame.data()));
+          q.ledger = false;
+          break;
+        }
+      }
+    }
+    Exported out{it->first, e.call_slot, std::move(e.chunk_id), e.base_idx, e.count,
+                 std::string(), e.worker_slot};
+    ledger_bytes_ -= e.payload.size();
+    out.payload = std::move(e.payload);
+    e.payload.clear();
+    erase_entry(it);
+    return out;
+  }
+
+  std::vector<Exported> export_tokens(const std::vector<std::string>& tokens) {
+    std::vector<Exported> out;
+    for (const auto& token : tokens) {
+      auto it = ledger_.find(token);
+      if (it != ledger_.end()) out.push_back(export_entry(it));
+    }
+    std::sort(out.begin(), out.end(), [](const Exported& a, const Exported& b) {
+      return a.base_idx != b.base_idx ? a.base_idx < b.base_idx : a.token < b.token;
+    });
+    return out;
+  }
 
   static bool has_credit(const Fn& fn, const Load& load, size_t backlog) {
     if (load.items < fn.cap_items) return true;
@@ -421,7 +819,7 @@
   }
 
   int place(int fn_slot, Fn& fn, const std::string& token, uint64_t count,
-            const uint8_t* frame, size_t len, size_t backlog) {
+            const FrameSrc& src, size_t backlog) {
     std::vector<std::pair<uint64_t, int>> order;
     for (int slot : fn.eligible) {
       auto it = workers_.find(slot);
@@ -432,10 +830,19 @@
     std::sort(order.begin(), order.end());
     for (auto& cand : order) {
       Worker& w = workers_[cand.second];
-      if (w.ring->too_large(len) || !w.ring->push(frame, len)) continue;
+      if (w.ring->too_large(src.len)) continue;
+      uint8_t* dst = w.ring->reserve(src.len);
+      if (!dst) continue;
+      if (src.encode) src.encode->write(dst);
+      else std::memcpy(dst, src.data, src.len);
+      w.ring->commit();
       Load& load = w.load[fn_slot];
       load.items += count;
       load.chunks++;
+      if (src.encode) {
+        load.ledger_items += count;
+        w.ledger_chunks++;
+      }
       w.inflight[token] = Inflight{fn_slot, count};
       pushed_++;
       return cand.second;
@@ -445,6 +852,11 @@
 
   std::unordered_map<int, Worker> workers_;
   std::unordered_map<int, Fn> fns_;
+  std::unordered_map<int, Call> calls_;
+  LedgerMap ledger_;
+  uint64_t ledger_bytes_ = 0;
+  size_t max_frame_ = 0;
+  DrainSummary* summary_ = nullptr;
   uint64_t pushed_ = 0;
 };
 
diff --git a/csrc/ledger_stress.cpp b/csrc/ledger_stress.cpp
--- /dev/null
+++ b/csrc/ledger_stress.cpp
@@ -0,0 +1,312 @@
+
+#include <poll.h>
+
+#include <atomic>
+#include <cstdio>
+#include <cstdlib>
+#include <set>
+#include <string>
+#include <thread>
+#include <vector>
+
+#include "lane.h"
+#include "ring.h"
+
+using namespace modal_amd;
+
+namespace {
+
+constexpr int kWorkers = 2;
+constexpr int kChunks = 20000;
+constexpr int kPerCall = 2000;
+constexpr int kRemoveAt = 5000;
+constexpr int kClosedCall = 6;
+constexpr uint64_t kRingBytes = 64 * 1024;
+constexpr uint64_t kCount = 64;
+constexpr uint64_t kCapItems = 128;
+constexpr uint32_t kMinChunks = 2;
+constexpr int kFn = 0;
+
+#define CHECK(cond)                                                      \
+  do {                                                                   \
+    if (!(cond)) {                                                       \
+      std::fprintf(stderr, "CHECK failed: %s (line %d)\n", #cond, __LINE__); \
+      std::abort();                                                      \
+    }                                                                    \
+  } while (0)
+
+void put_str(std::string& out, const std::string& s) {
+  out.resize(out.size() + MsgWriter::str_size(s.size()));
+  MsgWriter w{reinterpret_cast<uint8_t*>(out.data()) + out.size() - MsgWriter::str_size(s.size())};
+  w.str(s);
+}
+
+enum Kind { kClean, kExtraKey, kWrongCount };
+Kind kind_of(int seq) { return seq % 10 == 3 ? kExtraKey : seq % 10 == 7 ? kWrongCount : kClean; }
+
+std::string result_of(int seq) { return std::string((size_t)(seq % 700), (char)('a' + seq % 26)); }
+
+std::string encode_done(const std::string& token, int seq) {
+  Kind kind = kind_of(seq);
+  std::string data = result_of(seq);
+  std::string out;
+  out.push_back((char)(kind == kExtraKey ? 0x89 : 0x88));
+  put_str(out, "t");
+  put_str(out, "chunk_done");
+  put_str(out, "token");
+  put_str(out, token);
+  put_str(out, "call_id");
+  put_str(out, "fc-" + std::to_string(seq / kPerCall));
+  put_str(out, "chunk_id");
+  put_str(out, token.substr(2));
+  put_str(out, "function_id");
+  put_str(out, "fu-stress");
+  put_str(out, "count");
+  out.push_back((char)(kind == kWrongCount ? kCount - 1 : kCount));
+  put_str(out, "data");
+  out.push_back((char)0xc5);
+  out.push_back((char)(data.size() >> 8));
+  out.push_back((char)(data.size() & 0xff));
+  out += data;
+  put_str(out, "cis");
+  out.push_back((char)0xc0);
+  if (kind == kExtraKey) {
+    put_str(out, "failed");
+    out.push_back((char)0xc3);
+  }
+  return out;
+}
+
+std::string make_payload(int seq) {
+  std::string out = std::to_string(seq) + ":";
+  out.resize(1024 + (size_t)((seq * 2654435761u) % 3072), (char)('a' + seq % 26));
+  return out;
+}
+
+std::string chunk_id_of(int seq) { return "c" + std::to_string(seq); }
+int seq_of(std::string_view token) { return std::atoi(std::string(token.substr(3)).c_str()); }
+
+std::string expected_frame(int seq) {
+  std::string chunk_id = chunk_id_of(seq), token = "g:" + chunk_id, payload = make_payload(seq);
+  std::string call_id = "fc-" + std::to_string(seq / kPerCall);
+  ChunkFrame f{"fu-stress", call_id, chunk_id, token, payload, "meth", (int64_t)kCount, 3};
+  std::string out(f.size(), '\0');
+  f.write(reinterpret_cast<uint8_t*>(out.data()));
+  return out;
+}
+
+bool wait_fd(int fd, int timeout_ms) {
+  struct pollfd pfd = {fd, POLLIN, 0};
+  return ::poll(&pfd, 1, timeout_ms) > 0;
+}
+
+}
+
+int main() {
+  char dir_template[] = "/tmp/ledger-stress-XXXXXX";
+  CHECK(::mkdtemp(dir_template) != nullptr);
+  std::string dir = dir_template;
+
+  std::vector<std::shared_ptr<Ring>> to_worker_tx, to_worker_rx, from_worker_tx, from_worker_rx;
+  for (int i = 0; i < kWorkers; i++) {
+    std::string in = dir + "/in." + std::to_string(i), outp = dir + "/out." + std::to_string(i);
+    to_worker_tx.push_back(std::make_shared<Ring>(in, kRingBytes, true));
+    to_worker_rx.push_back(std::make_shared<Ring>(in, 0, false));
+    from_worker_tx.push_back(std::make_shared<Ring>(outp, kRingBytes, true));
+    from_worker_rx.push_back(std::make_shared<Ring>(outp, 0, false));
+  }
+
+  std::atomic<bool> stop{false};
+  std::atomic<int> answered{0};
+
+  std::thread worker([&] {
+    RingHub hub(dir + "/worker.bell", 20);
+    for (int i = 0; i < kWorkers; i++) hub.add_ring(i, to_worker_rx[i]);
+    auto sched_bell = std::make_shared<BellFile>(dir + "/sched.bell", true);
+    for (int i = 0; i < kWorkers; i++) from_worker_tx[i]->set_shared_bell(sched_bell);
+    std::vector<std::pair<int, std::string>> replies;
+    while (!stop.load()) {
+      wait_fd(hub.fd(), 50);
+      replies.clear();
+      hub.drain([&](int slot, const uint8_t* ptr, size_t len) {
+        MsgReader r{ptr, ptr + len};
+        uint64_t n_keys;
+        std::string_view key, value, token;
+        CHECK(r.read_map_header(&n_keys) && n_keys == 9);
+        for (int i = 0; i < 5; i++) {
+          CHECK(r.read_str(&key) && r.read_str(&value));
+          if (key == "token") token = value;
+        }
+        CHECK(token.size() > 3);
+        int seq = seq_of(token);
+        std::string body(reinterpret_cast<const char*>(ptr), len);
+        CHECK(body == expected_frame(seq));
+        replies.emplace_back(slot, encode_done(std::string(token), seq));
+      });
+      for (auto& reply : replies) {
+        const auto* ptr = reinterpret_cast<const uint8_t*>(reply.second.data());
+        while (!from_worker_tx[reply.first]->push(ptr, reply.second.size())) {
+          if (stop.load()) return;
+          std::this_thread::yield();
+        }
+        answered.fetch_add(1);
+      }
+    }
+  });
+
+  {
+    RingHub hub(dir + "/sched.bell", 20);
+    ChunkLane lane;
+    for (int i = 0; i < kWorkers; i++) {
+      hub.add_ring(i, from_worker_rx[i]);
+      auto bell = std::make_shared<BellFile>(dir + "/worker.bell", true);
+      to_worker_tx[i]->set_shared_bell(bell);
+      lane.add_worker(i, to_worker_tx[i]);
+      lane.set_eligible(kFn, i, true);
+    }
+    lane.set_cap(kFn, kCapItems, kMinChunks);
+    lane.set_fn_consts(kFn, "fu-stress", 3);
+
+    std::vector<int> delivered(kChunks, 0);
+    std::vector<bool> closed(kChunks, false);
+    std::vector<int> call_settled(kChunks / kPerCall, 0);
+    std::set<std::string> owned;
+    std::set<std::string> ever_owned;
+    int settled = 0, next = 0, exported_by_frame = 0, exported_by_worker = 0, dropped = 0;
+    bool removed = false;
+    int live_workers = kWorkers;
+
+    auto settle = [&](int seq) {
+      settled++;
+      int call = seq / kPerCall;
+      if (++call_settled[call] == kPerCall && call != kClosedCall) lane.close_call(call);
+    };
+    auto deliver = [&](int seq) {
+      CHECK(seq >= 0 && seq < kChunks && !closed[seq]);
+      CHECK(delivered[seq]++ == 0);
+      settle(seq);
+    };
+    auto check_credit = [&] {
+      for (int i = 0; i < live_workers; i++) {
+        CHECK(lane.outstanding_items(kFn, i) <= kCapItems);
+        CHECK(lane.ledger_items(kFn, i) <= lane.outstanding_items(kFn, i));
+      }
+    };
+    auto take = [&](int call) {
+      static const uint64_t kBudgets[] = {1, 64, 100, 200, 128, 63};
+      for (size_t round = 0;; round++) {
+        uint64_t budget = kBudgets[round % 6];
+        bool over = false;
+        std::vector<ReadyGroup> groups = lane.take_outputs(call, budget, &over);
+        if (groups.empty()) break;
+        uint64_t items = 0;
+        for (auto& g : groups) {
+          CHECK(g.count == kCount && g.base_idx % kCount == 0);
+          int seq = (int)(g.base_idx / kCount);
+          CHECK(seq / kPerCall == call && kind_of(seq) == kClean);
+          CHECK(g.data == result_of(seq));
+          items += g.count;
+          deliver(seq);
+        }
+        CHECK(over ? groups.size() == 1 && items > budget : items <= budget);
+      }
+    };
+
+    std::vector<Assignment> assignments;
+    ChunkDone parsed;
+    while (settled < kChunks || lane.ledger_size() > 0) {
+      while (next < kChunks && lane.queued(kFn) < 8) {
+        int call = next / kPerCall;
+        if (next % kPerCall == 0) lane.open_call(call, kFn, "fc-" + std::to_string(call), "meth");
+        if (next == kRemoveAt && !removed) {
+          std::vector<Exported> lost = lane.export_worker(1);
+          hub.remove_ring(1);
+          std::vector<std::string> tokens = lane.remove_worker(1);
+          CHECK(!lost.empty());
+          for (auto it = lost.rbegin(); it != lost.rend(); ++it) {
+            CHECK(it->worker_slot == 1 && it->payload == make_payload(seq_of(it->token)));
+            CHECK(std::find(tokens.begin(), tokens.end(), it->token) != tokens.end());
+            CHECK(owned.insert(it->token).second);
+            ever_owned.insert(it->token);
+            std::string frame = expected_frame(seq_of(it->token));
+            lane.submit(kFn, it->token, it->count,
+                        reinterpret_cast<const uint8_t*>(frame.data()), frame.size(), true);
+            exported_by_worker++;
+          }
+          for (auto& t : tokens) CHECK(owned.count(t) == 1);
+          removed = true;
+          live_workers = 1;
+        }
+        if (call == kClosedCall && next % kPerCall == kPerCall / 2) {
+          take(call);
+          size_t before = lane.ledger_size();
+          lane.close_call(call);
+          CHECK(lane.ledger_size() <= before);
+          CHECK(lane.put_chunk(call, "late", 0, kCount, "x", false) == -3);
+          for (int seq = call * kPerCall; seq < (call + 1) * kPerCall; seq++) {
+            if (delivered[seq] || owned.count("g:" + chunk_id_of(seq))) continue;
+            closed[seq] = true;
+            dropped++;
+            settle(seq);
+          }
+          next = (call + 1) * kPerCall;
+          continue;
+        }
+        std::string payload = make_payload(next);
+        int rc = lane.put_chunk(call, chunk_id_of(next), (uint64_t)next * kCount, kCount, payload,
+                                false);
+        CHECK(rc >= -1 && rc < kWorkers);
+        next++;
+        check_credit();
+      }
+      wait_fd(hub.fd(), 50);
+      assignments.clear();
+      DrainSummary summary;
+      std::vector<int> done_now;
+      auto ordinary_done = [&](std::string_view token) {
+        CHECK(owned.erase(std::string(token)) == 1);
+        done_now.push_back(seq_of(token));
+      };
+      lane.drain_ledger(
+          hub,
+          [&](int, const ChunkDone& done) {
+            CHECK(kind_of(seq_of(done.token)) != kExtraKey);
+            ordinary_done(done.token);
+          },
+          [&](int, const uint8_t* ptr, size_t len) {
+            CHECK(parse_chunk_done(ptr, len, &parsed) == FrameKind::kDoneOther);
+            CHECK(kind_of(seq_of(parsed.token)) == kExtraKey);
+            ordinary_done(parsed.token);
+          },
+          [&](Exported&& e) {
+            int seq = seq_of(e.token);
+            CHECK(kind_of(seq) != kClean && e.worker_slot >= 0);
+            CHECK(e.payload == make_payload(seq) && e.base_idx == (uint64_t)seq * kCount);
+            CHECK(owned.insert(e.token).second);
+            ever_owned.insert(e.token);
+            exported_by_frame++;
+          },
+          &assignments, &summary);
+      for (auto& a : assignments) CHECK(ever_owned.count(a.token) == 1);
+      for (int seq : done_now) deliver(seq);
+      for (auto& c : summary.calls) take(c.call_slot);
+      check_credit();
+    }
+    CHECK(settled == kChunks && owned.empty());
+    CHECK(lane.ledger_size() == 0 && lane.ledger_bytes() == 0 && lane.queued(kFn) == 0);
+    CHECK(lane.inflight(0) == 0 && lane.ledger_inflight(0) == 0);
+    for (int seq = 0; seq < kChunks; seq++) CHECK(delivered[seq] + (closed[seq] ? 1 : 0) == 1);
+    CHECK(exported_by_frame > 1000 && exported_by_worker > 0 && dropped > 0);
+    std::printf(
+        "ledger_stress ok: %d chunks, %d exported by frame, %d by export_worker, %d dropped by "
+        "close_call, pushed=%llu, hub notifies=%llu waits=%llu\n",
+        kChunks, exported_by_frame, exported_by_worker, dropped,
+        (unsigned long long)lane.pushed(), (unsigned long long)hub.notifies(),
+        (unsigned long long)hub.waits());
+    stop.store(true);
+    worker.join();
+  }
+  CHECK(answered.load() > 0);
+  std::string cmd = "rm -rf " + dir;
+  return std::system(cmd.c_str()) == 0 ? 0 : 1;
+}
diff --git a/modal_amd/flash.py b/modal_amd/flash.py
--- a/modal_amd/flash.py
+++ b/modal_amd/flash.py
@@ -151,7 +151,7 @@
             pool = scheduler.pool
             backlog = len(pool.pending.get(function_id, ()))
             inflight = sum(
-                w.outstanding.get(function_id, 0) for w in pool.workers.values()
+                pool.outstanding_for(w, function_id) for w in pool.workers.values()
             )
             replicas = max(1, self.current_replicas())
             return (backlog + inflight) / replicas
@@ -188,7 +188,7 @@
             victims = [
                 w
                 for w in pool.workers.values()
-                if w.alive and not w.draining and not w.inflight
+                if w.alive and not w.draining and not pool.worker_busy(w)
             ][: current - desired]
             for w in victims:
                 w.draining = True
diff --git a/modal_amd/scheduler/calls.py b/modal_amd/scheduler/calls.py
--- a/modal_amd/scheduler/calls.py
+++ b/modal_amd/scheduler/calls.py
@@ -132,6 +132,9 @@
         return f"{self.call_id}:{self.idx}:{self.retry_count}"
 
 
+PORT_READY = ("port",)
+
+
 class ChunkGroup:
 
     __slots__ = (
@@ -180,6 +183,11 @@
         self._waiters: dict[int, asyncio.Future] = {}
         self.gen_queues: dict[int, asyncio.Queue] = {}
         self.done_event = asyncio.Event()
+        self.port: Optional[int] = None
+        self.port_method = ""
+        self.port_ready = 0
+        self.port_signalled = False
+        self.port_retired = False
 
 
     def _drop_chunk(self, chunk_id: str) -> None:
diff --git a/modal_amd/scheduler/core.py b/modal_amd/scheduler/core.py
--- a/modal_amd/scheduler/core.py
+++ b/modal_amd/scheduler/core.py
@@ -19,6 +19,7 @@
     GENERIC_STATUS_TERMINATED,
     MAX_INPUTS_OUTSTANDING_DEFAULT,
     MAX_INTERNAL_FAILURE_COUNT,
+    PORT_READY,
     CallRecord,
     FunctionDef,
     InputRecord,
@@ -244,6 +245,7 @@
                 and now - rec.finished_at > self.CALL_RETENTION_SECONDS
             ):
                 self.calls.pop(call_id, None)
+                self.pool.ledger_close(rec)
                 for chunk_id in list(rec.chunks):
                     rec._drop_chunk(chunk_id)
                 dropped += 1
@@ -519,7 +521,12 @@
                 "task_id": w.task_id,
                 "gpu_index": w.gpu_index,
                 "alive": w.alive,
-                "inflight": len(w.inflight),
+                "inflight": len(w.inflight)
+                + (
+                    self.pool._lane.ledger_inflight(w.hub_slot)
+                    if self.pool._lane is not None and w.hub_slot is not None
+                    else 0
+                ),
                 "last_heartbeat_age": max(0.0, time.time() - w.last_heartbeat),
             }
             if w.gpu_stats:
@@ -608,7 +615,7 @@
     async def function_get_current_stats(self, function_id: str) -> dict:
         backlog = len(self.pool.pending.get(function_id, ()))
         runners = sum(
-            1 for w in self.pool.workers.values() if w.outstanding.get(function_id, 0) > 0
+            1 for w in self.pool.workers.values() if self.pool.outstanding_for(w, function_id) > 0
         )
         return {"backlog": backlog, "num_total_tasks": runners}
 
@@ -752,6 +759,11 @@
                     function_call_id, items, chunks={chunk_id: payload}
                 )
             }
+        if type(payload) is bytes and not getattr(record, "durable", False):
+            base = self.pool.ledger_put(record, fdef, chunk_id, payload, count, method)
+            if base is not None:
+                self.metrics_counters["inputs_total"] += count
+                return {"idx_base": base, "count": count}
         group = record.add_chunk(chunk_id, payload, count, method)
         self.metrics_counters["inputs_total"] += count
         self.pool.enqueue_chunk(record, group, record.function_id)
@@ -778,12 +790,43 @@
         clear_on_success: bool = True,
     ) -> list[dict]:
         record = self._call(function_call_id)
+        if not clear_on_success and record.port is not None:
+            self.pool.ledger_retire(record)
         out: list[dict] = []
         n_vals = 0
 
+        def take_port() -> None:
+            nonlocal n_vals
+            lane, port = self.pool._lane, record.port
+            if lane is None or port is None or n_vals >= max_values:
+                return
+            for base, count, data, over in lane.take_outputs(port, max_values - n_vals):
+                record.port_ready -= count
+                if over:
+                    expand(("g", base, count, self.register_out_chunk(data, count), None))
+                    continue
+                self._out_chunk_seq += 1
+                out.append(
+                    {
+                        "group": True,
+                        "idx_base": base,
+                        "count": count,
+                        "cis": None,
+                        "val_off": 0,
+                        "out_chunk": f"oc{self._out_chunk_seq}",
+                        "status": 1,
+                        "chunk_data": data,
+                    }
+                )
+                n_vals += count
+
         def expand(entry: Any) -> None:
             nonlocal n_vals
-            if type(entry) is tuple and entry and entry[0] == "g":
+            if entry is PORT_READY:
+                record.port_signalled = False
+                if record.port_ready > 0:
+                    take_port()
+            elif type(entry) is tuple and entry and entry[0] == "g":
                 _tag, base, count, out_chunk, cis = entry[:5]
                 val_off = entry[5] if len(entry) > 5 else 0
                 n = count if cis is None else len(cis)
@@ -838,23 +881,28 @@
 
         deadline = time.time() + timeout
         while not out:
-            if record.output_pushback:
-                entry = record.output_pushback.popleft()
-            else:
+            if record.port_ready > 0 and not record.output_pushback:
+                take_port()
+            if not out:
                 try:
-                    remaining = deadline - time.time()
-                    if remaining <= 0:
+                    entry = take_nowait()
+                except asyncio.QueueEmpty:
+                    try:
+                        remaining = deadline - time.time()
+                        if remaining <= 0:
+                            break
+                        entry = await asyncio.wait_for(record.output_ready.get(), remaining)
+                    except asyncio.TimeoutError:
                         break
-                    entry = await asyncio.wait_for(record.output_ready.get(), remaining)
-                except asyncio.TimeoutError:
-                    break
-            expand(entry)
+                expand(entry)
             while n_vals < max_values:
                 try:
                     entry = take_nowait()
                 except asyncio.QueueEmpty:
                     break
                 expand(entry)
+        if record.port is not None and record.port_ready <= 0 and record.done_event.is_set():
+            self.pool.ledger_close(record)
         chunks_seen: set[str] = set()
         for item in out:
             cid = item.get("out_chunk")
@@ -903,6 +951,7 @@
     ) -> None:
         record = self._call(function_call_id)
         record.cancelled = True
+        self.pool.ledger_retire(record)
         tokens = []
         for rec in record.inputs.values():
             if not rec.final:
diff --git a/modal_amd/scheduler/workerhost.py b/modal_amd/scheduler/workerhost.py
--- a/modal_amd/scheduler/workerhost.py
+++ b/modal_amd/scheduler/workerhost.py
@@ -16,6 +16,7 @@
 from .calls import (
     GENERIC_STATUS_INTERNAL_FAILURE,
     MAX_INTERNAL_FAILURE_COUNT,
+    PORT_READY,
     FunctionDef,
     InputRecord,
 )
@@ -105,6 +106,11 @@
         self._lane_fn_version: dict[str, Optional[int]] = {}
         self._lane_groups: dict[str, tuple] = {}
         self._lane_refresh_fns: set[str] = set()
+        self._ledger_on = os.environ.get("MODAL_AMD_LANE_LEDGER", "1") != "0"
+        self._lane_calls: dict[int, Any] = {}
+        self._next_call_slot = 0
+        self._lane_scale_fns: set[str] = set()
+        self._limit_inputs_cache: Optional[tuple] = None
 
     def _start_hub(self) -> None:
         if not native_lane_enabled():
@@ -112,6 +118,7 @@
         try:
             self._hub = _core.RingHub(self._hub_bell, 20)
             self._lane = _core.ChunkLane()
+            self._lane.set_max_frame(LANE_MAX_FRAME)
             asyncio.get_running_loop().add_reader(self._hub.fd(), self._on_hub_ready)
         except Exception as exc:
             self._hub = None
@@ -134,7 +141,13 @@
         hub, lane = self._hub, self._lane
         if hub is None or lane is None:
             return
-        completions, raw_frames, assignments = lane.drain(hub)
+        if self._lane_calls:
+            calls, slots, exports, completions, raw_frames, assignments = lane.drain_ledger(hub)
+            self._ledger_settled(calls, slots)
+            for entry in exports:
+                self._ledger_import(entry)
+        else:
+            completions, raw_frames, assignments = lane.drain(hub)
         for token, slot in assignments:
             self._lane_assigned(token, slot)
         workers = self._lane_workers
@@ -167,6 +180,7 @@
                     w.lane_fns.discard(fid)
                     self._lane.set_eligible(slot, w.hub_slot, False)
             self._lane.set_cap(slot, credit_cap(fdef), LANE_MIN_CHUNKS)
+            self._lane.set_fn_consts(slot, fid, fdef.max_concurrent_inputs)
             self._lane_fn_version[fid] = fdef.definition_version
         return slot
 
@@ -197,9 +211,51 @@
         if slot >= 0:
             self._lane_assigned(token, slot)
         else:
-            self._lane_refresh_fns.add(fdef.function_id)
+            self._lane_backlogged(fdef)
+        return True
+
+    def _lane_backlogged(self, fdef: FunctionDef, no_eligible: Optional[bool] = None) -> None:
+        fid = fdef.function_id
+        eligible = 0
+        for w in self._lane_workers.values():
+            if fid in w.lane_fns:
+                eligible += 1
+        if no_eligible is None:
+            no_eligible = eligible == 0
+        if no_eligible or eligible < len(self._lane_workers):
+            self._lane_refresh_fns.add(fid)
             self._dispatch_wake.set()
-        return True
+        elif self._scale_headroom(fdef):
+            self._lane_scale_fns.add(fid)
+            self._dispatch_wake.set()
+
+    def _scale_headroom(self, fdef: FunctionDef) -> bool:
+        if self._pending_spawns > 0:
+            return False
+        limit = self._pool_limit(fdef)
+        if fdef.max_containers:
+            limit = min(limit, fdef.max_containers)
+        if len(self.workers) < limit:
+            return True
+        any_kind = not fdef.needs_gpu
+        current = 0
+        for w in self.workers.values():
+            if w.alive and (any_kind or w.gpu_index is not None):
+                current += 1
+        return current < limit
+
+    async def _lane_autoscale(self) -> None:
+        lane = self._lane
+        for fid in list(self._lane_scale_fns):
+            self._lane_scale_fns.discard(fid)
+            fn_slot = self._lane_fn_slots.get(fid)
+            fdef = self.scheduler.functions.get(fid)
+            if lane is None or fn_slot is None or fdef is None:
+                continue
+            backlog = lane.queued(fn_slot)
+            if backlog:
+                active = sum(1 for w in self._lane_workers.values() if fid in w.lane_fns)
+                await self._maybe_scale_up(fdef, backlog=backlog, active=active)
 
     def _lane_assigned(self, token: str, slot: int) -> None:
         entry = self._lane_groups.get(token)
@@ -272,6 +328,130 @@
             if backlog:
                 await self._maybe_scale_up(fdef, backlog=backlog, active=len(candidates))
 
+    def ledger_put(
+        self, record: Any, fdef: FunctionDef, chunk_id: str, payload: bytes, count: int, method: str
+    ) -> Optional[int]:
+        lane = self._lane
+        if (
+            lane is None
+            or not self._ledger_on
+            or not self._lane_workers
+            or record.cancelled
+            or record.port_retired
+        ):
+            return None
+        self._lane_fn_slot(fdef)
+        port = record.port
+        if port is None:
+            port = self._ledger_open(record, fdef, method)
+        elif record.port_method != method:
+            return None
+        base = record.next_idx
+        placed = lane.put_chunk(port, chunk_id, base, count, payload)
+        if placed == -3:
+            return None
+        record.next_idx = base + count
+        if placed >= 0:
+            w = self._lane_workers.get(placed)
+            if w is not None:
+                w.last_active = time.time()
+                w.conn.ring_frames_sent += 1
+        else:
+            self._lane_backlogged(fdef, no_eligible=placed == -2)
+        return base
+
+    def _ledger_open(self, record: Any, fdef: FunctionDef, method: str) -> int:
+        port = self._next_call_slot
+        self._next_call_slot += 1
+        self._lane.open_call(port, self._lane_fn_slots[fdef.function_id], record.call_id, method)
+        self._lane_calls[port] = record
+        record.port = port
+        record.port_method = method
+        return port
+
+    def ledger_close(self, record: Any) -> None:
+        port, record.port = record.port, None
+        if port is None:
+            return
+        self._lane_calls.pop(port, None)
+        record.port_ready = 0
+        if self._lane is not None:
+            self._lane.close_call(port)
+
+    def ledger_retire(self, record: Any) -> None:
+        record.port_retired = True
+        port, lane = record.port, self._lane
+        if port is None or lane is None:
+            return
+        for entry in lane.export_call(port):
+            self._ledger_import(entry)
+        for base, count, data, _over in lane.take_outputs(port, 1 << 62):
+            out_chunk = self.scheduler.register_out_chunk(data, count)
+            record.output_ready.put_nowait(("g", base, count, out_chunk, None))
+        self.ledger_close(record)
+
+    def _ledger_import(self, entry: tuple) -> None:
+        from .calls import ChunkGroup
+
+        token, port, chunk_id, base_idx, count, payload, slot = entry
+        record = self._lane_calls.get(port)
+        if record is None:
+            return
+        group = ChunkGroup(chunk_id, base_idx, count, record.port_method)
+        record.chunks[chunk_id] = {"data": payload, "refs": count}
+        record.chunk_groups[chunk_id] = group
+        self._lane_groups[token] = (record, group)
+        w = self._lane_workers.get(slot) if slot >= 0 else None
+        if w is not None:
+            group.state = "inflight"
+            group.worker_id = w.worker_id
+            w.inflight[token] = ("g", record, group)
+            fid = record.function_id
+            w.outstanding[fid] = w.outstanding.get(fid, 0) + count
+
+    def _ledger_settled(self, calls: list, slots: list) -> None:
+        now = time.time()
+        workers = self._lane_workers
+        for slot, completed, pushed in slots:
+            w = workers.get(slot)
+            if w is not None:
+                w.last_active = now
+                w.conn.ring_frames_received += completed
+                w.conn.ring_frames_sent += pushed
+        total = 0
+        for port, _chunks, items in calls:
+            record = self._lane_calls.get(port)
+            if record is None:
+                continue
+            total += items
+            record.completed += items
+            record.port_ready += items
+            if not record.port_signalled:
+                record.port_signalled = True
+                record.output_ready.put_nowait(PORT_READY)
+            record._check_done()
+        if total:
+            self.scheduler.metrics_counters["outputs_total"] += total
+            if self.pending and any(self.pending.values()):
+                self._dispatch_wake.set()
+
+    def worker_busy(self, w: WorkerHandle) -> bool:
+        if w.inflight:
+            return True
+        return (
+            self._lane is not None
+            and w.hub_slot is not None
+            and self._lane.ledger_inflight(w.hub_slot) > 0
+        )
+
+    def outstanding_for(self, w: WorkerHandle, function_id: str) -> int:
+        n = w.outstanding.get(function_id, 0)
+        if self._lane is not None and w.hub_slot is not None:
+            fn_slot = self._lane_fn_slots.get(function_id)
+            if fn_slot is not None:
+                n += self._lane.ledger_items(fn_slot, w.hub_slot)
+        return n
+
     async def start(self) -> None:
         os.makedirs(self.run_dir, exist_ok=True)
         self._start_hub()
@@ -299,7 +479,7 @@
             for w in self.workers.values()
             if w.alive
             and not w.draining
-            and not w.inflight
+            and not self.worker_busy(w)
             and not w.external
             and now - w.last_active > window
         ]
@@ -353,7 +533,7 @@
                 if not w.alive:
                     continue
                 stale = now - w.last_heartbeat
-                if stale > 60.0 and w.inflight:
+                if stale > 60.0 and self.worker_busy(w):
                     self.scheduler.log(
                         f"worker {w.worker_id} missed heartbeats for {stale:.0f}s; recycling"
                     )
@@ -522,6 +702,9 @@
                         conn.sync_handler = lambda m, h=handle: self._on_lane_frame(h, m)
                         self._lane_refresh_fns.update(
                             rec.function_id for rec, _g in self._lane_groups.values()
+                        )
+                        self._lane_refresh_fns.update(
+                            fid for fid, s in self._lane_fn_slots.items() if self._lane.queued(s)
                         )
                     self.workers[worker_id] = handle
                     self._pending_spawns = max(0, self._pending_spawns - 1)
@@ -592,6 +775,9 @@
         self.workers.pop(handle.worker_id, None)
         lost: list[str] = []
         if handle.hub_slot is not None:
+            if self._lane is not None and not self._stopping:
+                for entry in self._lane.export_worker(handle.hub_slot):
+                    self._ledger_import(entry)
             self._hub_conns.pop(handle.hub_slot, None)
             self._lane_workers.pop(handle.hub_slot, None)
             handle.lane_fns.clear()
@@ -775,6 +961,8 @@
     async def _dispatch_once(self) -> None:
         if self._lane_refresh_fns:
             await self._lane_dispatch()
+        if self._lane_scale_fns:
+            await self._lane_autoscale()
         for fid, q in list(self.pending.items()):
             if not q:
                 continue
@@ -793,11 +981,11 @@
             candidates = self._apply_placement(fdef, candidates)
             if not candidates:
                 continue
-            candidates.sort(key=lambda w: w.outstanding.get(fid, 0))
+            candidates.sort(key=lambda w: self.outstanding_for(w, fid))
             for w in candidates:
                 if not q:
                     break
-                credit = w.credit_for(fdef)
+                credit = credit_cap(fdef) - self.outstanding_for(w, fid)
                 if credit <= 0:
                     continue
                 batch: list[InputRecord] = []
@@ -863,11 +1051,18 @@
             gpu_index = (current + i) % n_gpus if n_gpus else None
             await self.spawn_worker(gpu_index=gpu_index if fdef.needs_gpu or n_gpus else None)
 
+    def _limit_inputs(self) -> tuple:
+        cached = self._limit_inputs_cache
+        now = time.monotonic()
+        if cached is None or now >= cached[0]:
+            from ..config import config
+
+            cached = (now + 1.0, self._gpu_count(), config.get("worker_count"))
+            self._limit_inputs_cache = cached
+        return cached[1], cached[2]
+
     def _pool_limit(self, fdef: FunctionDef) -> int:
-        from ..config import config
-
-        n_gpus = self._gpu_count()
-        configured = config.get("worker_count")
+        n_gpus, configured = self._limit_inputs()
         if fdef.needs_gpu:
             return max(configured or 0, n_gpus, 1)
         if configured:
@@ -1105,6 +1300,11 @@
 
     async def cancel_inputs(self, tokens: list[str], terminate: bool = False) -> None:
         if self._lane is not None:
+            if self._lane_calls:
+                for t in tokens:
+                    if t.startswith("g:") and t not in self._lane_groups:
+                        for entry in self._lane.export_token(t):
+                            self._ledger_import(entry)
             for token in self._lane.cancel([t for t in tokens if t in self._lane_groups]):
                 self._lane_groups.pop(token, None)
         by_worker: dict[int, list[str]] = {}
```

After: 1.695 million items/s (median of 2 runs). About the same (+0.1%).
